# duwt/OrienMask

Hardware: AMD Instinct MI355X
Metric: images/sec end-to-end (544^2, bs=32) forward+postprocess (higher is better)
Workload: dtype f32 (fp32 tensors and accumulation; products from hi/lo fp16 pairs of the fp32 operands, three fp16 MFMAs per product group)

## Files before the change

### include/orienmask_hip.h

```cpp
#ifndef ORIENMASK_HIP_H
#define ORIENMASK_HIP_H

#include <stddef.h>
#include <stdint.h>

#ifdef __cplusplus
extern "C" {
#endif

#define OM_VERSION 140

#define OM_OK 0
#define OM_EINVAL (-1)
#define OM_ESTATE (-2)
#define OM_ENOMEM (-3)
#define OM_EHIP (-4)

#define OM_MAX_SCALES 3
#define OM_MAX_ANCHORS 9

typedef struct om_model om_model;
typedef void* om_stream;

typedef struct om_layer_info {
// ... 40 lines not shown
int om_model_layer_info(const om_model* m, int index, om_layer_info* info);
size_t om_model_weight_floats(const om_model* m);
int om_model_load_weights(om_model* m, const void* packed_dev, size_t bytes, int dtype);

size_t om_model_weight_split_words(const om_model* m);
int om_model_load_weights_split(om_model* m, const void* packed_split_dev, size_t bytes);
int om_model_set_precision(om_model* m, int mode);
int om_model_set_latency_cells(om_model* m, long long cells);
int om_model_set_latency_ksplit(om_model* m, int max_parts);
int om_model_get_precision(const om_model* m);
int om_model_set_upsample_on_read(om_model* m, int enable);

size_t om_forward_workspace_bytes(const om_model* m, int B, int H, int W);
int om_forward(om_model* m, const float* x, int B, int H, int W, float* bbox32, float* bbox16, float* bbox8,
               float* oriens, void* workspace, size_t ws_bytes, om_stream stream);
#define OM_STATUS_SPLIT_RANGE 1
#define OM_STATUS_SK_TIMEOUT 2
size_t om_forward_status_offset(const om_model* m, int B, int H, int W);

size_t om_model_weight_halfs(const om_model* m);
int om_model_load_weights_f16(om_model* m, const void* packed_f16_dev, size_t bytes);
size_t om_forward_f16_workspace_bytes(const om_model* m, int B, int H, int W);
int om_forward_f16(om_model* m, const float* x, int B, int H, int W, float* bbox32, float* bbox16, float* bbox8,
                   float* oriens, void* workspace, size_t ws_bytes, om_stream stream);
int om_layer_tile_f16(const om_model* m, int index, int B, int H, int W, int* bm, int* bn, int* algo);

int om_layer_output_view(const om_model* m, int index, int B, int H, int W, int f16, size_t* byte_offset, int* channels,
                         int* pix_stride, int* div);
int om_model_keep_activations(om_model* m, int keep);

int om_layer_tile(const om_model* m, int index, int B, int H, int W, int* bm, int* bn, int* algo);
int om_profile_enable(om_model* m, int enable);
int om_profile_enable_layers(om_model* m, const unsigned char* layer_mask, int n_layers);
int om_profile_read(om_model* m, float* layer_ms, float* layer_pre_ms, int n_layers, int* n_forwards);

int om_conv2d(const float* in, int B, int H, int W, int cin, int in_pix_stride, const float* w,
              const float* scale, const float* shift, int cout, int ksize, int stride, int leaky,
              const float* res, int res_pix_stride, float* out, int out_pix_stride, om_stream stream);
int om_conv2d_mode(const float* in, int B, int H, int W, int cin, int in_pix_stride, const float* w,
                   const float* scale, const float* shift, int cout, int ksize, int stride, int leaky,
                   const float* res, int res_pix_stride, float* out, int out_pix_stride, int out_mode, int up,
                   om_stream stream);
size_t om_conv2d_winograd_scratch_bytes(int B, int H, int W, int cin);
int om_conv2d_winograd(const float* in, int B, int H, int W, int cin, int in_pix_stride, const float* u,
                       const float* scale, const float* shift, int cout, int leaky, const float* res,
                       int res_pix_stride, float* out, int out_pix_stride, void* scratch, size_t scratch_bytes,
                       om_stream stream);
int om_conv2d_f16(const void* in, int B, int H, int W, int cin, int in_pix_stride, const void* w, const float* scale,
                  const float* shift, int cout, int ksize, int stride, int leaky, const void* res, int res_pix_stride,
                  void* out, int out_pix_stride, int out_f32, om_stream stream);
int om_conv2d_stem_f16(const float* in, int B, int H, int W, const float* w, const float* scale, const float* shift,
                       int cout, void* out, om_stream stream);
size_t om_conv2d_winograd24_scratch_bytes(int B, int H, int W, int cin);
int om_conv2d_winograd24(const float* in, int B, int H, int W, int cin, int in_pix_stride, const float* u,
                         const float* scale, const float* shift, int cout, int leaky, const float* res,
                         int res_pix_stride, float* out, int out_pix_stride, void* scratch, size_t scratch_bytes,
                         om_stream stream);
int om_conv2d_split(const float* in, int B, int H, int W, int cin, int in_pix_stride, const void* w_split,
                    const float* scale_split, const float* shift, int cout, int ksize, int stride, int leaky, const float* res,
                    int res_pix_stride, float* out, int out_pix_stride, int out_mode, int up, int tile_bm, int tile_bn,
                    int32_t* status_dev, om_stream stream);
int om_conv2d_split_k(const float* in, int B, int H, int W, int cin, int in_pix_stride, const void* w_split,
                      const float* scale_split, const float* shift, int cout, int ksize, int stride, int leaky, const float* res,
                      int res_pix_stride, float* out, int out_pix_stride, int out_mode, int up, int tile_bm, int tile_bn,
                      int max_parts, int32_t* status_dev, om_stream stream);
int om_conv2d_split_gather(int nseg, const float* const* seg_ptr, const int* seg_channels, const int* seg_pix_stride,
                           const int* seg_up, int B, int H, int W, const void* w_split, const float* scale_split, const float* shift,
                           int cout, int leaky, float* out, int out_pix_stride, int32_t* status_dev, om_stream stream);
int om_conv2d_winograd24_split(const float* in, int B, int H, int W, int cin, int in_pix_stride, const void* u_split,
                               const float* scale_split, const float* shift, int cout, int leaky, const float* res,
                               int res_pix_stride, float* out, int out_pix_stride, void* scratch, size_t scratch_bytes,
                               int32_t* status_dev, om_stream stream);
int om_conv2d_wino14_split(const float* in, int B, int H, int W, int cin, int in_pix_stride, const void* u14_split,
                           const float* scale_split, const float* shift, int cout, int leaky, const float* res,
                           int res_pix_stride, float* out, int out_pix_stride, int32_t* status_dev, om_stream stream);
int om_conv2d_wino14_blocks(int B, int H, int W, int* classes, int* row_pitch, long long* m_tiles);
size_t om_conv2d_wino14_wide_scratch_bytes(int B, int H, int W, int cin);
int om_conv2d_wino14_wide(const float* in, int B, int H, int W, int cin, int in_pix_stride, const void* u14_split,
                          const float* scale_split, const float* shift, int cout, int leaky, const float* res,
                          int res_pix_stride, float* out, int out_pix_stride, void* scratch, size_t scratch_bytes,
                          int32_t* status_dev, om_stream stream);
int om_set_wino14_wide(int on);
int om_get_wino14_wide(void);
int om_set_stem_fusion(int which, int on);
int om_get_stem_fusion(int which);
int om_set_conv3x3_f16_variant(int mode);
int om_get_conv3x3_f16_variant(void);
int om_conv2d_stem(const float* in, int B, int H, int W, const float* w, const float* scale,
                   const float* shift, int cout, float* out, om_stream stream);
int om_conv2d_stem2_split(const float* in, int B, int H, int W, const float* w1, const float* scale1, const float* shift1,
                          const void* w2_split, const float* scale2_split, const float* shift2, int cout2, int leaky2, float* out,
                          int out_pix_stride, int32_t* status_dev, om_stream stream);
int om_conv2d_stem3_split(const float* in, int B, int H, int W, const float* w1, const float* scale1, const float* shift1,
                          const void* w2_split, const float* scale2_split, const float* shift2, int cout2, int leaky2, float* out,
                          int out_pix_stride, const void* w3_split, const float* scale3_split, const float* shift3, int cout3, int leaky3,
                          float* out3, int out3_pix_stride, int32_t* status_dev, om_stream stream);
int om_conv2d_stem2_f16(const float* in, int B, int H, int W, const float* w1, const float* scale1, const float* shift1,
                        const void* w2_f16, const float* scale2, const float* shift2, int cout2, int leaky2, void* out,
                        int out_pix_stride, om_stream stream);

int om_preprocess(const float* in_nhwc, int N, int h, int w, int resize_h, int resize_w, const float* mean3,
                  const float* std3, int pad_top, int pad_left, int out_h, int out_w, float pad_value, float* out_nchw,
                  om_stream stream);
int om_pad_nchw(const float* in, long long planes, int h, int w, int pad_top, int pad_left, int out_h, int out_w,
                float pad_value, float* out, om_stream stream);

size_t om_postprocess_workspace_bytes(const om_post_cfg* cfg, int B);
int om_postprocess(const om_post_cfg* cfg, const float* bbox32, const float* bbox16, const float* bbox8,
                   const float* oriens, int B, float* out_bbox, int64_t* out_cls, uint8_t* out_mask,
                   int32_t* out_count, int32_t* out_keep, void* workspace, size_t ws_bytes, om_stream stream);
int om_postprocess_detect(const om_post_cfg* cfg, const float* bbox32, const float* bbox16, const float* bbox8, int B,
                          float* out_bbox, int64_t* out_cls, int32_t* out_count, int32_t* out_keep, void* workspace, size_t ws_bytes,
                          om_stream stream);
int om_postprocess_assemble(const om_post_cfg* cfg, const float* oriens, int B, const int32_t* out_count, uint8_t* out_mask,
                            void* workspace, size_t ws_bytes, om_stream stream);
int om_model_attach_postprocess(om_model* m, const om_post_cfg* cfg, float* out_bbox, int64_t* out_cls, uint8_t* out_mask,
                                int32_t* out_count, int32_t* out_keep, void* post_workspace, size_t post_ws_bytes);

int om_postprocess_candidates(const om_post_cfg* cfg, const float* bbox32, const float* bbox16, const float* bbox8, int B,
                              float* cand_dets, int64_t* cand_cls, int32_t* cand_field, int32_t* cand_count, void* workspace,
                              size_t ws_bytes, om_stream stream);
int om_postprocess_masks(const om_post_cfg* cfg, const float* oriens, int B, const float* dets, const int32_t* field,
                         const int32_t* count, uint8_t* out_mask, void* workspace, size_t ws_bytes, om_stream stream);

int om_post_kernel_occupancy(int which, int* threads, int* vgprs, int* lds_bytes, int* max_blocks_per_cu);

int om_recover_bbox(const float* bbox, int K, int stride, const int32_t* collate_pad6, const int32_t* pad6, int hflip,
                    int vflip, int orig_h, int orig_w, float* out_xywh, om_stream stream);
int om_recover_masks_rle(const uint8_t* mask, int K, int H, int W, int crop_top, int crop_down, int crop_left,
                         int crop_right, int hflip, int vflip, int orig_h, int orig_w, uint32_t* counts, int max_runs,
                         int32_t* n_runs, uint8_t* resized_or_null, om_stream stream);
typedef struct om_rle_image {
    const uint8_t* mask;
    int32_t K, H, W;
    int32_t crop_top, crop_down, crop_left, crop_right;
    int32_t hflip, vflip, orig_h, orig_w;
} om_rle_image;
int om_recover_masks_rle_strings(const om_rle_image* images, int n_images, uint32_t* counts, int max_runs, int32_t* n_runs,
                                 uint8_t* str_bytes, long long str_capacity, int32_t* str_cursor, int32_t* str_off,
                                 int32_t* str_len, om_stream stream);

#define OM_VIS_MAX_KEPT 512
#define OM_VIS_BATCH 16
typedef struct om_vis_image {
    const float* image;
    uint8_t* out;
    float* out_float;
    const uint8_t* mask;
    const int32_t* keep;
    const float* colors;
    const int32_t* boxes;
    int32_t n_keep, Hn, Wn;
    int32_t crop_left, crop_right, crop_top, crop_down;
    int32_t h, w;
    int32_t with_mask, draw_boxes;
    float alpha;
} om_vis_image;
size_t om_visualize_workspace_bytes(const om_vis_image* images, int n_images);
int om_visualize(const om_vis_image* images, int n_images, void* workspace, size_t ws_bytes, om_stream stream);

size_t om_cocoeval_workspace_bytes(long long bitmap_words, int n_masks);
int om_cocoeval_masks(int n_masks, const int32_t* mask_hw, const int64_t* mask_word_off, const int32_t* mask_src_first,
                      const int64_t* mask_src_word_off, int n_poly, int n_srcs, const int32_t* src_kind, const int32_t* src_mask, const int64_t* src_data_off,
                      const int32_t* src_len, const int64_t* src_word_off, const double* poly, const uint32_t* counts,
                      const uint8_t* strings, long long bitmap_words, void* workspace, size_t ws_bytes, om_stream stream);
int om_cocoeval_mask_stats(int n_masks, long long bitmap_words, const void* workspace, int32_t* stats, om_stream stream);
// ... 146 lines not shown
```

### orienmask_amd/csrc/conv_igemm_split.hip

```cpp
#include <cstdlib>

#include "conv_f16_common.h"

namespace om {

struct IgemmSParams {
    const _Float16* in;
    const _Float16* w;
    const float* scale;
    const float* shift;
    const float* res;
    float* out;
    int* ticket;
    int* status;
    int H, W, cin_h, in_pix_stride_h;
    int Ho, Wo, HoWo, cout;
    int ks, stride, pad;
    int M, kc, ksteps, taps;
    int n_tiles, total_tiles;
    float* partial;
    int* kflags;
    int ksplit, total_tickets, m_tiles;
    int leaky, res_pix_stride, out_pix_stride, out_mode, up;
    int vec_io;
    int total_in_pixels;
    int w_bytes;
    int nseg, nimg;
    const _Float16* seg_ptr[4];
    int seg_stride_h[4], seg_shift[4], seg_end[4];
};

template <int BM, int BN>
constexpr int split_blocks_per_cu() { return BM * BN >= 256 * 128 ? 2 : (BM * BN >= 128 * 128 ? 3 : 4); }

template <int BM, int BN, int WM, int WN, bool FAST = false>
__device__ __forceinline__ void split_epilogue(const IgemmSParams& p, f32x4* smem, const f32x16 (&acc)[WM / 32][WN / 32],
                                               int m0, int n0, int tid, int wm, int wn, int fi, int fk, float (&sc)[8], float (&sh)[8]) {
    constexpr int TM = WM / 32, TN = WN / 32;
    constexpr int CH8 = BN / 8;
    constexpr int RP = 256 / CH8;
    constexpr int CH = BN / 4;
    f32x4* sC = smem;
    const int n8 = tid % CH8, r0 = tid / CH8;
    const int n = n0 + n8 * 8;
    const int nvalid = p.cout - n;
    const bool vec = p.vec_io && nvalid >= 8;
    if constexpr (!FAST) {
#pragma unroll
        for (int k = 0; k < 8; ++k) { sc[k] = p.scale[n + k]; sh[k] = p.shift[n + k]; }
    }
    float nonfinite = 0.f;
#pragma unroll 1
    for (int pass = 0; pass < BM / WM; ++pass) {
        if (wm == pass) {
#pragma unroll
            for (int a = 0; a < TM; ++a) {
                const int ml = a * 32 + fi;
#pragma unroll
                for (int b = 0; b < TN; ++b)
#pragma unroll
                    for (int g = 0; g < 4; ++g) {
                        const int n4 = (wn * WN + b * 32) / 4 + 2 * g + fk;
                        f32x4 v = {acc[a][b][4 * g], acc[a][b][4 * g + 1], acc[a][b][4 * g + 2], acc[a][b][4 * g + 3]};
                        sC[ml * CH + (n4 ^ (ml & 7))] = v;
                    }
            }
        }
        asm volatile("s_waitcnt lgkmcnt(0)" ::: "memory");
        __builtin_amdgcn_s_barrier();
        if constexpr (FAST) {
#pragma unroll
            for (int ps = 0; ps < (WM + RP - 1) / RP; ++ps) {
                const int ml = ps * RP + r0;
                const int m = m0 + pass * WM + ml;
                if (ml >= WM) continue;
                const f32x4 v0 = sC[ml * CH + ((2 * n8) ^ (ml & 7))];
                const f32x4 v1 = sC[ml * CH + ((2 * n8 + 1) ^ (ml & 7))];
                float v[8] = {v0[0], v0[1], v0[2], v0[3], v1[0], v1[1], v1[2], v1[3]};
#pragma unroll
                for (int k = 0; k < 8; ++k) {
                    const float t = fmaf(v[k], sc[k], sh[k]);
                    v[k] = p.leaky ? (t > 0.f ? t : t * 0.1f) : t;
                    nonfinite = fmaf(t, 0.f, nonfinite);
                }
                if (m < p.M) {
                    float* o = p.out + (size_t)m * p.out_pix_stride + n;
                    *reinterpret_cast<f32x4*>(o) = f32x4{v[0], v[1], v[2], v[3]};
                    *reinterpret_cast<f32x4*>(o + 4) = f32x4{v[4], v[5], v[6], v[7]};
                }
            }
        } else if (p.out_mode != 2) {
#pragma unroll 2
            for (int ps = 0; ps < (WM + RP - 1) / RP; ++ps) {
                const int ml = ps * RP + r0;
                const int m = m0 + pass * WM + ml;
                if (ml >= WM || m >= p.M || nvalid <= 0) continue;
                const f32x4 v0 = sC[ml * CH + ((2 * n8) ^ (ml & 7))];
                const f32x4 v1 = sC[ml * CH + ((2 * n8 + 1) ^ (ml & 7))];
                float v[8] = {v0[0], v0[1], v0[2], v0[3], v1[0], v1[1], v1[2], v1[3]};
#pragma unroll
                for (int k = 0; k < 8; ++k) {
                    const float t = fmaf(v[k], sc[k], sh[k]);
                    v[k] = p.leaky ? (t > 0.f ? t : t * 0.1f) : t;
                    nonfinite = fmaf(t, 0.f, nonfinite);
                }
                if (p.out_mode == 0) {
                    float* o = p.out + (size_t)m * p.out_pix_stride + n;
                    if (p.res) {
                        const float* rp = p.res + (size_t)m * p.res_pix_stride + n;
                        if (vec) {
                            const f32x4 ra = *reinterpret_cast<const f32x4*>(rp), rb = *reinterpret_cast<const f32x4*>(rp + 4);
#pragma unroll
                            for (int k = 0; k < 4; ++k) { v[k] += ra[k]; v[4 + k] += rb[k]; }
                        } else {
                            for (int k = 0; k < 8 && k < nvalid; ++k) v[k] += rp[k];
                        }
                    }
                    if (vec) {
                        *reinterpret_cast<f32x4*>(o) = f32x4{v[0], v[1], v[2], v[3]};
                        *reinterpret_cast<f32x4*>(o + 4) = f32x4{v[4], v[5], v[6], v[7]};
                    } else {
                        for (int k = 0; k < 8 && k < nvalid; ++k) o[k] = v[k];
                    }
                } else {
                    const int bi = m / p.HoWo;
                    const int rr = m - bi * p.HoWo;
                    const int oy = rr / p.Wo, ox = rr - oy * p.Wo;
                    const int Wu = p.Wo * p.up;
                    const size_t base = ((size_t)bi * p.Ho * p.up + (size_t)oy * p.up) * Wu + (size_t)ox * p.up;
                    for (int dy = 0; dy < p.up; ++dy)
                        for (int dx = 0; dx < p.up; ++dx) {
                            float* o = p.out + (base + (size_t)dy * Wu + dx) * p.out_pix_stride + n;
                            if (vec) {
                                *reinterpret_cast<f32x4*>(o) = f32x4{v[0], v[1], v[2], v[3]};
                                *reinterpret_cast<f32x4*>(o + 4) = f32x4{v[4], v[5], v[6], v[7]};
                            } else {
                                for (int k = 0; k < 8 && k < nvalid; ++k) o[k] = v[k];
                            }
                        }
                }
            }
        } else {
            const float* sCf = reinterpret_cast<const float*>(smem);
            const int nch = min(BN, p.cout - n0);
            for (int idx = tid; idx < nch * WM; idx += 256) {
                const int nl = idx / WM, ml = idx - nl * WM;
                const int m = m0 + pass * WM + ml;
                if (m >= p.M) continue;
                const int nn = n0 + nl;
                float t = fmaf(sCf[(ml * CH + ((nl >> 2) ^ (ml & 7))) * 4 + (nl & 3)], p.scale[nn], p.shift[nn]);
                nonfinite = fmaf(t, 0.f, nonfinite);
                if (p.leaky) t = t > 0.f ? t : t * 0.1f;
                const int bi = m / p.HoWo;
                const int rr = m - bi * p.HoWo;
                p.out[((size_t)bi * p.cout + nn) * p.HoWo + rr] = t;
            }
        }
        asm volatile("s_waitcnt lgkmcnt(0)" ::: "memory");
        __builtin_amdgcn_s_barrier();
    }
    if (p.status && nonfinite != nonfinite) atomicOr(p.status, OM_STATUS_SPLIT_RANGE);
}

template <int BN>
__device__ __forceinline__ void split_scale_shift(const IgemmSParams& p, int n0, int tid, float (&sc)[8], float (&sh)[8]) {
    const int n = n0 + (tid % (BN / 8)) * 8;
    const f32x4 a0 = *reinterpret_cast<const f32x4*>(p.scale + n), a1 = *reinterpret_cast<const f32x4*>(p.scale + n + 4);
    const f32x4 b0 = *reinterpret_cast<const f32x4*>(p.shift + n), b1 = *reinterpret_cast<const f32x4*>(p.shift + n + 4);
#pragma unroll
    for (int k = 0; k < 4; ++k) { sc[k] = a0[k]; sc[4 + k] = a1[k]; sh[k] = b0[k]; sh[4 + k] = b1[k]; }
}

__device__ __forceinline__ void split8(const f32x4& x0, const f32x4& x1, f16x8& hi, f16x8& lo) {
#pragma unroll
    for (int i = 0; i < 4; ++i) {
        hi[i] = (_Float16)x0[i];
        hi[4 + i] = (_Float16)x1[i];
    }
#pragma unroll
    for (int i = 0; i < 4; ++i) {
        lo[i] = (_Float16)(x0[i] - (float)hi[i]);
        lo[4 + i] = (_Float16)(x1[i] - (float)hi[4 + i]);
    }
}

template <int BM, int BN, int WM, int WN, bool FAST = false, int NBUF = 3>
__global__ __launch_bounds__(256, (NBUF > 3 ? 2 : split_blocks_per_cu<BM, BN>())) void conv_igemm_split_kernel(const IgemmSParams p) {
    constexpr int TM = WM / 32, TN = WN / 32;
    constexpr int NWN = BN / WN;
    constexpr int A_CH = BM / 64, B_CH = (BN + 63) / 64, NP = A_CH + B_CH;
    constexpr int STAGE = (BM + (BN < 64 ? 64 : BN)) * 4;
    static_assert((BM / WM) * (BN / WN) == 4, "four waves per workgroup");
    static_assert(BM % 64 == 0, "A tile = whole 64-row pieces");
    static_assert(WM * BN / 4 <= NBUF * STAGE, "one wave-row of the fp32 C tile must fit in the operand ring");
    __shared__ f32x4 smem[NBUF * STAGE + 1];
    int* const s_ticket = reinterpret_cast<int*>(smem + NBUF * STAGE);
    constexpr bool KSPLIT = NBUF > 3;

    const int tid = threadIdx.x;
    const int lane = tid & 63;
    const int wave = tid >> 6;
    const int wave_u = __builtin_amdgcn_readfirstlane(wave);
    const int wm = wave / NWN, wn = wave % NWN;
    const int lrow = tid >> 2, lcol = tid & 3;
    const int scol = lcol ^ ((lrow >> 2) & 3);
    const int fi = lane & 31, fk = lane >> 5;
    const int fsw = (fi >> 2) & 3;

    for (int round = 0;; ++round) {
        int tile;
        int s_begin = 0, nsteps = p.ksteps;
        [[maybe_unused]] int part = 0;
        int tile_n, tile_m;
        if constexpr (KSPLIT) {
            if (round) break;
            const int b = blockIdx.x, x = b & 7;
            int unit = b >> 3;
            for (int y = 0; y < x; ++y) unit += (p.total_tickets - y + 7) >> 3;
            tile_m = unit % p.m_tiles;
            const int t = unit / p.m_tiles;
            tile_n = t % p.n_tiles;
            part = t / p.n_tiles;
            tile = tile_m * p.n_tiles + tile_n;
            s_begin = part * p.ksteps / p.ksplit;
            nsteps = (part + 1) * p.ksteps / p.ksplit - s_begin;
        } else {
            if (tid == 0) *s_ticket = atomicAdd(p.ticket, 1);
            asm volatile("s_waitcnt lgkmcnt(0)" ::: "memory");
            __builtin_amdgcn_s_barrier();
            tile = *s_ticket;
            if (tile >= p.total_tiles) break;
            tile = __builtin_amdgcn_readfirstlane(tile);
            tile_n = tile % p.n_tiles;
            tile_m = tile / p.n_tiles;
        }
        const int m0 = tile_m * BM, n0 = tile_n * BN;

        int rowoff[A_CH];
        unsigned invmask[A_CH];
        const int b_first = (m0 < p.M ? m0 : p.M - 1) / p.HoWo;
#pragma unroll
        for (int j = 0; j < A_CH; ++j) {
            int m = m0 + lrow + 64 * j;
            const bool mok = m < p.M;
            if (!mok) m = p.M - 1;
            const int b = m / p.HoWo;
            const int rr = m - b * p.HoWo;
            const int oy = rr / p.Wo;
            const int ox = rr - oy * p.Wo;
            const int iy0 = oy * p.stride - p.pad, ix0 = ox * p.stride - p.pad;
            rowoff[j] = (((b - b_first) * p.H * p.W + iy0 * p.W + ix0) * p.in_pix_stride_h + scol * 8) * 2;
            unsigned badrow = 0, badcol = 0;
#pragma unroll
            for (int k = 0; k < 3; ++k) {
                badrow |= ((unsigned)(iy0 + k) < (unsigned)p.H ? 0u : 1u) << k;
// ... 76 lines not shown
#pragma unroll
        for (int st = 0; st < NBUF; ++st) {
#pragma unroll
            for (int piece = 0; piece < NP; ++piece) issue_piece(piece, st, st < nsteps);
            advance();
        }
        asm volatile("s_waitcnt vmcnt(%0)" ::"i"((NBUF - 1) * NP) : "memory");
        __builtin_amdgcn_s_barrier();
        read_raw(0);
        convert();
        int buf = 0;
        for (int s = 0; s < nsteps; ++s) {
            const int buf1 = buf == NBUF - 1 ? 0 : buf + 1;
            asm volatile("s_waitcnt vmcnt(%0) lgkmcnt(0)" ::"i"((NBUF - 2) * NP) : "memory");
            __builtin_amdgcn_s_barrier();
            read_raw(buf1);
            const bool live3 = s + NBUF < nsteps;
#pragma unroll
            for (int piece = 0; piece < NP; ++piece) issue_piece(piece, buf, live3);
#pragma unroll
            for (int a = 0; a < TM; ++a)
#pragma unroll
                for (int b = 0; b < TN; ++b) {
                    acc[a][b] = __builtin_amdgcn_mfma_f32_32x32x16_f16(bh[b], al[a], acc[a][b], 0, 0, 0);
                    acc[a][b] = __builtin_amdgcn_mfma_f32_32x32x16_f16(bl[b], ah[a], acc[a][b], 0, 0, 0);
                    acc[a][b] = __builtin_amdgcn_mfma_f32_32x32x16_f16(bh[b], ah[a], acc[a][b], 0, 0, 0);
                }
            convert();
            buf = buf1;
            advance();
        }
        asm volatile("s_waitcnt vmcnt(0) lgkmcnt(0)" ::: "memory");
        __syncthreads();

        if constexpr (KSPLIT) {
            if (p.ksplit > 1) {
                const auto rs_part = __builtin_amdgcn_make_buffer_rsrc(p.partial, 0, 0x7FFFFFFF, 0x00020000);
                constexpr int PART_BYTES = TM * TN * 4 * 256 * 16;
                const int pbase = (tile * p.ksplit + part) * PART_BYTES + tid * 16;
#pragma unroll
                for (int a = 0; a < TM; ++a)
#pragma unroll
                    for (int b = 0; b < TN; ++b)
#pragma unroll
                        for (int g = 0; g < 4; ++g) {
                            const f32x4 v = {acc[a][b][4 * g], acc[a][b][4 * g + 1], acc[a][b][4 * g + 2], acc[a][b][4 * g + 3]};
                            __builtin_amdgcn_raw_buffer_store_b128(__builtin_bit_cast(__attribute__((__vector_size__(4 * sizeof(unsigned)))) unsigned, v),
                                                                   rs_part, pbase, ((a * TN + b) * 4 + g) * 256 * 16, 16);
                        }
                asm volatile("s_waitcnt vmcnt(0)" ::: "memory");
                __syncthreads();
                if (tid == 0) s_ticket[1] = __hip_atomic_fetch_add(p.kflags + tile, 1, __ATOMIC_RELAXED, __HIP_MEMORY_SCOPE_AGENT);
                __syncthreads();
                if (s_ticket[1] != p.ksplit - 1) break;
#pragma unroll
                for (int a = 0; a < TM; ++a)
#pragma unroll
                    for (int b = 0; b < TN; ++b)
#pragma unroll
                        for (int r = 0; r < 16; ++r) acc[a][b][r] = 0.f;
                for (int q = 0; q < p.ksplit; ++q) {
                    const int qbase = (tile * p.ksplit + q) * PART_BYTES + tid * 16;
#pragma unroll
                    for (int a = 0; a < TM; ++a)
#pragma unroll
                        for (int b = 0; b < TN; ++b)
#pragma unroll
                            for (int g = 0; g < 4; ++g) {
                                const f32x4 v = __builtin_bit_cast(f32x4, __builtin_amdgcn_raw_buffer_load_b128(rs_part, qbase, ((a * TN + b) * 4 + g) * 256 * 16, 16));
#pragma unroll
                                for (int k = 0; k < 4; ++k) acc[a][b][4 * g + k] += v[k];
                            }
                }
                asm volatile("s_waitcnt vmcnt(0)" ::: "memory");
            }
        }

        float sc[8], sh[8];
        if constexpr (FAST) split_scale_shift<BN>(p, n0, tid, sc, sh);
        split_epilogue<BM, BN, WM, WN, FAST>(p, smem, acc, m0, n0, tid, wm, wn, fi, fk, sc, sh);
    }
}

template <int BM, int BN, int WM, int WN, bool GATHER = false, bool FAST = false, int NBUF = 2>
__global__ __launch_bounds__(256, 2) void conv_igemm_split_wide_kernel(const IgemmSParams p) {
    constexpr int TM = WM / 32, TN = WN / 32;
    constexpr int NWN = BN / WN;
    constexpr int A_CH = BM / 32, B_CH = BN / 32, NP = A_CH + B_CH;
    constexpr bool KSPLIT = NBUF > 2;
    static_assert(!(KSPLIT && GATHER), "the deep-ring form has no gathered input");
    constexpr int STAGE = (BM + BN) * 8;
    static_assert((BM / WM) * (BN / WN) == 4, "four waves per workgroup");
    static_assert(BM % 32 == 0 && BN % 32 == 0, "whole 32-row pieces");
    static_assert(WM * BN / 4 <= NBUF * STAGE, "one wave-row of the fp32 C tile must fit in the operand ring");
    __shared__ f32x4 smem[NBUF * STAGE + 1];
    int* const s_ticket = reinterpret_cast<int*>(smem + NBUF * STAGE);

    const int tid = threadIdx.x;
    const int lane = tid & 63;
    const int wave = tid >> 6;
    const int wave_u = __builtin_amdgcn_readfirstlane(wave);
    const int wm = wave / NWN, wn = wave % NWN;
    const int lrow = tid >> 3, lcol = tid & 7;
    const int scol = lcol ^ ((lrow >> 1) & 7);
    const int fi = lane & 31, fk = lane >> 5;
    const int fsw = (fi >> 1) & 7;

    if constexpr (!KSPLIT) {
        if (tid == 0) *s_ticket = atomicAdd(p.ticket, 1);
        asm volatile("s_waitcnt lgkmcnt(0)" ::: "memory");
        __builtin_amdgcn_s_barrier();
    }
    for (int round = 0;; ++round) {
        int tile, tile_n, tile_m;
        [[maybe_unused]] int part = 0;
        if constexpr (KSPLIT) {
            if (round) break;
            const int b = blockIdx.x, x = b & 7;
            int unit = b >> 3;
            for (int y = 0; y < x; ++y) unit += (p.total_tickets - y + 7) >> 3;
            tile_m = unit % p.m_tiles;
            const int t = unit / p.m_tiles;
            tile_n = t % p.n_tiles;
            part = t / p.n_tiles;
            tile = tile_m * p.n_tiles + tile_n;
        } else {
            tile = *s_ticket;
            if (tile >= p.total_tiles) break;
            tile = __builtin_amdgcn_readfirstlane(tile);
            tile_n = tile % p.n_tiles;
            tile_m = tile / p.n_tiles;
        }
        const int m0 = tile_m * BM, n0 = tile_n * BN;

        int rowoff[A_CH];
        unsigned invmask[A_CH];
        [[maybe_unused]] int g_img[A_CH], g_y[A_CH], g_x[A_CH];
        const int b_first = (m0 < p.M ? m0 : p.M - 1) / p.HoWo;
#pragma unroll
        for (int j = 0; j < A_CH; ++j) {
            int m = m0 + lrow + 32 * j;
            const bool mok = m < p.M;
            if (!mok) m = p.M - 1;
            const int b = m / p.HoWo;
            const int rr = m - b * p.HoWo;
            const int oy = rr / p.Wo;
            const int ox = rr - oy * p.Wo;
            const int iy0 = oy * p.stride - p.pad, ix0 = ox * p.stride - p.pad;
            rowoff[j] = (((b - b_first) * p.H * p.W + iy0 * p.W + ix0) * p.in_pix_stride_h + scol * 8) * 2;
            if constexpr (GATHER) { g_img[j] = b - b_first; g_y[j] = oy; g_x[j] = ox; }
            unsigned badrow = 0, badcol = 0;
#pragma unroll
            for (int k = 0; k < 3; ++k) {
                badrow |= ((unsigned)(iy0 + k) < (unsigned)p.H ? 0u : 1u) << k;
                badcol |= ((unsigned)(ix0 + k) < (unsigned)p.W ? 0u : 1u) << k;
            }
            unsigned inv;
            if (p.ks == 3) {
                inv = ((badrow & 1u) ? 0x007u : 0u) | ((badrow & 2u) ? 0x038u : 0u) | ((badrow & 4u) ? 0x1C0u : 0u) | badcol * 0x49u;
            } else {
                inv = (badrow | badcol) & 1u;
            }
            invmask[j] = mok ? inv : 0xFFFFFFFFu;
        }
        int rowoffB[B_CH];
        const int row_halfs = p.taps * p.cin_h;
#pragma unroll
        for (int j = 0; j < B_CH; ++j) rowoffB[j] = ((n0 + lrow + 32 * j) * row_halfs + scol * 8) * 2;
        const _Float16* in_base = p.in + (size_t)b_first * p.H * p.W * p.in_pix_stride_h;
        const size_t in_left = ((size_t)p.total_in_pixels - (size_t)b_first * p.H * p.W) * p.in_pix_stride_h * 2;
        int in_bytes = in_left < 0x7FFFFFFFull ? (int)in_left : 0x7FFFFFFF;
        [[maybe_unused]] int seg = 0, seg_c0 = 0, seg_c1 = 0x7FFFFFFF;
        [[maybe_unused]] auto set_segment = [&](int g) {
            auto pick = [g](const auto (&v)[4]) { return g == 0 ? v[0] : g == 1 ? v[1] : g == 2 ? v[2] : v[3]; };
            const int sh = pick(p.seg_shift), Hs = p.Ho >> sh, Ws = p.Wo >> sh, st = pick(p.seg_stride_h);
            in_base = pick(p.seg_ptr) + (size_t)b_first * Hs * Ws * st;
            const size_t left = (size_t)(p.nimg - b_first) * Hs * Ws * st * 2;
            in_bytes = left < 0x7FFFFFFFull ? (int)left : 0x7FFFFFFF;
#pragma unroll
            for (int j = 0; j < A_CH; ++j)
                rowoff[j] = (((g_img[j] * Hs + (g_y[j] >> sh)) * Ws + (g_x[j] >> sh)) * st + scol * 8) * 2;
            seg = g;
            seg_c0 = g == 0 ? 0 : g == 1 ? p.seg_end[0] : g == 2 ? p.seg_end[1] : p.seg_end[2];
            seg_c1 = pick(p.seg_end);
        };
        if constexpr (GATHER) set_segment(0);

        const int kc2 = p.kc >> 1;
        int nstages = p.taps * kc2;
        int n_kh = 0, n_kw = 0, n_cc = 0;
        if constexpr (KSPLIT) {
            const int s_begin = part * nstages / p.ksplit;
            nstages = (part + 1) * nstages / p.ksplit - s_begin;
            const int tap0 = s_begin / kc2;
            n_cc = s_begin - tap0 * kc2;
            n_kh = tap0 / p.ks;
            n_kw = tap0 - n_kh * p.ks;
        }
        auto advance = [&]() {
            if (++n_cc == kc2) {
                n_cc = 0;
                if (++n_kw == p.ks) { n_kw = 0; ++n_kh; }
            }
        };
        auto issue_piece = [&](int piece, int buf, bool live) {
            f32x4* dst = smem + buf * STAGE + wave_u * 64;
            if (piece < A_CH) {
                const int j = piece;
                if constexpr (GATHER) {
                    if (piece == 0 && live && n_cc >= seg_c1) set_segment(seg + 1);
                }
                const auto rs_in = __builtin_amdgcn_make_buffer_rsrc(const_cast<_Float16*>(in_base), 0, live ? in_bytes : 0, 0x00020000);
                const int tap = n_kh * p.ks + n_kw;
                const int tap_off = GATHER ? (n_cc - seg_c0) * 128
                                           : ((n_kh * p.W + n_kw) * p.in_pix_stride_h + n_cc * 64) * 2;
                const int voff = (rowoff[j] + tap_off) | ((invmask[j] << (31 - tap)) & 0x80000000u);
                __builtin_amdgcn_raw_ptr_buffer_load_lds(rs_in, (lds_ptr_t)(dst + j * 256), 16, voff, 0, 0, 0);
            } else {
                const int j = piece - A_CH;
                const auto rs_w = __builtin_amdgcn_make_buffer_rsrc(const_cast<_Float16*>(p.w), 0, live ? p.w_bytes : 0, 0x00020000);
                const int koff = ((n_kh * p.ks + n_kw) * p.cin_h + n_cc * 64) * 2;
                const int vo = rowoffB[j] + koff;
                __builtin_amdgcn_raw_ptr_buffer_load_lds(rs_w, (lds_ptr_t)(dst + BM * 8 + j * 256), 16, vo, 0, 0, 0);
            }
        };

// ... 35 lines not shown
                    acc[a][b] = __builtin_amdgcn_mfma_f32_32x32x16_f16(bh[b], ah[a], acc[a][b], 0, 0, 0);
                }
        };

#pragma unroll
        for (int st = 0; st < NBUF; ++st) {
#pragma unroll
            for (int piece = 0; piece < NP; ++piece) issue_piece(piece, st, st < nstages);
            advance();
        }
        [[maybe_unused]] int next_ticket = 0;
        if constexpr (!KSPLIT) {
            if (tid == 0) next_ticket = atomicAdd(p.ticket, 1);
        }
        asm volatile("s_waitcnt vmcnt(%0)" ::"i"((NBUF - 1) * NP) : "memory");
        __builtin_amdgcn_s_barrier();
        read_raw(0, 0);
        convert();
        int buf = 0;
        for (int s = 0; s < nstages; ++s) {
            read_raw(buf, 1);
            multiply();
            convert();
            asm volatile("s_waitcnt vmcnt(%0) lgkmcnt(0)" ::"i"((NBUF - 2) * NP) : "memory");
            __builtin_amdgcn_s_barrier();
            const bool live2 = s + NBUF < nstages;
#pragma unroll
            for (int piece = 0; piece < NP; ++piece) issue_piece(piece, buf, live2);
            advance();
            const int buf1 = buf == NBUF - 1 ? 0 : buf + 1;
            read_raw(buf1, 0);
            multiply();
            convert();
            buf = buf1;
        }
        asm volatile("s_waitcnt vmcnt(0) lgkmcnt(0)" ::: "memory");
        if constexpr (!KSPLIT) {
            if (tid == 0) *s_ticket = next_ticket;
        }
        __syncthreads();
        if constexpr (KSPLIT) {
            if (p.ksplit > 1) {
                const auto rs_part = __builtin_amdgcn_make_buffer_rsrc(p.partial, 0, 0x7FFFFFFF, 0x00020000);
                constexpr int PART_BYTES = TM * TN * 4 * 256 * 16;
                const int pbase = (tile * p.ksplit + part) * PART_BYTES + tid * 16;
#pragma unroll
                for (int a = 0; a < TM; ++a)
#pragma unroll
                    for (int b = 0; b < TN; ++b)
#pragma unroll
                        for (int g = 0; g < 4; ++g) {
                            const f32x4 v = {acc[a][b][4 * g], acc[a][b][4 * g + 1], acc[a][b][4 * g + 2], acc[a][b][4 * g + 3]};
                            __builtin_amdgcn_raw_buffer_store_b128(__builtin_bit_cast(__attribute__((__vector_size__(4 * sizeof(unsigned)))) unsigned, v),
                                                                   rs_part, pbase, ((a * TN + b) * 4 + g) * 256 * 16, 16);
                        }
                asm volatile("s_waitcnt vmcnt(0)" ::: "memory");
                __syncthreads();
                if (tid == 0) s_ticket[1] = __hip_atomic_fetch_add(p.kflags + tile, 1, __ATOMIC_RELAXED, __HIP_MEMORY_SCOPE_AGENT);
                __syncthreads();
                if (s_ticket[1] != p.ksplit - 1) break;
#pragma unroll
                for (int a = 0; a < TM; ++a)
#pragma unroll
                    for (int b = 0; b < TN; ++b)
#pragma unroll
                        for (int r = 0; r < 16; ++r) acc[a][b][r] = 0.f;
                for (int q = 0; q < p.ksplit; ++q) {
                    const int qbase = (tile * p.ksplit + q) * PART_BYTES + tid * 16;
#pragma unroll
                    for (int a = 0; a < TM; ++a)
#pragma unroll
                        for (int b = 0; b < TN; ++b)
#pragma unroll
                            for (int g = 0; g < 4; ++g) {
                                const f32x4 v = __builtin_bit_cast(f32x4, __builtin_amdgcn_raw_buffer_load_b128(rs_part, qbase, ((a * TN + b) * 4 + g) * 256 * 16, 16));
#pragma unroll
                                for (int kk = 0; kk < 4; ++kk) acc[a][b][4 * g + kk] += v[kk];
                            }
                }
                asm volatile("s_waitcnt vmcnt(0)" ::: "memory");
            }
        }

        split_epilogue<BM, BN, WM, WN, FAST>(p, smem, acc, m0, n0, tid, wm, wn, fi, fk, sc, sh);
    }
}

template <int BM, int BN, int WM, int WN, bool WIDE = false, bool GATHER = false, int NBUF = 3, int WSTAGES = 0>
static int launch_tile_split(IgemmSParams p, int cout_pad, int blocks_per_cu, hipStream_t stream) {
    const int m_tiles = (p.M + BM - 1) / BM;
    p.n_tiles = cout_pad / BN;
    const long long total = (long long)m_tiles * p.n_tiles;
    OM_REQUIRE(total > 0 && total < (1ll << 31), OM_EINVAL, "conv split: %lld tiles out of range", total);
    p.total_tiles = (int)total;
    constexpr bool DEEP = WIDE ? WSTAGES > 2 : NBUF > 3;
    int parts = 1;
    if constexpr (DEEP) {
        if (p.ksplit > 1 && p.partial && total <= SK_SLOTS) {
            parts = p.ksplit;
            if (parts > 512 / (int)total) parts = 512 / (int)total;
            if (parts > p.ksteps / 16) parts = p.ksteps / 16;
            if (parts > 8) parts = 8;
            if (parts < 1) parts = 1;
        }
    }
    p.ksplit = parts;
    p.total_tickets = p.total_tiles * parts;
    p.m_tiles = m_tiles;
    const long long tickets = total * parts;
    long long grid = tickets < 256ll * blocks_per_cu ? tickets : 256ll * blocks_per_cu;
    if constexpr (DEEP) {
        OM_REQUIRE(tickets <= 512, OM_EINVAL, "conv split: %lld units in a deep-ring launch", tickets);
        grid = tickets;
    }
    const bool fast = p.out_mode == 0 && !p.res && p.vec_io && p.cout == cout_pad;
    if constexpr (WIDE) {
        constexpr int WNBUF = DEEP ? WSTAGES : 2;
        if (fast) hipLaunchKernelGGL((conv_igemm_split_wide_kernel<BM, BN, WM, WN, GATHER, true, WNBUF>), dim3((unsigned)grid), dim3(256), 0, stream, p);
        else hipLaunchKernelGGL((conv_igemm_split_wide_kernel<BM, BN, WM, WN, GATHER, false, WNBUF>), dim3((unsigned)grid), dim3(256), 0, stream, p);
    } else {
        if (fast) hipLaunchKernelGGL((conv_igemm_split_kernel<BM, BN, WM, WN, true, NBUF>), dim3((unsigned)grid), dim3(256), 0, stream, p);
        else hipLaunchKernelGGL((conv_igemm_split_kernel<BM, BN, WM, WN, false, NBUF>), dim3((unsigned)grid), dim3(256), 0, stream, p);
    }
    OM_CHECK_HIP(hipGetLastError());
    return OM_OK;
}

void conv_tile_for_split(int M, int cout_pad, int* bm, int* bn, bool gather) {
    if (gather) { *bm = 128; *bn = 128; return; }
    struct Cand { int bm, bn; double eff; };
    const Cand cands[] = {{128, 128, 1.00}, {256, 128, 0.91}, {128, 64, 0.82}, {64, 64, 0.69}, {128, 32, 0.57}};
    double best = 1e300;
    for (const Cand& c : cands) {
        if (cout_pad % c.bn) continue;
        const double cost = (double)((M + c.bm - 1) / c.bm) * (cout_pad / c.bn) * c.bm * c.bn / c.eff;
        if (cost < best) { best = cost; *bm = c.bm; *bn = c.bn; }
    }
    const Cand small[] = {{128, 64, 0}, {64, 64, 0}};
    for (const Cand& c : small) {
        const long long tiles = (long long)((M + *bm - 1) / *bm) * (cout_pad / *bn);
        if (tiles > 128 || cout_pad % c.bn || c.bm * c.bn >= *bm * *bn) continue;
        *bm = c.bm; *bn = c.bn;
    }
}

int launch_conv_igemm_split(const ConvArgs& a, hipStream_t stream) {
    OM_REQUIRE((a.in || a.nseg > 0) && a.w && a.scale && a.shift && a.out, OM_EINVAL, "conv split: null pointer");
    OM_REQUIRE(a.cin % 16 == 0 && a.cin >= 16, OM_EINVAL, "conv split: cin=%d must be a multiple of 16", a.cin);
    OM_REQUIRE(a.ks == 1 || a.ks == 3, OM_EINVAL, "conv split: ksize=%d not supported", a.ks);
    OM_REQUIRE(a.stride == 1 || a.stride == 2, OM_EINVAL, "conv split: stride=%d not supported", a.stride);
    OM_REQUIRE((a.nseg > 0 || (a.in_pix_stride % 4 == 0 && (reinterpret_cast<uintptr_t>(a.in) & 15) == 0)) &&
                   (reinterpret_cast<uintptr_t>(a.w) & 15) == 0,
               OM_EINVAL, "conv split: input view / weights must be 16-byte aligned");
    OM_REQUIRE(a.cout_pad % 32 == 0 && a.cout <= a.cout_pad, OM_EINVAL, "conv split: cout_pad=%d", a.cout_pad);
    OM_REQUIRE((long long)a.B * a.H * a.W * a.in_pix_stride < (1ll << 40) && (long long)a.B * a.H * a.W < (1ll << 31) &&
                   (long long)a.B * a.Ho * a.Wo < (1ll << 31),
               OM_EINVAL, "conv split: problem too large");
    OM_REQUIRE(!(a.res && a.out_mode != 0), OM_EINVAL, "conv split: residual only with plain NHWC output");
    OM_REQUIRE(a.ticket, OM_EINVAL, "conv split: the tile queue needs a zeroed ticket word");
    IgemmSParams p;
    p.in = reinterpret_cast<const _Float16*>(a.in); p.w = reinterpret_cast<const _Float16*>(a.w);
    p.scale = a.scale; p.shift = a.shift; p.res = a.res; p.out = a.out; p.ticket = a.ticket; p.status = a.status;
    p.H = a.H; p.W = a.W; p.cin_h = 2 * a.cin; p.in_pix_stride_h = 2 * a.in_pix_stride;
    p.Ho = a.Ho; p.Wo = a.Wo; p.HoWo = a.Ho * a.Wo; p.cout = a.cout;
    p.ks = a.ks; p.stride = a.stride; p.pad = a.ks / 2;
    p.M = a.B * a.Ho * a.Wo; p.taps = a.ks * a.ks;
    p.kc = a.cin / 16;
    p.ksteps = p.taps * p.kc;
    p.leaky = a.leaky; p.res_pix_stride = a.res_pix_stride; p.out_pix_stride = a.out_pix_stride;
    p.out_mode = a.out_mode; p.up = a.up;
    p.n_tiles = 0; p.total_tiles = 0;
    p.partial = a.sk_partial; p.kflags = a.ticket + SK_FLAG_OFF; p.ksplit = a.ksplit_max; p.total_tickets = 0;
    p.total_in_pixels = a.B * a.H * a.W;
    p.w_bytes = a.cout_pad * p.taps * a.cin * 4;
    p.vec_io = (a.out_mode != 2 && a.out_pix_stride % 4 == 0 && (reinterpret_cast<uintptr_t>(a.out) & 15) == 0 &&
                (!a.res || (a.res_pix_stride % 4 == 0 && (reinterpret_cast<uintptr_t>(a.res) & 15) == 0)))
                   ? 1 : 0;
    p.nseg = 0; p.nimg = a.B;
    for (int g = 0; g < 4; ++g) { p.seg_ptr[g] = p.in; p.seg_stride_h[g] = 0; p.seg_shift[g] = 0; p.seg_end[g] = 0x7FFFFFFF; }
    if (a.nseg > 0) {
        OM_REQUIRE(a.nseg <= 4 && a.ks == 1 && a.stride == 1 && a.cout_pad % 128 == 0, OM_EINVAL,
                   "conv split: a gathered input needs a 1x1 stride-1 layer with cout_pad %% 128 == 0 and at most 4 segments (nseg=%d ks=%d "
                   "stride=%d cout_pad=%d)", a.nseg, a.ks, a.stride, a.cout_pad);
        int end = 0;
        for (int g = 0; g < a.nseg; ++g) {
            const int up = a.seg_up[g];
            int sh = 0;
            while ((1 << sh) < up) ++sh;
            OM_REQUIRE(a.seg_ptr[g] && up >= 1 && (1 << sh) == up && a.H % up == 0 && a.W % up == 0 && a.seg_channels[g] > 0 &&
                           a.seg_channels[g] % 32 == 0 && a.seg_pix_stride[g] % 4 == 0 && a.seg_pix_stride[g] >= a.seg_channels[g] &&
                           (reinterpret_cast<uintptr_t>(a.seg_ptr[g]) & 15) == 0,
                       OM_EINVAL, "conv split: segment %d (channels=%d pix_stride=%d up=%d) of a gathered input", g, a.seg_channels[g],
                       a.seg_pix_stride[g], up);
            end += a.seg_channels[g] / 32;
            p.seg_ptr[g] = reinterpret_cast<const _Float16*>(a.seg_ptr[g]);
            p.seg_stride_h[g] = 2 * a.seg_pix_stride[g]; p.seg_shift[g] = sh; p.seg_end[g] = end;
        }
        OM_REQUIRE(end * 32 == a.cin, OM_EINVAL, "conv split: the segments hold %d channels, the layer reads %d", end * 32, a.cin);
        p.nseg = a.nseg;
        p.in = p.seg_ptr[0];
    }
    int bm, bn;
    conv_tile_for_split(p.M, a.cout_pad, &bm, &bn, a.nseg > 0);
    OM_REQUIRE(a.nseg == 0 || (bm == 128 && bn == 128), OM_EINVAL, "conv split: no gathered-input kernel with a %d x %d tile", bm, bn);
    if (a.nseg > 0) return launch_tile_split<128, 128, 64, 64, true, true>(p, a.cout_pad, 2, stream);
    if (a.force_bm || a.force_bn) {
        const bool built = (a.force_bm == 256 && a.force_bn == 128) || (a.force_bm == 128 && (a.force_bn == 128 || a.force_bn == 64 || a.force_bn == 32)) ||
                           (a.force_bm == 64 && a.force_bn == 64);
        OM_REQUIRE(built && a.cout_pad % a.force_bn == 0, OM_EINVAL, "conv split: %d x %d is not a built tile shape for cout_pad=%d",
                   a.force_bm, a.force_bn, a.cout_pad);
        bm = a.force_bm; bn = a.force_bn;
    }
    if (bm == 256 && bn == 128) return launch_tile_split<256, 128, 128, 64>(p, a.cout_pad, 2, stream);
    if (bm == 128 && bn == 128 && a.cin % 32 == 0 && !a.force_bm) return launch_tile_split<128, 128, 64, 64, true>(p, a.cout_pad, 2, stream);
    if (bm == 128 && bn == 128) return launch_tile_split<128, 128, 64, 64>(p, a.cout_pad, 3, stream);
    const long long ntile = (long long)((p.M + bm - 1) / bm) * (a.cout_pad / bn);
    const bool deep = ntile <= 256 && (!a.force_bm || a.ksplit_max >= 1);
    if (deep && a.cin % 32 == 0) {
        if (bm == 128 && bn == 64) return launch_tile_split<128, 64, 64, 32, true, false, 3, 3>(p, a.cout_pad, 2, stream);
        if (bm == 64 && bn == 64) return launch_tile_split<64, 64, 32, 32, true, false, 3, 4>(p, a.cout_pad, 2, stream);
    }
    if (bm == 128 && bn == 64 && deep) return launch_tile_split<128, 64, 64, 32, false, false, 5>(p, a.cout_pad, 2, stream);
    if (bm == 64 && bn == 64 && deep) return launch_tile_split<64, 64, 32, 32, false, false, 8>(p, a.cout_pad, 2, stream);
    if (bm == 128 && bn == 64) return launch_tile_split<128, 64, 64, 32>(p, a.cout_pad, 4, stream);
    if (bm == 64 && bn == 64) return launch_tile_split<64, 64, 32, 32>(p, a.cout_pad, 4, stream);
    return launch_tile_split<128, 32, 32, 32>(p, a.cout_pad, 4, stream);
}

}
```

### orienmask_amd/csrc/conv_wino14.hip

```cpp
#include "wino14_shared.h"

namespace om {

constexpr int W14_RING = 4;
constexpr int W14_EMAX = 144;
constexpr int W14_VPLANE = W14_EMAX * 4;
constexpr int W14_VBUF = 6 * W14_VPLANE;
constexpr int W14_UGRP = 3 * W14_BN * 4;
constexpr int W14_THREADS = 768;

template <int MODE>
__global__ __launch_bounds__(W14_THREADS, 3) void wino14_split_kernel(const Wino14Params p) {
    __shared__ f32x4 smem[2 * W14_VBUF + W14_RING * W14_UGRP + 1];
    int* const s_ticket = reinterpret_cast<int*>(smem + 2 * W14_VBUF + W14_RING * W14_UGRP);
    f32x4* const s_u = smem + 2 * W14_VBUF;

    const int tid = threadIdx.x;
    const int lane = tid & 63;
    const int wave = __builtin_amdgcn_readfirstlane(tid >> 6);
    const int ngroups = 6 * p.nch;

    int q_xcd = 0, q_hops = 0;
    auto draw_tile = [&]() {
        const int m_tiles = p.total_tiles / p.n_tiles;
// ... 237 lines not shown
            for (int r = 0; r < 16; ++r) acc[j][r] = 0.f;
        if (W14_EPI_OPS<MODE> == 0 || first_of_wg) asm volatile("s_waitcnt vmcnt(0)" ::: "memory");
        else asm volatile("s_waitcnt vmcnt(%0)" ::"n"(W14_EPI_OPS<MODE>) : "memory");
        first_of_wg = false;
        __builtin_amdgcn_s_barrier();
        const int next_tile = __builtin_amdgcn_readfirstlane(s_ticket[tslot ^ 1]);
        f32x4 ca[4], na[4];
        auto read_a = [&](f32x4(&f)[4], const f32x4* sV, int j, int ky) {
            f[0] = sV[w14_plane(j) * W14_VPLANE + aoff_hi[ky]];
            f[1] = sV[w14_plane(j) * W14_VPLANE + aoff_lo[ky]];
        };
        auto read_b = [&](f32x4(&f)[4], int ky, int slot) {
            f[2] = s_u[slot * W14_UGRP + ky * (W14_BN * 4) + boff_hi];
            f[3] = s_u[slot * W14_UGRP + ky * (W14_BN * 4) + boff_lo];
        };
        auto read_frags = [&](f32x4(&f)[4], const f32x4* sV, int j, int ky, int slot) {
            read_a(f, sV, j, ky);
            read_b(f, ky, slot);
        };
        read_frags(ca, smem, 0, 0, 0);
        auto mma = [&](const f32x4(&f)[4], auto plc) {
            constexpr int pl = decltype(plc)::value;
            const f16x8 ah = __builtin_bit_cast(f16x8, f[0]), al = __builtin_bit_cast(f16x8, f[1]);
            const f16x8 bh = __builtin_bit_cast(f16x8, f[2]), bl = __builtin_bit_cast(f16x8, f[3]);
            acc[pl] = __builtin_amdgcn_mfma_f32_32x32x16_f16(bh, al, acc[pl], 0, 0, 0);
            acc[pl] = __builtin_amdgcn_mfma_f32_32x32x16_f16(bl, ah, acc[pl], 0, 0, 0);
            acc[pl] = __builtin_amdgcn_mfma_f32_32x32x16_f16(bh, ah, acc[pl], 0, 0, 0);
        };
        int g = 0;
        for (int c = 0; c < p.nch; ++c) {
            const f32x4* sV = smem + (c & 1) * W14_VBUF;
            [[maybe_unused]] const f32x4* sVn = smem + ((c & 1) ^ 1) * W14_VBUF;
            auto group = [&](auto jc) {
                constexpr int j = decltype(jc)::value;
                const int slot = g % W14_RING, slot1 = slot == W14_RING - 1 ? 0 : slot + 1;
#pragma unroll
                for (int ky = 0; ky < 3; ++ky) {
                    if (ky < 2) read_frags(na, sV, j, ky + 1, slot);
                    else if (j < 5) read_frags(na, sV, j + 1, 0, slot1);
                    else if (c + 1 < p.nch) read_frags(na, sVn, 0, 0, slot1);
                    mma(ca, std::integral_constant<int, w14_plane(j)>{});
#pragma unroll
                    for (int i = 0; i < 4; ++i) ca[i] = na[i];
                    if (ky == 0) issue_group(ubase, g + W14_RING - 1);
                }
                if (g + W14_RING - 1 >= ngroups) asm volatile("s_waitcnt vmcnt(0) lgkmcnt(0)" ::: "memory");
                else if (wave < 4) asm volatile("s_waitcnt vmcnt(2) lgkmcnt(0)" ::: "memory");
                else asm volatile("s_waitcnt vmcnt(1) lgkmcnt(0)" ::: "memory");
                __builtin_amdgcn_s_barrier();
                ++g;
            };
            group(std::integral_constant<int, 0>{});
            group(std::integral_constant<int, 1>{});
            group(std::integral_constant<int, 2>{});
            group(std::integral_constant<int, 3>{});
            group(std::integral_constant<int, 4>{});
            group(std::integral_constant<int, 5>{});
        }
        Wino14Tile tn = tl;
        if (next_tile < p.total_tiles) wino14_decode(p, next_tile, tn);
        wino14_epilogue<MODE>(p, acc, tl, smem + W14_VBUF + wave * 256, wm, wn, lane, [&]() {
            if (next_tile < p.total_tiles) {
                const int ub = tn.tile_n * p.nch * 6 * (W14_UGRP * 16);
                issue_group(ub, 0);
                issue_group(ub, 1);
                issue_group(ub, 2);
            }
        });
        tl = tn;
        tile = next_tile;
        tslot ^= 1;
    }
}

constexpr int W14B_UGRP = 2 * W14_UGRP;

struct Wino14VParams {
    const float* in;
    _Float16* v;
    int B, H, W, in_ps, in_bytes, nch, TW, gtot;
    long long items;
};

__device__ __forceinline__ f32x4 w14_point(const f32x4 (&d)[6], int j) {
    const f32x4 c4 = 4.f, cm4 = -4.f, c2 = 2.f, cm2 = -2.f, cm5 = -5.f;
    switch (j) {
        case 0: return __builtin_elementwise_fma(d[2], cm5, __builtin_elementwise_fma(d[0], c4, d[4]));
        case 1: return __builtin_elementwise_fma(d[1] + d[2], cm4, d[3] + d[4]);
        case 2: return __builtin_elementwise_fma(d[1] - d[2], c4, d[4] - d[3]);
        case 3: return __builtin_elementwise_fma(d[3] - d[1], c2, d[4] - d[2]);
        case 4: return __builtin_elementwise_fma(d[3] - d[1], cm2, d[4] - d[2]);
        default: return __builtin_elementwise_fma(d[3], cm5, __builtin_elementwise_fma(d[1], c4, d[5]));
    }
}

__global__ __launch_bounds__(256) void wino14_v_kernel(const Wino14VParams p) {
    const long long id = (long long)blockIdx.x * 256 + threadIdx.x;
    if (id >= p.items) return;
    const int o = (int)(id & 1);
    long long r = id >> 1;
    const int t = (int)(r % p.TW); r /= p.TW;
    const int c = (int)(r % p.nch); r /= p.nch;
    const int b = (int)(r / p.H), y = (int)(r - (long long)b * p.H);
    const auto rs_in = __builtin_amdgcn_make_buffer_rsrc(const_cast<float*>(p.in), 0, p.in_bytes, 0x00020000);
    f32x4 d[2][6];
#pragma unroll
    for (int x = 0; x < 6; ++x) {
        const int px = 4 * t - 1 + x;
        const bool ok = (unsigned)px < (unsigned)p.W;
        const int off = ok ? (((b * p.H + y) * p.W + px) * p.in_ps + 16 * c + 8 * o) * 4 : (int)0x80000000;
        d[0][x] = __builtin_bit_cast(f32x4, __builtin_amdgcn_raw_buffer_load_b128(rs_in, off, 0, 0));
        d[1][x] = __builtin_bit_cast(f32x4, __builtin_amdgcn_raw_buffer_load_b128(rs_in, ok ? off + 16 : off, 0, 0));
    }
    const long long G = (long long)b * (p.H + 2) + y + 1;
#pragma unroll
    for (int j = 0; j < 6; ++j) {
        f16x8 h, l;
#pragma unroll
        for (int q = 0; q < 2; ++q) {
            const f32x4 v = w14_point(d[q], j);
            const f16x4 hh = __builtin_convertvector(v, f16x4);
            f32x4 rem;
#pragma unroll
            for (int k = 0; k < 4; ++k) rem[k] = __builtin_fmaf((float)hh[k], -1.0f, v[k]);
            const f16x4 ll = __builtin_convertvector(rem, f16x4);
#pragma unroll
            for (int k = 0; k < 4; ++k) { h[4 * q + k] = hh[k]; l[4 * q + k] = ll[k]; }
        }
        _Float16* e = p.v + ((((long long)c * 6 + j) * p.gtot + G) * p.TW + t) * 32;
        *reinterpret_cast<f16x8*>(e + 8 * o) = h;
        *reinterpret_cast<f16x8*>(e + 16 + 8 * o) = l;
    }
}

struct Wino14WideParams {
    Wino14Params k;
    const _Float16* v;
    int v_bytes, TW;
};

template <int MODE>
__global__ __launch_bounds__(512, 2) void wino14_wide_kernel(const Wino14WideParams pw) {
    const Wino14Params& p = pw.k;
    static_assert(W14_EMAX == 144, "the nine 1-KiB pieces of a V plane and the 128-entry sub-tile offsets below assume 144 entries");
    __shared__ f32x4 smem[2 * W14_VBUF + 2 * W14B_UGRP + 1];
    f32x4* const s_u = smem + 2 * W14_VBUF;
    int* const s_ticket = reinterpret_cast<int*>(smem + 2 * W14_VBUF + 2 * W14B_UGRP);
    const int tid = threadIdx.x, lane = tid & 63;
    const int wave = __builtin_amdgcn_readfirstlane(tid >> 6);
    const int wm2 = wave >> 2, wn4 = wave & 3;
    const int fi = lane & 31, fk = lane >> 5;
    const int ngroups = 6 * p.nch;
    const int n_tiles2 = p.n_tiles >> 1, total2 = (p.total_tiles / p.n_tiles) * n_tiles2;
    const int TW = pw.TW, hp2 = p.H + 2;
    const int ecount = (p.R + 2) * p.Ct;
    const auto rs_u = __builtin_amdgcn_make_buffer_rsrc(const_cast<_Float16*>(p.u), 0, p.u_bytes, 0x00020000);
    const auto rs_v = __builtin_amdgcn_make_buffer_rsrc(const_cast<_Float16*>(pw.v), 0, pw.v_bytes, 0x00020000);
    const int drow = lane >> 2, dcol = lane & 3;
    int dvo[3], dhalf[3];
#pragma unroll
    for (int i = 0; i < 3; ++i) {
        const int piece = wave + 8 * i;
        dhalf[i] = piece >= 12;
        const int row = 16 * (piece - 12 * dhalf[i]) + drow;
        dvo[i] = row * 64 + ((dcol ^ ((row >> 2) & 3)) * 16);
    }
    const int swB = (fi >> 2) & 3;
    const int brow = (wn4 >> 1) * (W14_UGRP) + (32 * (wn4 & 1) + fi) * 4;
    const int boff_hi = brow + (fk ^ swB), boff_lo = brow + ((2 + fk) ^ swB);
    int aoff_hi[3], aoff_lo[3];
#pragma unroll
    for (int ky = 0; ky < 3; ++ky) {
        const int e = 64 * wm2 + fi + ky * p.Ct;
        const int sw = (e >> 2) & 3;
        aoff_hi[ky] = e * 4 + (fk ^ sw);
        aoff_lo[ky] = e * 4 + ((2 + fk) ^ sw);
    }
    auto issue_group = [&](int tn2, int g) {
        if (g >= ngroups) return;
        const int slot = g & 1;
        const int c = g / 6, j = g - 6 * c;
#pragma unroll
        for (int i = 0; i < 3; ++i) {
            const int t64 = 2 * tn2 + dhalf[i];
            const int soff = ((t64 * p.nch + c) * 6 + w14_plane(j)) * (W14_UGRP * 16);
            __builtin_amdgcn_raw_ptr_buffer_load_lds(rs_u, (lds_ptr_t)(s_u + slot * W14B_UGRP + (wave + 8 * i) * 64), 16, dvo[i], soff, 0, 0);
        }
    };
    int vsrc[2];
    auto setup_v = [&](const Wino14Tile& tl) {
#pragma unroll
        for (int i = 0; i < 2; ++i) {
            const int e = 16 * (wave + 8 * i) + drow;
            const int rr = e / p.Ct, t = e - rr * p.Ct;
            const int sw = (e >> 2) & 3;
            const int g = tl.g0 - 1 + rr;
            const int b = g / hp2;
            const int y = g - b * hp2 - 1;
            const bool ok = e < ecount && g >= 0 && g < p.gtot && y >= 0 && y < p.H && tl.t0 + t < TW;
            vsrc[i] = ok ? ((g * TW + tl.t0 + t) * 64 + ((dcol ^ sw) * 16)) : (int)0x80000000;
        }
    };
    auto issue_v_plane = [&](int c, int pl, int vb) {
        if (c >= p.nch) return;
        const int soff = (c * 6 + pl) * (p.gtot * TW * 64);
        __builtin_amdgcn_raw_ptr_buffer_load_lds(rs_v, (lds_ptr_t)(smem + vb * W14_VBUF + pl * W14_VPLANE + wave * 64), 16, vsrc[0], soff, 0, 0);
        if (wave == 0)
            __builtin_amdgcn_raw_ptr_buffer_load_lds(rs_v, (lds_ptr_t)(smem + vb * W14_VBUF + pl * W14_VPLANE + 8 * 64), 16, vsrc[1], soff, 0, 0);
    };
    f32x16 acc[2][6];
    for (;;) {
// ... 169 lines not shown
    s.npix = (long long)a.B * a.H * a.W;
    s.in_bytes = (s.npix - 1) * a.in_pix_stride * 4 + (long long)a.cin * 4;
    s.out_bytes = ((s.npix - 1) * a.out_pix_stride + a.cout) * 4;
    s.res_bytes = has_res ? ((s.npix - 1) * a.res_pix_stride + a.cout) * 4 : 0;
    s.aligned_in = a.in_pix_stride % 4 == 0 && in_align_bytes >= 16;
    s.fast_io = a.cout % 4 == 0 && a.out_pix_stride % 4 == 0 && out_align_bytes >= 16 &&
                (!has_res || (a.res_pix_stride % 4 == 0 && res_align_bytes >= 16)) && s.out_bytes < 0x7FFFFFF0ll && s.res_bytes < 0x7FFFFFF0ll;
    long long m_tiles = 0;
    if (fused) {
        s.ncls = wino14_blocks(a.B, a.H, a.W, s.cls, &s.hp, &s.gtot, &m_tiles);
    } else {
        wino14_geometry(a.B, a.H, a.W, &s.R, &s.Ct, &s.ncb, &s.nrb);
        s.hp = a.H + 2; s.gtot = (long long)a.B * s.hp;
        m_tiles = (long long)s.nrb * s.ncb;
        s.ncls = s.R >= 1 && s.Ct >= 1 ? 1 : 0;
        s.cls[0] = Wino14Class{0, s.Ct, s.ncb, s.R, s.nrb, 0};
    }
    if (s.ncls == 1) s.cls[1] = Wino14Class{0, s.cls[0].Ct, s.cls[0].ncb, s.cls[0].R, 0, m_tiles < (1ll << 31) ? (int)m_tiles : 0};
    s.total_tiles = m_tiles * (a.cout_pad / W14_BN);
    s.u_bytes = wino14_weight_halfs(a.cout_pad, a.cin) * 2;
    return s;
}
static bool wino14_layer_kind_ok(const ConvArgs& a) { return a.ks == 3 && a.stride == 1 && a.out_mode == 0 && a.cin % 16 == 0 && a.cin >= 16 && a.cout_pad % 64 == 0; }

static int wino14_fill_params(const ConvArgs& a, bool fused, Wino14Params& p) {
    OM_REQUIRE(a.in && a.w && a.scale && a.shift && a.out && a.ticket, OM_EINVAL, "wino14: null pointer");
    OM_REQUIRE(wino14_layer_kind_ok(a), OM_EINVAL, "wino14: 3x3 stride-1 NHWC layers only, cin=%d cout_pad=%d", a.cin, a.cout_pad);
    OM_REQUIRE((reinterpret_cast<uintptr_t>(a.w) & 15) == 0, OM_EINVAL, "wino14: the weights must be 16-byte aligned");
    const Wino14Shape s = wino14_shape(a, fused, align_bytes(a.in), align_bytes(a.out), a.res != nullptr, align_bytes(a.res));
    OM_REQUIRE(s.fits(), OM_EINVAL, "wino14: %d x %d x %d: input view (%lld bytes) not 16-byte aligned, or it, the weights, %lld pixels or "
               "%lld tiles (first block %d x %d) out of range", a.B, a.H, a.W, s.in_bytes, s.npix, s.total_tiles, s.cls[0].R, s.cls[0].Ct);
    p.in = a.in; p.u = reinterpret_cast<const _Float16*>(a.w); p.scale = a.scale; p.shift = a.shift; p.res = a.res; p.out = a.out;
    p.ticket = a.ticket; p.status = a.status;
    p.B = a.B; p.H = a.H; p.W = a.W; p.in_ps = a.in_pix_stride; p.in_bytes = (int)s.in_bytes;
    p.cout = a.cout; p.out_ps = a.out_pix_stride; p.res_ps = a.res_pix_stride; p.leaky = a.leaky;
    p.fast_io = s.fast_io ? 1 : 0;
    p.out_bytes = s.fast_io ? (int)s.out_bytes : 0;
    p.res_bytes = s.fast_io ? (int)s.res_bytes : 0;
    p.R = s.R; p.Ct = s.Ct; p.ncb = s.ncb; p.gtot = (int)s.gtot; p.hp = s.hp;
    for (int k = 0; k < W14_MAXCLS; ++k) p.cls[k] = s.cls[k];
    p.n_tiles = a.cout_pad / W14_BN;
    p.nch = a.cin / 16;
    p.total_tiles = (int)s.total_tiles;
    p.u_bytes = (int)s.u_bytes;
    return OM_OK;
}

int launch_conv_wino14_split(const ConvArgs& a, hipStream_t stream) {
    Wino14Params p;
    if (int rc = wino14_fill_params(a, true, p)) return rc;
    const long long total = p.total_tiles;
    const long long grid = total < 256 ? total : 256;
    if (!p.fast_io) hipLaunchKernelGGL(wino14_split_kernel<2>, dim3((unsigned)grid), dim3(W14_THREADS), 0, stream, p);
    else if (a.res) hipLaunchKernelGGL(wino14_split_kernel<1>, dim3((unsigned)grid), dim3(W14_THREADS), 0, stream, p);
    else hipLaunchKernelGGL(wino14_split_kernel<0>, dim3((unsigned)grid), dim3(W14_THREADS), 0, stream, p);
    OM_CHECK_HIP(hipGetLastError());
    return OM_OK;
}

size_t wino14_wide_scratch_floats(int B, int H, int W, int cin) {
    return (size_t)(cin / 16) * 6 * B * (H + 2) * ((W + 3) / 4) * 16;
}

bool wino14_wide_supported(const ConvArgs& a, int in_align_bytes, int out_align_bytes, bool has_res, int res_align_bytes) {
    if (!wino14_layer_kind_ok(a) || a.cout_pad % 128) return false;
    const Wino14Shape s = wino14_shape(a, false, in_align_bytes, out_align_bytes, has_res, res_align_bytes);
    return s.fits() && s.fast_io && wino14_wide_scratch_floats(a.B, a.H, a.W, a.cin) * 4 < 0x7FFFFFF0ull;
}

int launch_conv_wino14_wide(const ConvArgs& a, float* scratch, hipStream_t stream) {
    OM_REQUIRE(scratch && (reinterpret_cast<uintptr_t>(scratch) & 15) == 0, OM_EINVAL, "wino14 wide: scratch must be 16-byte aligned");
    OM_REQUIRE(wino14_wide_supported(a, align_bytes(a.in), align_bytes(a.out), a.res != nullptr, align_bytes(a.res)), OM_EINVAL,
               "wino14 wide: cout_pad=%d must be a multiple of 128, the views 16-byte aligned and, like V, below 2 GiB", a.cout_pad);
    Wino14WideParams pw;
    if (int rc = wino14_fill_params(a, false, pw.k)) return rc;
    const int TW = (a.W + 3) / 4;
    pw.TW = TW;
    pw.v = reinterpret_cast<const _Float16*>(scratch);
    pw.v_bytes = (int)(wino14_wide_scratch_floats(a.B, a.H, a.W, a.cin) * 4);
    Wino14VParams pv;
    pv.in = a.in; pv.v = reinterpret_cast<_Float16*>(scratch);
    pv.B = a.B; pv.H = a.H; pv.W = a.W; pv.in_ps = a.in_pix_stride; pv.in_bytes = pw.k.in_bytes; pv.nch = pw.k.nch; pv.TW = TW; pv.gtot = pw.k.gtot;
    pv.items = (long long)a.B * a.H * TW * pv.nch * 2;
    hipLaunchKernelGGL(wino14_v_kernel, dim3((unsigned)((pv.items + 255) / 256)), dim3(256), 0, stream, pv);
    OM_CHECK_HIP(hipGetLastError());
    if (a.mid_event) OM_CHECK_HIP(hipEventRecord(a.mid_event, stream));
    const long long total2 = (long long)(pw.k.total_tiles / pw.k.n_tiles) * (pw.k.n_tiles / 2);
    const unsigned grid = (unsigned)(total2 < 256 ? total2 : 256);
    if (a.res) hipLaunchKernelGGL(wino14_wide_kernel<1>, dim3(grid), dim3(512), 0, stream, pw);
    else hipLaunchKernelGGL(wino14_wide_kernel<0>, dim3(grid), dim3(512), 0, stream, pw);
    OM_CHECK_HIP(hipGetLastError());
    return OM_OK;
}

}
```

### orienmask_amd/csrc/om_common.h

```cpp
#pragma once
#include <hip/hip_runtime.h>
#include <cstdarg>
#include <cstdint>
#include <cstdio>

#include "../../include/orienmask_hip.h"

namespace om {

void set_error(const char* fmt, ...);

#define OM_CHECK_HIP(expr)                                                              \
    do {                                                                                \
        hipError_t _e = (expr);                                                         \
        if (_e != hipSuccess) {                                                         \
            om::set_error("%s failed: %s (%s:%d)", #expr, hipGetErrorString(_e), __FILE__, __LINE__); \
            return OM_EHIP;                                                             \
        }                                                                               \
    } while (0)

#define OM_REQUIRE(cond, code, ...)                                                     \
    do {                                                                                \
        if (!(cond)) {                                                                  \
            om::set_error(__VA_ARGS__);                                                 \
            return (code);                                                              \
        }                                                                               \
    } while (0)

static inline int round_up(int v, int m) { return (v + m - 1) / m * m; }
static inline size_t align_up(size_t v, size_t a) { return (v + a - 1) / a * a; }
static inline int align_bytes(uintptr_t addr) { return (int)((addr | 256) & (~(addr | 256) + 1)); }
static inline int align_bytes(const void* p) { return align_bytes(reinterpret_cast<uintptr_t>(p)); }

struct ConvArgs {
    const float* in;
    const float* w;
    const float* scale;
    const float* shift;
    const float* res;
    float* out;
    int* ticket = nullptr;
    float* sk_partial = nullptr;
    hipEvent_t mid_event = nullptr;
    int B, H, W, cin, in_pix_stride;
    int Ho, Wo, cout, cout_pad;
    int ks, stride;
    int leaky;
    int res_pix_stride;
    int out_pix_stride;
    int out_mode;
    int up;
    int split = 0;
    int* status = nullptr;
    int ksplit_max = 0;
    int force_bm = 0, force_bn = 0;
    int nseg = 0;
    const float* seg_ptr[4] = {nullptr, nullptr, nullptr, nullptr};
    int seg_channels[4] = {0, 0, 0, 0}, seg_pix_stride[4] = {0, 0, 0, 0}, seg_up[4] = {1, 1, 1, 1};
};

constexpr int SK_SLOTS = 1024;
constexpr int SK_FLAG_OFF = 16;
constexpr int SYNC_WORDS = SK_FLAG_OFF + SK_SLOTS;
constexpr int STATUS_WORDS = 16;
constexpr size_t SK_PARTIAL_BYTES = (size_t)512 * 32 * 256 * 16;

int launch_conv_igemm(const ConvArgs& a, hipStream_t stream);
int launch_conv_igemm_split(const ConvArgs& a, hipStream_t stream);
void conv_tile_for_split(int M, int cout_pad, int* bm, int* bn, bool gather = false);

struct ConvArgsH {
    const void* in;
    const void* w;
    const float* scale;
    const float* shift;
    const void* res;
    void* out;
    int* ticket = nullptr;
    int B, H, W, cin, in_pix_stride;
    int Ho, Wo, cout, cout_pad;
    int ks, stride;
    int leaky;
    int res_pix_stride;
    int out_pix_stride;
    int out_mode;
    int up;
    int out_f32;
    int nseg = 0;
    const void* seg_ptr[4] = {nullptr, nullptr, nullptr, nullptr};
    int seg_channels[4] = {0, 0, 0, 0}, seg_pix_stride[4] = {0, 0, 0, 0}, seg_up[4] = {1, 1, 1, 1};
};
int launch_conv_igemm_f16(const ConvArgsH& a, hipStream_t stream);
int launch_conv3x3_f16(const ConvArgsH& a, hipStream_t stream);
bool conv3x3_f16_supported(const ConvArgsH& a);
void conv3x3_tile_for_f16(int M, int cout_pad, int W, int kc, int* bm, int* bn);
int conv3x3_f16_get_tall();
void conv3x3_f16_set_tall(int mode);
void conv_tile_for_f16(int M, int cout_pad, int cin, int* bm, int* bn, bool gather = false);
inline size_t conv_f16_weight_halfs(int cout_pad, int ks, int cin) {
    return (size_t)cout_pad * ks * ks * cin;
}
int launch_conv_stem_f16(const float* in_nchw, int B, int H, int W, const float* w, const float* scale,
                         const float* shift, int cout, void* out_nhwc_f16, hipStream_t stream);
void conv_tile_for(int M, int cout_pad, int* bm, int* bn);
int launch_conv_winograd(const ConvArgs& a, float* scratch, hipStream_t stream);
size_t wino_scratch_floats(int B, int H, int W, int C);
int launch_conv_winograd24(const ConvArgs& a, float* scratch, hipStream_t stream);
size_t wino24_scratch_floats(int B, int H, int W, int C);
int launch_conv_wino14_split(const ConvArgs& a, hipStream_t stream);
size_t wino14_wide_scratch_floats(int B, int H, int W, int cin);
bool wino14_wide_supported(const ConvArgs& a, int in_align_bytes, int out_align_bytes, bool has_res, int res_align_bytes);
int launch_conv_wino14_wide(const ConvArgs& a, float* scratch, hipStream_t stream);
bool stem2_f16_supported(int B, int H, int W, int cout2, int out_pix_stride, int out_align_bytes);
int launch_conv_stem2_f16(const float* in_nchw, int B, int H, int W, const float* w1, const float* scale1, const float* shift1,
                          const void* w2_f16, const float* scale2, const float* shift2, int cout2, int leaky2, void* out_nhwc_f16,
                          int out_pix_stride, hipStream_t stream);
struct Stem2Third {
    const void* w_split;
    const float* scale_split;
    const float* shift;
    float* out;
    int cout, leaky, out_pix_stride;
};
bool stem2_split_supported(int B, int H, int W, int cout2, int out_pix_stride, int out_align_bytes, int cout3 = 0,
                           int out3_pix_stride = 0, int out3_align_bytes = 0);
int launch_conv_stem2_split(const float* in_nchw, int B, int H, int W, const float* w1, const float* scale1, const float* shift1,
                            const void* w2_split, const float* scale2_split, const float* shift2, int cout2, int leaky2,
                            float* out_nhwc, int out_pix_stride, int* status, hipStream_t stream, const Stem2Third* third = nullptr);
size_t wino14_weight_halfs(int cout_pad, int cin);
void wino14_geometry(int B, int H, int W, int* R, int* Ct, int* ncb, int* nrb);
constexpr int W14_MAXCLS = 2;
struct Wino14Class {
    int t0, Ct, ncb, R, nrb, m0;
};
int wino14_blocks(int B, int H, int W, Wino14Class* cls, int* pitch, long long* gtot, long long* m_tiles);
bool wino_enabled();
int wino_bn(long long T, int cout_pad);
bool wino_fused_for(int cin);
int launch_zero_words(void* ptr, size_t n_words, hipStream_t stream);
int launch_conv_stem(const float* in_nchw, int B, int H, int W, const float* w, const float* scale,
                     const float* shift, int cout, float* out_nhwc, hipStream_t stream);

}
```

### orienmask_amd/csrc/om_model.cpp

```cpp
#include <algorithm>
#include <atomic>
#include <cstdlib>
#include <cstring>
#include <mutex>
#include <string>
#include <vector>

#include "om_common.h"

namespace om {

static thread_local char g_err[512] = "";

void set_error(const char* fmt, ...) {
    va_list ap;
    va_start(ap, fmt);
    vsnprintf(g_err, sizeof(g_err), fmt, ap);
    va_end(ap);
}

enum : int { BUF_INPUT = -1, BUF_BBOX32 = -2, BUF_BBOX16 = -3, BUF_BBOX8 = -4, BUF_ORIENS = -5 };
constexpr int HEAD_PIX_STRIDE = 256;

struct BufDef {
    int div;
    int C;
};

struct View {
    int buf;
    int ch_off;
};

struct LayerDef {
    om_layer_info info;
    View in, out, res;
    bool has_res = false;
    bool stem = false;
    int in_div = 1;
    int out_mode = 0, up = 1;
    int side = -1;
    struct Seg { int producer; View view; int channels, up; };
    std::vector<Seg> gather;
};

enum class Form {
    Stem,
    Stem2Split, Stem3Split, Stem2F16,
    InPrevious,
    Igemm,
    Split, SplitGather, SplitDirect3x3,
    Wino, WinoFused, Wino24,
    Wino14, Wino14Wide,
    IgemmF16, IgemmF16Gather,
    Conv3x3F16, Conv3x3F16Tall,
};

struct LayerPlan {
    Form form = Form::Stem;
    int bm = 0, bn = 0;
    size_t scratch_floats = 0;
    enum Blob { F32, SPLIT, F16 } blob = F32;
    int64_t w_off = -1, scale_off = -1;
    int ksplit_max = 0;
    bool to_side = false;
    bool gather = false;
};

static int algo_code(Form f, bool f16) {
    switch (f) {
        case Form::Stem: return 0;
        case Form::Igemm: case Form::IgemmF16: return 1;
        case Form::Wino: return 2;
        case Form::WinoFused: return 3;
        case Form::Conv3x3F16: return 4;
        case Form::Wino24: case Form::IgemmF16Gather: return 5;
        case Form::Conv3x3F16Tall: return 6;
        case Form::Split: case Form::SplitDirect3x3: case Form::Stem2F16: return 7;
        case Form::Wino14: return 8;
        case Form::Stem2Split: case Form::Stem3Split: return 9;
        case Form::InPrevious: return f16 ? 8 : 10;
        case Form::SplitGather: return 11;
        case Form::Wino14Wide: return 12;
    }
    return -1;
}

template <class Args>
static void fill_conv_shape(Args& a, int B, int H, int W, int cin, int in_pix_stride, int cout, int cout_pad, int ks, int stride, int leaky,
                            int res_pix_stride, int out_pix_stride, int out_mode = 0, int up = 1) {
    a.B = B; a.H = H; a.W = W; a.cin = cin; a.in_pix_stride = in_pix_stride;
    a.Ho = H / stride; a.Wo = W / stride; a.cout = cout; a.cout_pad = cout_pad;
    a.ks = ks; a.stride = stride; a.leaky = leaky; a.res_pix_stride = res_pix_stride;
    a.out_pix_stride = out_pix_stride; a.out_mode = out_mode; a.up = up;
}

}

enum : int { SW_STEM3 = 0, SW_STEM2_F16 = 1, SW_W14_WIDE = 2 };
static int switch_default(const char* env) {
    const char* e = std::getenv(env);
    return (e && e[0] == '1') ? 0 : 1;
}
static std::atomic<int>& switch_flag(int which) {
    static std::atomic<int> flags[3] = {{switch_default("OM_NO_STEM3")}, {switch_default("OM_NO_STEM2_F16")}, {switch_default("OM_NO_W14_WIDE")}};
    return flags[which];
}
static bool switch_on(int which) { return switch_flag(which).load(std::memory_order_relaxed) != 0; }

struct om_model {
    int num_anchors = 0, num_classes = 0;
    int variant = 0;
    std::vector<om::BufDef> bufs;
    std::vector<om::LayerDef> layers;
    size_t weight_floats = 0;
    const float* weights = nullptr;
    size_t weight_halfs = 0;
    const _Float16* weights16 = nullptr;
    size_t split_words = 0;
    const float* weights_split = nullptr;
    int precision = 0;
    bool profiling = false;
    std::vector<unsigned char> prof_mask;
    std::vector<hipEvent_t> ev_pool;
    size_t ev_used = 0;
    int prof_forwards = 0;

    int new_buf(int div, int C) {
        bufs.push_back({div, C});
        return (int)bufs.size() - 1;
    }
    int pix_stride(int buf) const { return buf >= 0 ? bufs[buf].C : om::HEAD_PIX_STRIDE; }

    void add(const std::string& name, int cin, int cout, int ks, int stride, bool bn, om::View in, int in_div,
             om::View out, const om::View* res = nullptr, int out_mode = 0, int up = 1, bool stem = false) {
        om::LayerDef L;
        std::memset(&L.info, 0, sizeof(L.info));
        std::snprintf(L.info.name, sizeof(L.info.name), "%s", name.c_str());
        L.info.cin = cin; L.info.cout = cout; L.info.cout_pad = om::round_up(cout, 32);
        L.info.ksize = ks; L.info.stride = stride; L.info.has_bn = bn ? 1 : 0; L.info.leaky = bn ? 1 : 0;
        L.info.w_off = (int64_t)weight_floats;
        weight_floats += (size_t)L.info.cout_pad * ks * ks * cin;
        weight_floats = om::align_up(weight_floats, 4);
        L.info.scale_off = (int64_t)weight_floats; weight_floats += L.info.cout_pad;
        L.info.shift_off = (int64_t)weight_floats; weight_floats += L.info.cout_pad;
        L.info.wino_off = -1;
        L.info.wino_alt_off = -1;
        L.info.wino_planes = 0;
        if (ks == 3 && stride == 1 && !stem && L.info.cout_pad % 64 == 0 && cin % 32 == 0) {
            L.info.wino_planes = 24;
            weight_floats = om::align_up(weight_floats, 4);
            L.info.wino_off = (int64_t)weight_floats;
            weight_floats += (size_t)L.info.wino_planes * L.info.cout_pad * cin;
            weight_floats = om::align_up(weight_floats, 4);
            L.info.wino_alt_off = (int64_t)weight_floats;
            weight_floats += (size_t)16 * L.info.cout_pad * cin;
        }
        const bool wino = L.info.wino_planes != 0;
        L.info.wsplit_off = L.info.wsplit_scale_off = -1;
        if (!stem) {
            L.info.wsplit_off = (int64_t)split_words;
            split_words += (size_t)(wino ? 18 : ks * ks) * L.info.cout_pad * cin;
            L.info.wsplit_scale_off = (int64_t)split_words;
            split_words = om::align_up(split_words + L.info.cout_pad, 4);
        }
        L.info.wsplit_direct_off = L.info.wsplit_direct_scale_off = -1;
        if (wino) {
            L.info.wsplit_direct_off = (int64_t)split_words;
            split_words += (size_t)ks * ks * L.info.cout_pad * cin;
            L.info.wsplit_direct_scale_off = (int64_t)split_words;
            split_words = om::align_up(split_words + L.info.cout_pad, 4);
        }
        L.info.w16_off = -1;
        if (!stem) {
            L.info.w16_off = (int64_t)weight_halfs;
            weight_halfs = om::align_up(weight_halfs + om::conv_f16_weight_halfs(L.info.cout_pad, ks, cin), 8);
        }
        L.in = in; L.out = out; L.in_div = in_div; L.out_mode = out_mode; L.up = up; L.stem = stem;
        if (res) { L.res = *res; L.has_res = true; }
        layers.push_back(L);
    }

    om::View cbl(const std::string& name, om::View in, int cin, int cout, int ks, int div) {
        om::View o{new_buf(div, cout), 0};
        add(name, cin, cout, ks, 1, true, in, div, o);
        return o;
    }

// ... 109 lines not shown
                    ok = false;
            if (!ok) continue;
            for (auto& sg : segs)
                if (sg.producer >= 0) layers[sg.producer].side = new_buf(layers[sg.producer].in_div, layers[sg.producer].info.cout);
            C.gather = segs;
        }
    }
    bool upsample_on_read = true;
    bool keep_all = false;
    long long latency_cells = 0;
    int latency_ksplit = 8;
    struct PostAttach {
        bool on = false;
        om_post_cfg cfg;
        float* out_bbox = nullptr; int64_t* out_cls = nullptr; uint8_t* out_mask = nullptr;
        int32_t* out_count = nullptr; int32_t* out_keep = nullptr;
        void* ws = nullptr; size_t ws_bytes = 0;
    } post;
    struct Side { hipStream_t main = nullptr, side = nullptr; hipEvent_t ev_fork = nullptr, ev_join = nullptr; unsigned long long used = 0; };
    std::vector<Side> sides;
    Side capture_side;
    unsigned long long side_clock = 0;
    std::mutex side_mutex;
    int head_last = -2;
    void find_head_last() {
        head_last = -1;
        for (int l = 0; l < (int)layers.size(); ++l)
            if (std::strncmp(layers[l].info.name, "bbox_head", 9) == 0) head_last = l;
    }

    int take_side(hipStream_t main_stream, bool f16, PostAttach* post_q, Side* sd) {
        std::lock_guard<std::mutex> lock(side_mutex);
        *post_q = post;
        if (!post.on || f16 || head_last < 0) return OM_OK;
        hipStreamCaptureStatus cs = hipStreamCaptureStatusNone;
        if (hipStreamIsCapturing(main_stream, &cs) == hipSuccess && cs == hipStreamCaptureStatusActive) {
            OM_REQUIRE(capture_side.side, OM_ESTATE, "om_forward: stream capture with an attached postprocess, but no capture stream (re-attach)");
            *sd = capture_side;
            sd->main = main_stream;
            return OM_OK;
        }
        for (Side& have : sides)
            if (have.main == main_stream) { have.used = ++side_clock; *sd = have; }
        if (sd->side) return OM_OK;
        if (sides.size() >= 64) {
            size_t lru = 0;
            for (size_t i = 1; i < sides.size(); ++i)
                if (sides[i].used < sides[lru].used) lru = i;
            sides[lru].main = main_stream;
            sides[lru].used = ++side_clock;
            *sd = sides[lru];
            return OM_OK;
        }
        sd->main = main_stream;
        sd->used = ++side_clock;
        OM_CHECK_HIP(hipStreamCreateWithFlags(&sd->side, hipStreamNonBlocking));
        OM_CHECK_HIP(hipEventCreateWithFlags(&sd->ev_fork, hipEventDisableTiming));
        OM_CHECK_HIP(hipEventCreateWithFlags(&sd->ev_join, hipEventDisableTiming));
        sides.push_back(*sd);
        return OM_OK;
    }

    static int view_align_bytes(const om::View& v, bool f16) { return om::align_bytes((uintptr_t)v.ch_off * (f16 ? 2 : 4)); }

    int first_layers_fusable(bool f16, int B, int H, int W) const {
        if (layers.size() < 2 || !layers[0].stem || (f16 && !switch_on(SW_STEM2_F16))) return 0;
        const om::LayerDef& a = layers[0];
        const om::LayerDef& b = layers[1];
        if (!(a.info.cout == 32 && b.info.cin == 32 && b.info.ksize == 3 && b.info.stride == 2 && !b.has_res && b.out_mode == 0 &&
              b.in.buf == a.out.buf && b.in.ch_off == a.out.ch_off && b.out.buf >= 0))
            return 0;
        const int b_stride = pix_stride(b.out.buf), b_align = view_align_bytes(b.out, f16);
        if (f16) return b.info.w16_off >= 0 && om::stem2_f16_supported(B, H, W, b.info.cout, b_stride, b_align) ? 1 : 0;
        if (b.info.wsplit_off < 0 || b.info.wino_planes != 0 || !om::stem2_split_supported(B, H, W, b.info.cout, b_stride, b_align)) return 0;
        if (!switch_on(SW_STEM3) || layers.size() < 3) return 1;
        const om::LayerDef& c = layers[2];
        return c.info.cin == 64 && c.info.ksize == 1 && c.info.stride == 1 && !c.has_res && c.out_mode == 0 && c.in.buf == b.out.buf &&
                       c.in.ch_off == b.out.ch_off && c.info.wsplit_off >= 0 && c.out.buf >= 0 && c.gather.empty() && c.side < 0 &&
                       om::stem2_split_supported(B, H, W, b.info.cout, b_stride, b_align, c.info.cout, pix_stride(c.out.buf),
                                                 view_align_bytes(c.out, false))
                   ? 2 : 1;
    }

    template <class Args>
    void layer_shape(Args& a, const om::LayerDef& L, const om::LayerPlan& p, int B, int H, int W) const {
        const om_layer_info& li = L.info;
        om::fill_conv_shape(a, B, H / L.in_div, W / L.in_div, li.cin, pix_stride(L.in.buf), li.cout, li.cout_pad, li.ksize, li.stride,
                            li.leaky, L.has_res ? pix_stride(L.res.buf) : 0, pix_stride(p.to_side ? L.side : L.out.buf),
                            p.to_side ? 0 : L.out_mode, p.to_side ? 1 : L.up);
    }

    om::LayerPlan plan(int index, int B, int H, int W, bool f16) const {
        using om::Form;
        const om::LayerDef& L = layers[index];
        const om_layer_info& li = L.info;
        om::LayerPlan p;
        p.w_off = li.w_off; p.scale_off = li.scale_off;
        const bool split = !f16 && precision == 1;
        const int fused = (f16 || split) && !keep_all ? first_layers_fusable(f16, B, H, W) : 0;
        if (L.stem) {
            if (index == 0 && fused) { p.form = f16 ? Form::Stem2F16 : fused == 2 ? Form::Stem3Split : Form::Stem2Split; p.bm = 128; p.bn = 64; }
            return p;
        }
        if (index >= 1 && index <= fused) { p.form = Form::InPrevious; return p; }
        const int Hin = H / L.in_div, Win = W / L.in_div, Ho = Hin / li.stride, Wo = Win / li.stride;
        const long long cells = (long long)B * (H / 32) * (W / 32);
        const bool on_read = (f16 || split) && !keep_all && upsample_on_read;
        if (f16) {
            p.blob = om::LayerPlan::F16; p.w_off = li.w16_off;
            p.to_side = on_read && L.side >= 0; p.gather = on_read && !L.gather.empty();
            om::ConvArgsH a{};
            layer_shape(a, L, p, B, H, W);
            if (!p.gather && om::conv3x3_f16_supported(a)) {
                om::conv3x3_tile_for_f16(B * Ho * Wo, li.cout_pad, Wo, li.cin / 32, &p.bm, &p.bn);
                p.form = p.bm == 512 ? Form::Conv3x3F16Tall : Form::Conv3x3F16;
            } else {
                om::conv_tile_for_f16(B * Ho * Wo, li.cout_pad, li.cin, &p.bm, &p.bn, p.gather);
                p.form = p.gather ? Form::IgemmF16Gather : Form::IgemmF16;
            }
            return p;
        }
        const bool latency = split && !keep_all && latency_cells > 0 && cells < latency_cells;
        p.ksplit_max = latency ? latency_ksplit : 0;
        const bool wino = li.wino_planes != 0 && om::wino_enabled();
        if (wino && split) {
            om::Wino14Class cls[om::W14_MAXCLS];
            int pitch = 0;
            long long gtot = 0, m_tiles = 0;
            om::wino14_blocks(B, Hin, Win, cls, &pitch, &gtot, &m_tiles);
            const long long tiles = m_tiles * (li.cout_pad / 64);
            p.blob = om::LayerPlan::SPLIT;
            if (latency && tiles <= 128) {
                p.form = Form::SplitDirect3x3;
                p.w_off = li.wsplit_direct_off; p.scale_off = li.wsplit_direct_scale_off;
                om::conv_tile_for_split(B * Hin * Win, li.cout_pad, &p.bm, &p.bn);
                return p;
            }
            p.form = Form::Wino14; p.bm = 128; p.bn = 64;
            p.w_off = li.wsplit_off; p.scale_off = li.wsplit_scale_off;
            int R = 0, Ct = 0, ncb = 0, nrb = 0;
            om::wino14_geometry(B, Hin, Win, &R, &Ct, &ncb, &nrb);
            if (switch_on(SW_W14_WIDE) && li.cin >= 512 && (long long)nrb * ncb * (li.cout_pad / 64) > 256 && L.in.buf >= 0 && L.out.buf >= 0 && (!L.has_res || L.res.buf >= 0)) {
                om::ConvArgs a{};
                layer_shape(a, L, p, B, H, W);
                if (om::wino14_wide_supported(a, view_align_bytes(L.in, false), view_align_bytes(L.out, false), L.has_res,
                                              L.has_res ? view_align_bytes(L.res, false) : 0)) {
                    p.form = Form::Wino14Wide; p.bn = 128;
                    p.scratch_floats = om::wino14_wide_scratch_floats(B, Hin, Win, li.cin);
                }
            }
        } else if (wino && cells >= 1700ll) {
            p.form = Form::Wino24; p.bm = 64; p.bn = 64;
            p.w_off = li.wino_off;
            p.scratch_floats = om::wino24_scratch_floats(B, Hin, Win, li.cin);
        } else if (wino) {
            const bool fused_transform = om::wino_fused_for(li.cin);
            p.form = fused_transform ? Form::WinoFused : Form::Wino;
            p.bm = 64;
            p.bn = fused_transform ? (li.cout_pad % 128 == 0 ? 128 : 64) : om::wino_bn((long long)B * ((Hin + 1) / 2) * ((Win + 1) / 2), li.cout_pad);
            p.w_off = li.wino_alt_off;
            p.scratch_floats = om::wino_scratch_floats(B, Hin, Win, li.cin);
        } else if (split && li.wino_planes == 0) {
            p.blob = om::LayerPlan::SPLIT;
            p.w_off = li.wsplit_off; p.scale_off = li.wsplit_scale_off;
            p.to_side = on_read && L.side >= 0; p.gather = on_read && !L.gather.empty();
            p.form = p.gather ? Form::SplitGather : Form::Split;
            om::conv_tile_for_split(B * Ho * Wo, li.cout_pad, &p.bm, &p.bn, p.gather);
        } else {
            p.form = Form::Igemm;
            om::conv_tile_for(B * Ho * Wo, li.cout_pad, &p.bm, &p.bn);
        }
        return p;
    }

    size_t buf_floats(int i, int B, int H, int W) const {
        return (size_t)B * (H / bufs[i].div) * (W / bufs[i].div) * bufs[i].C;
    }

    struct Layout {
        std::vector<om::LayerPlan> plans;
        std::vector<size_t> buf_off;
        std::vector<size_t> scratch_off;
        size_t tickets_off = 0, partial_off = 0, total = 0;
    };

    Layout layout(int B, int H, int W, bool f16) const {
        const size_t esz = f16 ? 2 : 4;
        const int nb = (int)bufs.size(), nl = (int)layers.size();
        Layout out;
        out.plans.resize(nl);
        struct Item { size_t bytes; int first, last; size_t off; };
        std::vector<Item> items(nb + nl);
        for (int i = 0; i < nb; ++i) items[i] = {om::align_up(buf_floats(i, B, H, W) * esz, 256), nl, -1, 0};
        for (int l = 0; l < nl; ++l) {
            const om::LayerDef& L = layers[l];
            const om::LayerPlan& p = out.plans[l] = plan(l, B, H, W, f16);
            auto touch = [&](int buf) {
                if (buf < 0) return;
                if (l < items[buf].first) items[buf].first = l;
                if (l > items[buf].last) items[buf].last = l;
            };
            touch(L.in.buf); touch(L.out.buf);
            if (L.has_res) touch(L.res.buf);
            if (p.to_side) touch(L.side);
            if (p.gather)
                for (const auto& sg : L.gather)
                    if (sg.producer >= 0) touch(layers[sg.producer].side);
            items[nb + l] = {om::align_up(p.scratch_floats * sizeof(float), 256), l, l, 0};
        }
        if (keep_all)
            for (int i = 0; i < nb; ++i) { items[i].first = 0; items[i].last = nl; }
        std::vector<int> order;
        for (int i = 0; i < nb + nl; ++i)
            if (items[i].bytes && items[i].last >= items[i].first) order.push_back(i);
        std::stable_sort(order.begin(), order.end(), [&](int a, int b) { return items[a].first < items[b].first; });
        std::vector<int> placed;
        size_t peak = 0;
        for (int id : order) {
            Item& it = items[id];
            std::vector<std::pair<size_t, size_t>> busy;
            for (int o : placed)
                if (items[o].last >= it.first && items[o].first <= it.last) busy.push_back({items[o].off, items[o].off + items[o].bytes});
            std::sort(busy.begin(), busy.end());
            size_t at = 0;
            for (auto& b : busy) {
                if (at + it.bytes <= b.first) break;
                if (b.second > at) at = b.second;
            }
            it.off = at;
            if (at + it.bytes > peak) peak = at + it.bytes;
            placed.push_back(id);
        }
        out.buf_off.resize(nb);
        out.scratch_off.resize(nl);
        for (int i = 0; i < nb; ++i) out.buf_off[i] = items[i].off;
        for (int l = 0; l < nl; ++l) out.scratch_off[l] = items[nb + l].off;
        out.tickets_off = peak;
        out.partial_off = peak + om::align_up(((size_t)nl * om::SYNC_WORDS + om::STATUS_WORDS) * sizeof(int), 256);
        out.total = out.partial_off + (f16 ? 0 : om::SK_PARTIAL_BYTES);
        return out;
    }
};

namespace {

int fail_in(int rc, const char* what, const char* name) {
    char msg[512];
    std::snprintf(msg, sizeof(msg), "%s", om::g_err);
    om::set_error("%s %s: %s", what, name, msg);
    return rc;
}

struct LayerEvents {
    hipEvent_t ev_mid = nullptr, ev_stop = nullptr;
    hipStream_t stream = nullptr;
    int begin(om_model* m, int layer, hipStream_t s) {
        stream = s;
        if (!m->profiling || !(m->prof_mask.empty() || m->prof_mask[layer])) return OM_OK;
        while (m->ev_used + 3 > m->ev_pool.size()) {
            hipEvent_t e;
            OM_CHECK_HIP(hipEventCreate(&e));
            m->ev_pool.push_back(e);
        }
        OM_CHECK_HIP(hipEventRecord(m->ev_pool[m->ev_used], s));
        ev_mid = m->ev_pool[m->ev_used + 1];
        ev_stop = m->ev_pool[m->ev_used + 2];
        m->ev_used += 3;
        return OM_OK;
    }
    int mid() const {
        if (ev_mid) OM_CHECK_HIP(hipEventRecord(ev_mid, stream));
        return OM_OK;
    }
    ~LayerEvents() { if (ev_stop) (void)hipEventRecord(ev_stop, stream); }
};

struct JoinGuard {
    om_model::Side sd; bool forked;
    void join() {
        if (!forked) return;
        forked = false;
        (void)hipEventRecord(sd.ev_join, sd.side);
        (void)hipStreamWaitEvent(sd.main, sd.ev_join, 0);
    }
    ~JoinGuard() { join(); }
};

struct ForwardRun {
    const om_model* m;
    const float* x;
    int B, H, W;
    bool f16;
    float *bbox32, *bbox16, *bbox8, *oriens;
    char* workspace;
    const om_model::Layout* lay;
    hipStream_t stream;
    int* tickets;
    float* sk_partial;
    int* status;

    char* buf(int i) const { return workspace + lay->buf_off[i]; }
    void* ptr_of(const om::View& v) const {
        switch (v.buf) {
            case om::BUF_BBOX32: return bbox32;
            case om::BUF_BBOX16: return bbox16;
            case om::BUF_BBOX8: return bbox8;
            case om::BUF_ORIENS: return oriens;
            default: return buf(v.buf) + (size_t)v.ch_off * (f16 ? 2 : 4);
        }
    }
    const void* weights_of(const om::LayerPlan& p) const {
        if (p.blob == om::LayerPlan::F16) return m->weights16 + p.w_off;
        return (p.blob == om::LayerPlan::SPLIT ? m->weights_split : m->weights) + p.w_off;
    }
    const float* scale_of(const om::LayerPlan& p) const { return (p.blob == om::LayerPlan::SPLIT ? m->weights_split : m->weights) + p.scale_off; }

    template <class Args>
    Args conv_args(int index, const om::LayerPlan& p) const {
        const om::LayerDef& L = m->layers[index];
        Args a{};
        m->layer_shape(a, L, p, B, H, W);
        a.in = static_cast<decltype(a.in)>(ptr_of(L.in));
        a.w = static_cast<decltype(a.w)>(weights_of(p));
        a.scale = scale_of(p);
        a.shift = m->weights + L.info.shift_off;
        a.res = L.has_res ? static_cast<decltype(a.res)>(ptr_of(L.res)) : nullptr;
        a.out = static_cast<decltype(a.out)>(p.to_side ? static_cast<void*>(buf(L.side)) : ptr_of(L.out));
        a.ticket = tickets + (size_t)index * om::SYNC_WORDS;
        if (p.gather) {
            a.nseg = (int)L.gather.size();
            for (int g = 0; g < a.nseg; ++g) {
                const om::LayerDef::Seg& sg = L.gather[g];
                const int side = sg.producer >= 0 ? m->layers[sg.producer].side : -1;
                a.seg_ptr[g] = static_cast<decltype(a.in)>(side >= 0 ? static_cast<void*>(buf(side)) : ptr_of(sg.view));
                a.seg_pix_stride[g] = m->pix_stride(side >= 0 ? side : sg.view.buf);
                a.seg_channels[g] = sg.channels; a.seg_up[g] = sg.up;
            }
        }
        return a;
    }

    int launch_layer(int index, const om::LayerPlan& p, const LayerEvents& ev) const {
        using om::Form;
        const om::LayerDef& L = m->layers[index];
        if (p.form == Form::InPrevious) return ev.mid();
        if (p.form == Form::Stem2Split || p.form == Form::Stem3Split || p.form == Form::Stem2F16) return launch_first_layers(p, ev);
        if (p.form == Form::Stem) {
            if (int rc = ev.mid()) return rc;
            const float* shift = m->weights + L.info.shift_off;
            return f16 ? om::launch_conv_stem_f16(x, B, H / L.in_div, W / L.in_div, m->weights + p.w_off, scale_of(p), shift, L.info.cout, ptr_of(L.out), stream)
                       : om::launch_conv_stem(x, B, H / L.in_div, W / L.in_div, m->weights + p.w_off, scale_of(p), shift, L.info.cout,
                                              static_cast<float*>(ptr_of(L.out)), stream);
        }
        if (f16) {
            om::ConvArgsH a = conv_args<om::ConvArgsH>(index, p);
            a.out_f32 = L.out.buf < 0 ? 1 : 0;
            if (int rc = ev.mid()) return rc;
            return om::launch_conv_igemm_f16(a, stream);
        }
        om::ConvArgs a = conv_args<om::ConvArgs>(index, p);
        a.sk_partial = sk_partial;
        a.status = status;
        a.ksplit_max = p.ksplit_max;
        a.split = p.form == Form::Wino14 || p.form == Form::Wino14Wide ? 1 : 0;
        float* scratch = reinterpret_cast<float*>(workspace + lay->scratch_off[index]);
        switch (p.form) {
            case Form::Wino: case Form::WinoFused: a.mid_event = ev.ev_mid; return om::launch_conv_winograd(a, scratch, stream);
            case Form::Wino24: a.mid_event = ev.ev_mid; return om::launch_conv_winograd24(a, scratch, stream);
            case Form::Wino14Wide: a.mid_event = ev.ev_mid; return om::launch_conv_wino14_wide(a, scratch, stream);
            default: break;
        }
        if (int rc = ev.mid()) return rc;
        switch (p.form) {
            case Form::Wino14: return om::launch_conv_wino14_split(a, stream);
            case Form::Split: case Form::SplitGather: case Form::SplitDirect3x3: return om::launch_conv_igemm_split(a, stream);
            case Form::Igemm: return om::launch_conv_igemm(a, stream);
            default: break;
        }
        om::set_error("no launch for kernel form %d", (int)p.form);
        return OM_ESTATE;
    }

    int launch_first_layers(const om::LayerPlan& p, const LayerEvents& ev) const {
        const om::LayerDef& S = m->layers[0];
        const om::LayerDef& N = m->layers[1];
        const float *w = m->weights + p.w_off, *scale = scale_of(p), *shift = m->weights + S.info.shift_off;
        const float* n_shift = m->weights + N.info.shift_off;
        const int n_stride = m->pix_stride(N.out.buf);
        if (int rc = ev.mid()) return rc;
        if (p.form == om::Form::Stem2F16)
            return om::launch_conv_stem2_f16(x, B, H, W, w, scale, shift, m->weights16 + N.info.w16_off, m->weights + N.info.scale_off, n_shift,
                                             N.info.cout, N.info.leaky, ptr_of(N.out), n_stride, stream);
        om::Stem2Third third{};
        if (p.form == om::Form::Stem3Split) {
            const om::LayerDef& T = m->layers[2];
            third = {m->weights_split + T.info.wsplit_off, m->weights_split + T.info.wsplit_scale_off, m->weights + T.info.shift_off,
                     static_cast<float*>(ptr_of(T.out)), T.info.cout, T.info.leaky, m->pix_stride(T.out.buf)};
        }
        return om::launch_conv_stem2_split(x, B, H, W, w, scale, shift, m->weights_split + N.info.wsplit_off,
                                           m->weights_split + N.info.wsplit_scale_off, n_shift, N.info.cout, N.info.leaky,
                                           static_cast<float*>(ptr_of(N.out)), n_stride, status, stream,
                                           p.form == om::Form::Stem3Split ? &third : nullptr);
    }
};

int unit_ticket(hipStream_t stream, int** out) {
    static int* g_ticket = nullptr;
    if (!g_ticket) OM_CHECK_HIP(hipMalloc(reinterpret_cast<void**>(&g_ticket), om::SYNC_WORDS * sizeof(int)));
    if (int rc = om::launch_zero_words(g_ticket, om::SYNC_WORDS, stream)) return rc;
    *out = g_ticket;
    return OM_OK;
}

}

extern "C" {

int om_version(void) { return OM_VERSION; }
const char* om_last_error(void) { return om::g_err; }

int om_model_create(om_model** out, int num_anchors, int num_classes) {
    return om_model_create_variant(out, 0, num_anchors, num_classes);
}

int om_model_create_variant(om_model** out, int variant, int num_anchors, int num_classes) {
    OM_REQUIRE(out, OM_EINVAL, "om_model_create: out is null");
    OM_REQUIRE(variant == 0 || variant == 1, OM_EINVAL, "om_model_create_variant: variant %d (0 = FPNPlus, 1 = OrienMaskYOLO)", variant);
    OM_REQUIRE(num_anchors >= 1 && num_anchors <= 3 && num_classes >= 1 &&
                   num_anchors * (5 + num_classes) <= om::HEAD_PIX_STRIDE,
               OM_EINVAL, "om_model_create: unsupported head (anchors=%d classes=%d)", num_anchors, num_classes);
    om_model* m = new om_model();
    m->num_anchors = num_anchors;
    m->num_classes = num_classes;
    m->variant = variant;
    m->build();
    *out = m;
    return OM_OK;
}

void om_model_destroy(om_model* m) {
    if (!m) return;
    for (hipEvent_t e : m->ev_pool) (void)hipEventDestroy(e);
    if (m->capture_side.side) m->sides.push_back(m->capture_side);
    for (om_model::Side& sd : m->sides) {
        (void)hipEventDestroy(sd.ev_fork);
        (void)hipEventDestroy(sd.ev_join);
        (void)hipStreamDestroy(sd.side);
    }
// ... 372 lines not shown
}

size_t om_conv2d_winograd24_scratch_bytes(int B, int H, int W, int cin) {
    if (B <= 0 || H <= 0 || W <= 0 || cin <= 0) return 0;
    return om::align_up(om::wino24_scratch_floats(B, H, W, cin) * sizeof(float), 256) + om::SK_PARTIAL_BYTES;
}

static int conv2d_winograd24_impl(const float* in, int B, int H, int W, int cin, int in_pix_stride, const float* u,
                                  const float* scale, const float* shift, int cout, int leaky, const float* res,
                                  int res_pix_stride, float* out, int out_pix_stride, void* scratch, size_t scratch_bytes,
                                  om_stream stream, int split, int32_t* status_dev) {
    OM_REQUIRE(B > 0 && H > 0 && W > 0, OM_EINVAL, "om_conv2d_winograd24: bad shape");
    OM_REQUIRE(scratch && scratch_bytes >= om_conv2d_winograd24_scratch_bytes(B, H, W, cin), OM_ENOMEM,
               "om_conv2d_winograd24: scratch too small");
    om::ConvArgs a;
    a.in = in; a.w = u; a.scale = scale; a.shift = shift; a.res = res; a.out = out;
    om::fill_conv_shape(a, B, H, W, cin, in_pix_stride, cout, om::round_up(cout, 64), 3, 1, leaky, res_pix_stride, out_pix_stride);
    a.split = split; a.status = status_dev;
    if (int rc = unit_ticket(static_cast<hipStream_t>(stream), &a.ticket)) return rc;
    a.sk_partial = reinterpret_cast<float*>(static_cast<char*>(scratch) + om::align_up(om::wino24_scratch_floats(B, H, W, cin) * sizeof(float), 256));
    return om::launch_conv_winograd24(a, static_cast<float*>(scratch), static_cast<hipStream_t>(stream));
}

int om_conv2d_winograd24(const float* in, int B, int H, int W, int cin, int in_pix_stride, const float* u,
                         const float* scale, const float* shift, int cout, int leaky, const float* res,
                         int res_pix_stride, float* out, int out_pix_stride, void* scratch, size_t scratch_bytes,
                         om_stream stream) {
    return conv2d_winograd24_impl(in, B, H, W, cin, in_pix_stride, u, scale, shift, cout, leaky, res, res_pix_stride, out,
                                  out_pix_stride, scratch, scratch_bytes, stream, 0, nullptr);
}

int om_conv2d_winograd24_split(const float* in, int B, int H, int W, int cin, int in_pix_stride, const void* u_split,
                               const float* scale_split, const float* shift, int cout, int leaky, const float* res,
                               int res_pix_stride, float* out, int out_pix_stride, void* scratch, size_t scratch_bytes,
                               int32_t* status_dev, om_stream stream) {
    return conv2d_winograd24_impl(in, B, H, W, cin, in_pix_stride, static_cast<const float*>(u_split), scale_split, shift, cout,
                                  leaky, res, res_pix_stride, out, out_pix_stride, scratch, scratch_bytes, stream, 1, status_dev);
}

int om_conv2d_wino14_split(const float* in, int B, int H, int W, int cin, int in_pix_stride, const void* u14_split,
                           const float* scale_split, const float* shift, int cout, int leaky, const float* res,
                           int res_pix_stride, float* out, int out_pix_stride, int32_t* status_dev, om_stream stream) {
    OM_REQUIRE(B > 0 && H > 0 && W > 0, OM_EINVAL, "om_conv2d_wino14_split: bad shape");
    om::ConvArgs a;
    a.in = in; a.w = static_cast<const float*>(u14_split); a.scale = scale_split; a.shift = shift; a.res = res; a.out = out;
    om::fill_conv_shape(a, B, H, W, cin, in_pix_stride, cout, om::round_up(cout, 64), 3, 1, leaky, res_pix_stride, out_pix_stride);
    a.split = 1; a.status = status_dev;
    if (int rc = unit_ticket(static_cast<hipStream_t>(stream), &a.ticket)) return rc;
    return om::launch_conv_wino14_split(a, static_cast<hipStream_t>(stream));
}

int om_conv2d_wino14_blocks(int B, int H, int W, int* classes, int* row_pitch, long long* m_tiles) {
    OM_REQUIRE(B > 0 && H > 0 && W > 0 && classes && row_pitch && m_tiles, OM_EINVAL, "om_conv2d_wino14_blocks: bad argument");
    om::Wino14Class cls[om::W14_MAXCLS];
    long long gtot = 0;
    const int n = om::wino14_blocks(B, H, W, cls, row_pitch, &gtot, m_tiles);
    for (int k = 0; k < n; ++k) {
        const int v[5] = {cls[k].t0, cls[k].Ct, cls[k].ncb, cls[k].R, cls[k].nrb};
        for (int i = 0; i < 5; ++i) classes[5 * k + i] = v[i];
    }
    return n;
}

size_t om_conv2d_wino14_wide_scratch_bytes(int B, int H, int W, int cin) {
    if (B <= 0 || H <= 0 || W <= 0 || cin <= 0 || cin % 16) return 0;
    return om::align_up(om::wino14_wide_scratch_floats(B, H, W, cin) * sizeof(float), 256);
}

int om_conv2d_wino14_wide(const float* in, int B, int H, int W, int cin, int in_pix_stride, const void* u14_split,
                          const float* scale_split, const float* shift, int cout, int leaky, const float* res,
                          int res_pix_stride, float* out, int out_pix_stride, void* scratch, size_t scratch_bytes,
                          int32_t* status_dev, om_stream stream) {
    OM_REQUIRE(B > 0 && H > 0 && W > 0, OM_EINVAL, "om_conv2d_wino14_wide: bad shape");
    OM_REQUIRE(scratch && scratch_bytes >= om_conv2d_wino14_wide_scratch_bytes(B, H, W, cin), OM_ENOMEM,
               "om_conv2d_wino14_wide: scratch too small");
    om::ConvArgs a;
    a.in = in; a.w = static_cast<const float*>(u14_split); a.scale = scale_split; a.shift = shift; a.res = res; a.out = out;
    om::fill_conv_shape(a, B, H, W, cin, in_pix_stride, cout, om::round_up(cout, 64), 3, 1, leaky, res_pix_stride, out_pix_stride);
    a.split = 1; a.status = status_dev;
    if (int rc = unit_ticket(static_cast<hipStream_t>(stream), &a.ticket)) return rc;
    return om::launch_conv_wino14_wide(a, static_cast<float*>(scratch), static_cast<hipStream_t>(stream));
}

int om_set_wino14_wide(int on) {
    OM_REQUIRE(on == 0 || on == 1, OM_EINVAL, "om_set_wino14_wide: %d", on);
    switch_flag(SW_W14_WIDE).store(on, std::memory_order_relaxed);
    return OM_OK;
}
int om_get_wino14_wide(void) { return switch_on(SW_W14_WIDE) ? 1 : 0; }

int om_conv2d_stem3_split(const float* in, int B, int H, int W, const float* w1, const float* scale1, const float* shift1,
                          const void* w2_split, const float* scale2_split, const float* shift2, int cout2, int leaky2, float* out,
                          int out_pix_stride, const void* w3_split, const float* scale3_split, const float* shift3, int cout3, int leaky3,
                          float* out3, int out3_pix_stride, int32_t* status_dev, om_stream stream) {
    om::Stem2Third third{w3_split, scale3_split, shift3, out3, cout3, leaky3, out3_pix_stride};
    return om::launch_conv_stem2_split(in, B, H, W, w1, scale1, shift1, w2_split, scale2_split, shift2, cout2, leaky2, out,
                                       out_pix_stride, status_dev, static_cast<hipStream_t>(stream), &third);
}

int om_conv2d_stem2_f16(const float* in, int B, int H, int W, const float* w1, const float* scale1, const float* shift1,
                        const void* w2_f16, const float* scale2, const float* shift2, int cout2, int leaky2, void* out, int out_pix_stride,
                        om_stream stream) {
    return om::launch_conv_stem2_f16(in, B, H, W, w1, scale1, shift1, w2_f16, scale2, shift2, cout2, leaky2, out, out_pix_stride,
                                     static_cast<hipStream_t>(stream));
}

int om_set_stem_fusion(int which, int on) {
    OM_REQUIRE((which == 0 || which == 1) && (on == 0 || on == 1), OM_EINVAL, "om_set_stem_fusion: which=%d on=%d", which, on);
    switch_flag(which).store(on, std::memory_order_relaxed);
    return OM_OK;
}

int om_get_stem_fusion(int which) {
    if (which != 0 && which != 1) return -1;
    return switch_on(which) ? 1 : 0;
}

int om_get_conv3x3_f16_variant(void) { return om::conv3x3_f16_get_tall(); }

int om_set_conv3x3_f16_variant(int mode) {
    OM_REQUIRE(mode >= 0 && mode <= 2, OM_EINVAL, "om_set_conv3x3_f16_variant: %d", mode);
    om::conv3x3_f16_set_tall(mode);
    return OM_OK;
}

int om_conv2d_stem(const float* in, int B, int H, int W, const float* w, const float* scale, const float* shift,
                   int cout, float* out, om_stream stream) {
    return om::launch_conv_stem(in, B, H, W, w, scale, shift, cout, out, static_cast<hipStream_t>(stream));
}

int om_conv2d_stem2_split(const float* in, int B, int H, int W, const float* w1, const float* scale1, const float* shift1,
                          const void* w2_split, const float* scale2_split, const float* shift2, int cout2, int leaky2, float* out,
                          int out_pix_stride, int32_t* status_dev, om_stream stream) {
    return om::launch_conv_stem2_split(in, B, H, W, w1, scale1, shift1, w2_split, scale2_split, shift2, cout2, leaky2, out,
                                       out_pix_stride, status_dev, static_cast<hipStream_t>(stream));
}

}
```

### orienmask_amd/csrc/wino14_shared.h

```cpp
#pragma once
#include <cstdlib>
#include <type_traits>

#include "conv_f16_common.h"

namespace om {

typedef _Float16 f16x4 __attribute__((ext_vector_type(4)));
typedef _Float16 f16x2 __attribute__((ext_vector_type(2)));
typedef float f32x2 __attribute__((ext_vector_type(2)));
typedef unsigned u32x2 __attribute__((ext_vector_type(2)));
typedef unsigned u32x4v __attribute__((__vector_size__(4 * sizeof(unsigned))));

constexpr int W14_BM = 128, W14_BN = 64;

struct Wino14Params {
    const float* in;
    const _Float16* u;
    const float* scale;
    const float* shift;
    const float* res;
    float* out;
    int* ticket;
    int* status;
    int B, H, W, in_ps, in_bytes;
    int cout, out_ps, res_ps, leaky, fast_io, out_bytes, res_bytes;
    int R, Ct, ncb, gtot, hp;
    Wino14Class cls[W14_MAXCLS];
    int n_tiles, total_tiles, nch;
    int u_bytes;
};

__host__ __device__ constexpr int w14_plane(int g) { return g == 0 ? 0 : g == 1 ? 5 : g - 1; }

struct Wino14Tile {
    int g0, t0, n0, tile_n;
    int R, Ct;
};

__device__ __forceinline__ void wino14_decode(const Wino14Params& p, int tile, Wino14Tile& t) {
    static_assert(W14_MAXCLS == 2, "one comparison picks the class");
    t.tile_n = tile % p.n_tiles;
    const int tm = tile / p.n_tiles;
    const bool k = tm >= p.cls[1].m0;
    const int ncb = k ? p.cls[1].ncb : p.cls[0].ncb;
    const int tl = tm - (k ? p.cls[1].m0 : 0);
    const int rb = tl / ncb, cb = tl - rb * ncb;
    t.R = k ? p.cls[1].R : p.cls[0].R;
    t.Ct = k ? p.cls[1].Ct : p.cls[0].Ct;
    t.g0 = rb * t.R; t.t0 = (k ? p.cls[1].t0 : p.cls[0].t0) + cb * t.Ct; t.n0 = t.tile_n * W14_BN;
}

template <int MODE> constexpr int W14_EPI_OPS = MODE == 0 ? 16 : MODE == 1 ? 28 : 0;
template <int MODE, typename F>
__device__ __forceinline__ void wino14_epilogue(const Wino14Params& p, const f32x16 (&acc)[6], const Wino14Tile& tl, f32x4* sT, int wm,
                                                int wn, int lane, F before_requests) {
    asm volatile("" : "+v"(lane));
    const int fi = lane & 31, fk = lane >> 5;
    const int hp = p.hp;
    const int c8 = lane & 7;
    const int nb = tl.n0 + 32 * wn + 4 * c8;
    const int nvalid = p.cout - nb;
    const f32x4 sc = *reinterpret_cast<const f32x4*>(p.scale + nb);
    const f32x4 sh = *reinterpret_cast<const f32x4*>(p.shift + nb);
    int pix0[4], oxe[4];
#pragma unroll
    for (int rd = 0; rd < 4; ++rd) {
        const int ml = 32 * wm + 8 * rd + (lane >> 3);
        const int r = ml / tl.Ct, t = ml - r * tl.Ct;
        const int gg = tl.g0 + r;
        const int b = gg / hp;
        const int y = gg - b * hp - 1;
        const bool rowok = r < tl.R && gg < p.gtot && y >= 0 && y < p.H && nvalid > 0;
        oxe[rd] = rowok ? 4 * (tl.t0 + t) : p.W;
        pix0[rd] = (b * p.H + y) * p.W + 4 * (tl.t0 + t);
    }
    float nonfinite = 0.f;
    auto position = [&](int px, int gq, int k) {
        const int i = 4 * gq + k;
        if (px == 0) return acc[0][i] + acc[1][i] + acc[2][i] + acc[3][i] + acc[4][i];
        if (px == 1) return (acc[1][i] - acc[2][i]) + 2.f * (acc[3][i] - acc[4][i]);
        if (px == 2) return (acc[1][i] + acc[2][i]) + 4.f * (acc[3][i] + acc[4][i]);
        return (acc[1][i] - acc[2][i]) + 8.f * (acc[3][i] - acc[4][i]) + acc[5][i];
    };
    auto transpose_in = [&](int px) {
#pragma unroll
        for (int gq = 0; gq < 4; ++gq) {
            const f32x4 v = {position(px, gq, 0), position(px, gq, 1), position(px, gq, 2), position(px, gq, 3)};
            sT[fi * 8 + ((2 * gq + fk) ^ (fi & 7))] = v;
        }
    };
    auto transpose_out = [&](int rd) {
        const int e = 8 * rd + (lane >> 3);
        return sT[e * 8 + (c8 ^ (e & 7))];
    };
    auto activate = [&](f32x4 v, bool ok) {
        float nf = 0.f;
#pragma unroll
        for (int k = 0; k < 4; ++k) {
            const float tv = fmaf(v[k], sc[k], sh[k]);
            nf = fmaf(tv, 0.f, nf);
            v[k] = p.leaky ? fmaxf(tv, tv * 0.1f) : tv;
        }
        nonfinite += ok ? nf : 0.f;
        return v;
    };
    if constexpr (MODE < 2) {
        const auto rs_out = __builtin_amdgcn_make_buffer_rsrc(p.out, 0, p.out_bytes, 0x00020000);
        const auto rs_res = __builtin_amdgcn_make_buffer_rsrc(const_cast<float*>(p.res), 0, MODE == 1 ? p.res_bytes : 0, 0x00020000);
        auto offset = [&](int rd, int px, int ps) { return oxe[rd] + px < p.W ? ((pix0[rd] + px) * ps + nb) * 4 : (int)0x80000000; };
        f32x4 rc[4];
        if constexpr (MODE == 1) {
#pragma unroll
            for (int rd = 0; rd < 4; ++rd) rc[rd] = __builtin_bit_cast(f32x4, __builtin_amdgcn_raw_buffer_load_b128(rs_res, offset(rd, 0, p.res_ps), 0, 0));
        }
        before_requests();
        auto one_position = [&](auto pxc, auto nextc) {
            constexpr int px = decltype(pxc)::value, nx = decltype(nextc)::value;
            transpose_in(px);
            f32x4 v[4];
#pragma unroll
            for (int rd = 0; rd < 4; ++rd) {
                v[rd] = activate(transpose_out(rd), oxe[rd] + px < p.W);
                if constexpr (MODE == 1) v[rd] += rc[rd];
            }
            if constexpr (MODE == 1 && nx >= 0) {
#pragma unroll
                for (int rd = 0; rd < 4; ++rd)
                    rc[rd] = __builtin_bit_cast(f32x4, __builtin_amdgcn_raw_buffer_load_b128(rs_res, offset(rd, nx, p.res_ps), 0, 0));
            }
#pragma unroll
            for (int rd = 0; rd < 4; ++rd)
                __builtin_amdgcn_raw_buffer_store_b128(__builtin_bit_cast(u32x4v, v[rd]), rs_out, offset(rd, px, p.out_ps), 0, 0);
// ... 33 lines not shown
```

### orienmask_amd/lib.py

```python
import ctypes
import os

_HERE = os.path.dirname(os.path.abspath(__file__))
LIB_PATH = os.path.join(_HERE, "lib", "liborienmask_hip.so")

OM_MAX_SCALES = 3
OM_MAX_ANCHORS = 9
OM_STATUS_SPLIT_RANGE = 1
OM_STATUS_SK_TIMEOUT = 2


class LayerInfo(ctypes.Structure):
    _fields_ = [("name", ctypes.c_char * 64),
                ("cin", ctypes.c_int32), ("cout", ctypes.c_int32), ("cout_pad", ctypes.c_int32),
                ("ksize", ctypes.c_int32), ("stride", ctypes.c_int32),
                ("has_bn", ctypes.c_int32), ("leaky", ctypes.c_int32), ("wino_planes", ctypes.c_int32),
                ("w_off", ctypes.c_int64), ("scale_off", ctypes.c_int64), ("shift_off", ctypes.c_int64),
                ("wino_off", ctypes.c_int64), ("wino_alt_off", ctypes.c_int64), ("w16_off", ctypes.c_int64),
                ("wsplit_off", ctypes.c_int64), ("wsplit_scale_off", ctypes.c_int64),
                ("wsplit_direct_off", ctypes.c_int64), ("wsplit_direct_scale_off", ctypes.c_int64)]


class PostCfg(ctypes.Structure):
    _fields_ = [("num_scales", ctypes.c_int32),
# ... 12 lines not shown


class RleImage(ctypes.Structure):
    _fields_ = [("mask", ctypes.c_void_p), ("K", ctypes.c_int32), ("H", ctypes.c_int32), ("W", ctypes.c_int32),
                ("crop_top", ctypes.c_int32), ("crop_down", ctypes.c_int32), ("crop_left", ctypes.c_int32),
                ("crop_right", ctypes.c_int32), ("hflip", ctypes.c_int32), ("vflip", ctypes.c_int32),
                ("orig_h", ctypes.c_int32), ("orig_w", ctypes.c_int32)]


class VisImage(ctypes.Structure):
    _fields_ = [("image", ctypes.c_void_p), ("out", ctypes.c_void_p), ("out_float", ctypes.c_void_p), ("mask", ctypes.c_void_p),
                ("keep", ctypes.c_void_p), ("colors", ctypes.c_void_p), ("boxes", ctypes.c_void_p),
                ("n_keep", ctypes.c_int32), ("Hn", ctypes.c_int32), ("Wn", ctypes.c_int32),
                ("crop_left", ctypes.c_int32), ("crop_right", ctypes.c_int32), ("crop_top", ctypes.c_int32),
                ("crop_down", ctypes.c_int32), ("h", ctypes.c_int32), ("w", ctypes.c_int32),
                ("with_mask", ctypes.c_int32), ("draw_boxes", ctypes.c_int32), ("alpha", ctypes.c_float)]


OM_LOSS_MAX_CLASSES = 2047
OM_LOSS_MAX_GT = 1024
OM_LOSS_TERMS = 7
OM_LOSS_METRICS = 8
OM_LOSS_SCALE_FLOATS = OM_LOSS_TERMS + 2 * OM_LOSS_METRICS
OM_LOSS_FLAG_OFF = OM_MAX_SCALES * OM_LOSS_SCALE_FLOATS
OM_LOSS_RESULT_FLOATS = OM_LOSS_FLAG_OFF + 1
OM_LOSS_FLAG_NONFINITE_WH = 1
OM_LOSS_FLAG_TOO_MANY_GT = 2
OM_LOSS_FLAG_BAD_CLASS = 4


class LossCfg(ctypes.Structure):
    _fields_ = [("num_scales", ctypes.c_int32),
                ("grid_h", ctypes.c_int32 * OM_MAX_SCALES), ("grid_w", ctypes.c_int32 * OM_MAX_SCALES),
                ("image_h", ctypes.c_int32), ("image_w", ctypes.c_int32),
                ("anchors_of_scale", ctypes.c_int32 * OM_MAX_SCALES),
                ("anchor_mask", (ctypes.c_int32 * 3) * OM_MAX_SCALES),
                ("num_anchors_total", ctypes.c_int32),
                ("anchor_w", ctypes.c_float * OM_MAX_ANCHORS), ("anchor_h", ctypes.c_float * OM_MAX_ANCHORS),
                ("num_classes", ctypes.c_int32),
                ("center_region", ctypes.c_float), ("valid_region", ctypes.c_float),
                ("label_smooth", ctypes.c_float), ("label_on", ctypes.c_float),
                ("obj_ignore_threshold", ctypes.c_float),
                ("weight", (ctypes.c_float * OM_LOSS_TERMS) * OM_MAX_SCALES),
                ("bbox_stride", (ctypes.c_int64 * 4) * OM_MAX_SCALES),
                ("orien_stride", (ctypes.c_int64 * 3) * OM_MAX_SCALES)]


OM_VIS_MAX_KEPT = 512
OM_VIS_BATCH = 16

_vp, _i, _f, _sz = ctypes.c_void_p, ctypes.c_int, ctypes.c_float, ctypes.c_size_t

SIGNATURES = {
    "om_version": (_i, []),
    "om_last_error": (ctypes.c_char_p, []),
    "om_model_create": (_i, [ctypes.POINTER(_vp), _i, _i]),
    "om_model_create_variant": (_i, [ctypes.POINTER(_vp), _i, _i, _i]),
    "om_model_destroy": (None, [_vp]),
    "om_model_num_layers": (_i, [_vp]),
    "om_model_layer_info": (_i, [_vp, _i, ctypes.POINTER(LayerInfo)]),
    "om_model_weight_floats": (_sz, [_vp]),
    "om_model_load_weights": (_i, [_vp, _vp, _sz, _i]),
    "om_model_weight_split_words": (_sz, [_vp]),
    "om_model_load_weights_split": (_i, [_vp, _vp, _sz]),
    "om_model_set_precision": (_i, [_vp, _i]),
    "om_model_get_precision": (_i, [_vp]),
    "om_model_set_latency_cells": (_i, [_vp, ctypes.c_longlong]),
    "om_model_set_latency_ksplit": (_i, [_vp, _i]),
    "om_model_attach_postprocess": (_i, [_vp, ctypes.POINTER(PostCfg), _vp, _vp, _vp, _vp, _vp, _vp, ctypes.c_size_t]),
    "om_model_set_upsample_on_read": (_i, [_vp, _i]),
    "om_conv2d_split": (_i, [_vp, _i, _i, _i, _i, _i, _vp, _vp, _vp, _i, _i, _i, _i, _vp, _i, _vp, _i, _i, _i, _i, _i, _vp, _vp]),
    "om_conv2d_split_k": (_i, [_vp, _i, _i, _i, _i, _i, _vp, _vp, _vp, _i, _i, _i, _i, _vp, _i, _vp, _i, _i, _i, _i, _i, _i, _vp, _vp]),
    "om_conv2d_winograd24_split": (_i, [_vp, _i, _i, _i, _i, _i, _vp, _vp, _vp, _i, _i, _vp, _i, _vp, _i, _vp, _sz, _vp, _vp]),
    "om_set_stem_fusion": (_i, [_i, _i]),
    "om_get_stem_fusion": (_i, [_i]),
    "om_get_conv3x3_f16_variant": (_i, []),
    "om_set_conv3x3_f16_variant": (_i, [_i]),
    "om_conv2d_wino14_split": (_i, [_vp, _i, _i, _i, _i, _i, _vp, _vp, _vp, _i, _i, _vp, _i, _vp, _i, _vp, _vp]),
    "om_conv2d_wino14_blocks": (_i, [_i, _i, _i, ctypes.POINTER(_i), ctypes.POINTER(_i), ctypes.POINTER(ctypes.c_longlong)]),
    "om_conv2d_wino14_wide_scratch_bytes": (_sz, [_i, _i, _i, _i]),
    "om_conv2d_wino14_wide": (_i, [_vp, _i, _i, _i, _i, _i, _vp, _vp, _vp, _i, _i, _vp, _i, _vp, _i, _vp, _sz, _vp, _vp]),
    "om_set_wino14_wide": (_i, [_i]),
    "om_get_wino14_wide": (_i, []),
    "om_forward_workspace_bytes": (_sz, [_vp, _i, _i, _i]),
    "om_forward_status_offset": (_sz, [_vp, _i, _i, _i]),
    "om_forward": (_i, [_vp, _vp, _i, _i, _i, _vp, _vp, _vp, _vp, _vp, _sz, _vp]),
    "om_layer_tile": (_i, [_vp, _i, _i, _i, _i, ctypes.POINTER(ctypes.c_int), ctypes.POINTER(ctypes.c_int),
                           ctypes.POINTER(ctypes.c_int)]),
    "om_model_weight_halfs": (_sz, [_vp]),
    "om_model_load_weights_f16": (_i, [_vp, _vp, _sz]),
    "om_forward_f16_workspace_bytes": (_sz, [_vp, _i, _i, _i]),
    "om_forward_f16": (_i, [_vp, _vp, _i, _i, _i, _vp, _vp, _vp, _vp, _vp, _sz, _vp]),
    "om_layer_tile_f16": (_i, [_vp, _i, _i, _i, _i, ctypes.POINTER(ctypes.c_int), ctypes.POINTER(ctypes.c_int),
                               ctypes.POINTER(ctypes.c_int)]),
    "om_conv2d_f16": (_i, [_vp, _i, _i, _i, _i, _i, _vp, _vp, _vp, _i, _i, _i, _i, _vp, _i, _vp, _i, _i, _vp]),
    "om_conv2d_stem_f16": (_i, [_vp, _i, _i, _i, _vp, _vp, _vp, _i, _vp, _vp]),
    "om_conv2d_winograd_scratch_bytes": (_sz, [_i, _i, _i, _i]),
    "om_conv2d_winograd": (_i, [_vp, _i, _i, _i, _i, _i, _vp, _vp, _vp, _i, _i, _vp, _i, _vp, _i, _vp, _sz, _vp]),
    "om_layer_output_view": (_i, [_vp, _i, _i, _i, _i, _i, ctypes.POINTER(ctypes.c_size_t), ctypes.POINTER(ctypes.c_int),
                                  ctypes.POINTER(ctypes.c_int), ctypes.POINTER(ctypes.c_int)]),
    "om_model_keep_activations": (_i, [_vp, _i]),
    "om_conv2d_winograd24_scratch_bytes": (_sz, [_i, _i, _i, _i]),
    "om_conv2d_winograd24": (_i, [_vp, _i, _i, _i, _i, _i, _vp, _vp, _vp, _i, _i, _vp, _i, _vp, _i, _vp, _sz, _vp]),
    "om_profile_enable": (_i, [_vp, _i]),
    "om_profile_enable_layers": (_i, [_vp, ctypes.c_char_p, _i]),
    "om_profile_read": (_i, [_vp, ctypes.POINTER(ctypes.c_float), ctypes.POINTER(ctypes.c_float), _i,
                             ctypes.POINTER(ctypes.c_int)]),
    "om_conv2d": (_i, [_vp, _i, _i, _i, _i, _i, _vp, _vp, _vp, _i, _i, _i, _i, _vp, _i, _vp, _i, _vp]),
    "om_conv2d_mode": (_i, [_vp, _i, _i, _i, _i, _i, _vp, _vp, _vp, _i, _i, _i, _i, _vp, _i, _vp, _i, _i, _i, _vp]),
    "om_conv2d_stem": (_i, [_vp, _i, _i, _i, _vp, _vp, _vp, _i, _vp, _vp]),
    "om_conv2d_stem2_split": (_i, [_vp, _i, _i, _i, _vp, _vp, _vp, _vp, _vp, _vp, _i, _i, _vp, _i, _vp, _vp]),
    "om_conv2d_stem3_split": (_i, [_vp, _i, _i, _i, _vp, _vp, _vp, _vp, _vp, _vp, _i, _i, _vp, _i, _vp, _vp, _vp, _i, _i, _vp, _i, _vp, _vp]),
    "om_conv2d_stem2_f16": (_i, [_vp, _i, _i, _i, _vp, _vp, _vp, _vp, _vp, _vp, _i, _i, _vp, _i, _vp]),
    "om_conv2d_split_gather": (_i, [_i, ctypes.POINTER(_vp), ctypes.POINTER(_i), ctypes.POINTER(_i), ctypes.POINTER(_i), _i, _i, _i,
                                    _vp, _vp, _vp, _i, _i, _vp, _i, _vp, _vp]),
    "om_preprocess": (_i, [_vp, _i, _i, _i, _i, _i, ctypes.POINTER(ctypes.c_float), ctypes.POINTER(ctypes.c_float),
                           _i, _i, _i, _i, _f, _vp, _vp]),
    "om_pad_nchw": (_i, [_vp, ctypes.c_longlong, _i, _i, _i, _i, _i, _i, _f, _vp, _vp]),
    "om_postprocess_workspace_bytes": (_sz, [ctypes.POINTER(PostCfg), _i]),
    "om_postprocess": (_i, [ctypes.POINTER(PostCfg), _vp, _vp, _vp, _vp, _i, _vp, _vp, _vp, _vp, _vp, _vp, _sz, _vp]),
    "om_postprocess_detect": (_i, [ctypes.POINTER(PostCfg), _vp, _vp, _vp, _i, _vp, _vp, _vp, _vp, _vp, _sz, _vp]),
    "om_postprocess_assemble": (_i, [ctypes.POINTER(PostCfg), _vp, _i, _vp, _vp, _vp, _sz, _vp]),
    "om_postprocess_candidates": (_i, [ctypes.POINTER(PostCfg), _vp, _vp, _vp, _i, _vp, _vp, _vp, _vp, _vp, _sz, _vp]),
    "om_postprocess_masks": (_i, [ctypes.POINTER(PostCfg), _vp, _i, _vp, _vp, _vp, _vp, _vp, _sz, _vp]),
    "om_recover_bbox": (_i, [_vp, _i, _i, ctypes.POINTER(ctypes.c_int32), ctypes.POINTER(ctypes.c_int32), _i, _i, _i, _i,
                             _vp, _vp]),
    "om_recover_masks_rle": (_i, [_vp, _i, _i, _i, _i, _i, _i, _i, _i, _i, _i, _i, _vp, _i, _vp, _vp, _vp]),
    "om_recover_masks_rle_strings": (_i, [_vp, _i, _vp, _i, _vp, _vp, ctypes.c_longlong, _vp, _vp, _vp, _vp]),
    "om_visualize_workspace_bytes": (_sz, [_vp, _i]),
    "om_visualize": (_i, [_vp, _i, _vp, _sz, _vp]),
    "om_cocoeval_workspace_bytes": (_sz, [ctypes.c_longlong, _i]),
    "om_cocoeval_masks": (_i, [_i, _vp, _vp, _vp, _vp, _i, _i, _vp, _vp, _vp, _vp, _vp, _vp, _vp, _vp, ctypes.c_longlong, _vp, _sz, _vp]),
    "om_cocoeval_mask_stats": (_i, [_i, ctypes.c_longlong, _vp, _vp, _vp]),
    "om_cocoeval_mask_iou": (_i, [_i, _vp, _vp, _i, _vp, _vp, ctypes.c_longlong, _vp, _vp, _vp]),
    "om_cocoeval_bbox_iou": (_i, [_i, _vp, _vp, _vp, _vp, _vp, _vp]),
    "om_cocoeval_match": (_i, [_i, _vp, _vp, _vp, _vp, _vp, _vp, _vp, _vp, _vp, _vp, _i, _i, _vp, _vp, _vp, _vp]),
    "om_post_kernel_occupancy": (_i, [_i, ctypes.POINTER(_i), ctypes.POINTER(_i), ctypes.POINTER(_i), ctypes.POINTER(_i)]),
    "om_nms_workspace_bytes": (_sz, [_i]),
    "om_nms": (_i, [_vp, _i, _f, _vp, _vp, _vp, _sz, _vp]),
    "om_nms_ex": (_i, [_vp, _i, _f, _i, _vp, _vp, _vp, _sz, _vp]),
    "om_ref_math": (_i, [_vp, ctypes.c_longlong, _i, _i, _vp, _vp]),
    "om_loss_workspace_bytes": (_sz, [ctypes.POINTER(LossCfg), _i, _i]),
    "om_loss": (_i, [ctypes.POINTER(LossCfg), ctypes.POINTER(_vp), ctypes.POINTER(_vp), _i, _vp, _vp, _vp, _vp, _i, _vp, _vp, _sz, _vp]),
    "om_loss_targets": (_i, [ctypes.POINTER(LossCfg), ctypes.POINTER(_vp), _i, _vp, _vp, _vp, _vp, _i, _i, _vp, _vp, _vp, _vp, _vp, _vp,
                             _vp, _vp, _vp, _vp, _sz, _vp]),
    "om_augment_workspace_bytes": (_sz, [_i]),
    "om_augment": (_i, [_vp, _i, _vp, _i, ctypes.POINTER(_f), ctypes.POINTER(_f), _i, _i, _vp, _vp, _vp, _i, _vp, _i, _vp, _sz, _vp]),
    "om_loss_backward": (_i, [ctypes.POINTER(LossCfg), ctypes.POINTER(_vp), ctypes.POINTER(_vp), _i, _vp, _vp, _i, _vp, _vp, _sz, _vp,
                              ctypes.POINTER(_f), ctypes.POINTER(_vp), ctypes.POINTER(_vp), _vp]),
    "om_sgd_step": (_i, [_vp, _vp, _i, _vp, _i, _vp]),
    "om_bn_act_workspace_bytes": (_sz, [_i, _i, _i, _i]),
    "om_bn_act_forward": (_i, [_vp, _i, _i, _i, _i, _vp, _vp, _vp, _vp, _vp, _i, ctypes.c_double, ctypes.c_double, _f, _vp, _vp, _vp, _vp,
                               _vp, _sz, _vp]),
    "om_bn_act_backward": (_i, [_vp, _vp, _i, _i, _i, _i, _vp, _vp, _vp, _vp, _i, _f, _vp, _vp, _vp, _vp, _sz, _vp]),
    "om_bn_sync_stats": (_i, [_vp, _i, _i, _i, _i, _vp, _vp, _sz, _vp]),
    "om_bn_sync_forward": (_i, [_vp, _i, _i, _i, _i, _vp, _i, _vp, _vp, _vp, _vp, _vp, ctypes.c_double, ctypes.c_double, _f, _vp, _vp,
                                _vp, _vp, _vp, _vp]),
    "om_bn_sync_backward_sums": (_i, [_vp, _vp, _i, _i, _i, _i, _vp, _vp, _vp, _vp, _f, _vp, _vp, _vp, _vp, _sz, _vp]),
    "om_bn_sync_backward_dx": (_i, [_vp, _vp, _i, _i, _i, _i, _vp, _vp, _vp, _vp, _f, _vp, _i, _vp, _vp, _vp]),
    "om_conv2d_grad_workspace_bytes": (_sz, [_i, _i, _i, _i, _i, _i, _i]),
    "om_conv2d_grad_input": (_i, [_vp, _vp, _i, _i, _i, _i, _i, _i, _i, _vp, _vp, _sz, _vp]),
    "om_conv2d_grad_weight": (_i, [_vp, _vp, _i, _i, _i, _i, _i, _i, _i, _vp, _vp, _vp, _sz, _vp]),
    "om_conv2d_forward": (_i, [_vp, _vp, _vp, _i, _i, _i, _i, _i, _i, _i, _vp, _vp]),
    "om_route_concat_forward": (_i, [ctypes.POINTER(_vp), ctypes.POINTER(_i), ctypes.POINTER(_i), _i, _i, _i, _i, _vp, _vp]),
    "om_route_concat_backward": (_i, [_vp, ctypes.POINTER(_i), ctypes.POINTER(_i), _i, _i, _i, _i, ctypes.POINTER(_vp), _vp]),
}
# ... 48 lines not shown
```

### orienmask_amd/model.py

```python
import contextlib
import ctypes
import math

import torch
import torch.nn as nn

from . import lib as _lib
from . import pack as _pack
from .arch import model_convs, state_dict_entries

HEAD_PIX_STRIDE = 256
PRECISIONS = ("f32", "f32_split", "f16")
DEFAULT_PRECISION = "f32_split"


class Prediction(tuple):

    def __new__(cls, items, status=None, precision=None, rerun=None):
        self = super().__new__(cls, items)
        self.status = status
        self.precision = precision
        self.rerun = rerun
        return self

# ... 170 lines not shown
            _lib.check(_lib.load().om_model_load_weights_split(h, ctypes.c_void_p(blob.data_ptr()), blob.numel() * 4),
                       "om_model_load_weights_split")
        self._packed_split = blob

    LATENCY_CELLS = 3500

    def set_latency_mode(self, enable=True, cells=None, ksplit=None):
        self.latency_cells = int(cells if cells is not None else self.LATENCY_CELLS) if enable else 0
        _lib.check(_lib.load().om_model_set_latency_cells(self._ensure_handle(), self.latency_cells), "om_model_set_latency_cells")
        if ksplit is not None:
            _lib.check(_lib.load().om_model_set_latency_ksplit(self._ensure_handle(), int(ksplit)), "om_model_set_latency_ksplit")
        return self

    def set_upsample_on_read(self, enable=True):
        _lib.check(_lib.load().om_model_set_upsample_on_read(self._ensure_handle(), 1 if enable else 0), "om_model_set_upsample_on_read")
        self._workspace.clear()
        self._slot_workspaces.clear()
        return self

    def set_streams(self, n):
        if int(n) < 1:
            raise ValueError("n_streams must be >= 1")
        self.n_streams = int(n)
        return self

    @contextlib.contextmanager
    def workspace_slot(self, slot):
        if int(slot) < 0:
            raise ValueError("slot must be >= 0")
        prev, self._slot = self._slot, int(slot)
        try:
            yield self
        finally:
            self._slot = prev

    def packed_weights_f16(self, device):
        h = self._ensure_handle()
        if self._packed16 is None or self._packed16.device != device:
            total = _lib.load().om_model_weight_halfs(h)
            self.bind_packed_f16(_pack.pack_state_dict_f16(self.state_dict(), self._layers, total).to(device))
        return self._packed16

    def bind_packed_f16(self, blob):
        h = self._ensure_handle()
        _lib.require_cuda_tensor(blob, "packed fp16 weights", torch.float16)
        with torch.cuda.device(blob.device):
            _lib.check(_lib.load().om_model_load_weights_f16(h, ctypes.c_void_p(blob.data_ptr()), blob.numel() * 2),
                       "om_model_load_weights_f16")
        self._packed16 = blob

    def bind_packed(self, blob):
        h = self._ensure_handle()
        _lib.require_cuda_tensor(blob, "packed weights", torch.float32)
        L = _lib.load()
        with torch.cuda.device(blob.device):
            _lib.check(L.om_model_load_weights(h, ctypes.c_void_p(blob.data_ptr()), blob.numel() * 4, 0),
                       "om_model_load_weights")
        self._packed = blob
        self._packed_device = blob.device

    def forward(self, x):
        if self.training:
            raise RuntimeError("orienmask_amd.OrienMaskYOLOFPNPlus is inference-only: call .eval() first")
        _lib.require_cuda_tensor(x, "x", torch.float32)
        if x.dim() != 4 or x.shape[1] != 3 or x.shape[2] % 32 or x.shape[3] % 32:
            raise ValueError("x must be [B,3,H,W] with H and W multiples of 32, got %s" % (tuple(x.shape),))
        return self._forward(x.contiguous(), self.precision, self._slot)

    def _forward(self, x, precision, slot):
        B, _, H, W = x.shape
        dev = x.device
        L = _lib.load()
        self.packed_weights(dev)
        f16 = precision == "f16"
        if f16:
            self.packed_weights_f16(dev)
        h = self._handle
        split = precision == "f32_split"
        if split:
            self.packed_weights_split(dev)
        _lib.check(L.om_model_set_precision(h, 1 if split else 0), "om_model_set_precision")
        n_sub = self.n_streams if (self.n_streams > 1 and B % self.n_streams == 0) else 1
        Bs = B // n_sub
        switches = (L.om_get_wino14_wide(), L.om_get_stem_fusion(0), L.om_get_stem_fusion(1))
        key = (dev, Bs, H, W, f16, n_sub, switches, split)
        cache = self._workspace if slot == 0 else self._slot_workspaces.setdefault(slot, {})
        ws = cache.get(key)
        if ws is None:
            nbytes = (L.om_forward_f16_workspace_bytes if f16 else L.om_forward_workspace_bytes)(h, Bs, H, W)
            nbytes = (nbytes + 255) // 256 * 256
            for k in [k for k in cache if k[:7] != key[:7]]:
                del cache[k]
            ws = torch.empty(nbytes * n_sub, dtype=torch.uint8, device=dev)
            cache[key] = ws
        ws_each = ws.numel() // n_sub
        A = self.num_anchors
        bbox_dim = A * (5 + self.num_classes)
        heads = [torch.empty((B, H // s, W // s, HEAD_PIX_STRIDE), dtype=torch.float32, device=dev) for s in (32, 16, 8)]
        oriens = torch.empty((B, 6 * A, H // 4, W // 4), dtype=torch.float32, device=dev)
        fwd = L.om_forward_f16 if f16 else L.om_forward

        def launch(i, stream_ptr):
            xs, hs, os_ = x[i * Bs:], [t[i * Bs:] for t in heads], oriens[i * Bs:]
            return fwd(h, ctypes.c_void_p(xs.data_ptr()), Bs, H, W, ctypes.c_void_p(hs[0].data_ptr()),
                       ctypes.c_void_p(hs[1].data_ptr()), ctypes.c_void_p(hs[2].data_ptr()), ctypes.c_void_p(os_.data_ptr()),
                       ctypes.c_void_p(ws.data_ptr() + i * ws_each), ws_each, stream_ptr)

        with torch.cuda.device(dev):
            if n_sub == 1:
                _lib.check(launch(0, _lib.current_stream_ptr(dev)), "om_forward")
            else:
                cur = torch.cuda.current_stream(dev)
                side = self._side_streams.setdefault(dev, [])
                while len(side) < n_sub:
                    side.append(torch.cuda.Stream(device=dev))
                for i in range(n_sub):
                    side[i].wait_stream(cur)
                    _lib.check(launch(i, ctypes.c_void_p(side[i].cuda_stream)), "om_forward")
                for i in range(n_sub):
                    cur.wait_stream(side[i])
            status = None
            if not f16:
                off = L.om_forward_status_offset(h, Bs, H, W)
                status = ws.view(n_sub, ws_each)[:, off:off + 4].clone().view(torch.int32).reshape(n_sub)
        bboxes = [t[..., :bbox_dim].permute(0, 3, 1, 2) for t in heads]
        o32, o16, o8 = torch.split(oriens, A * 2, dim=1)
        rerun = (lambda: self._forward(x, "f32", slot)) if split else None
        return Prediction(((bboxes[0], o32), (bboxes[1], o16), (bboxes[2], o8)), status=status, precision=precision, rerun=rerun)

    def profile_enable(self, enable=True):
        _lib.check(_lib.load().om_profile_enable(self._ensure_handle(), 1 if enable else 0), "om_profile_enable")

    def keep_activations(self, keep=True):
        _lib.check(_lib.load().om_model_keep_activations(self._ensure_handle(), 1 if keep else 0), "om_model_keep_activations")
        self._workspace.clear()
        self._slot_workspaces.clear()
        return self

    def layer_output(self, name, x_shape):
        h = self._ensure_handle()
        idx = [l["name"] for l in self._layers].index(name)
        B, _, H, W = x_shape
        f16 = self.precision == "f16"
        ws = next(iter(self._workspace.values()))
        off, ch, ps, div = ctypes.c_size_t(0), ctypes.c_int(0), ctypes.c_int(0), ctypes.c_int(0)
        _lib.check(_lib.load().om_layer_output_view(h, idx, B, H, W, 1 if f16 else 0, ctypes.byref(off), ctypes.byref(ch),
                                                    ctypes.byref(ps), ctypes.byref(div)), "om_layer_output_view")
        dt = torch.float16 if f16 else torch.float32
        esz = 2 if f16 else 4
        hh, ww = H // div.value, W // div.value
        flat = ws[off.value:off.value + ((B * hh * ww - 1) * ps.value + ch.value) * esz].view(dt)
        return torch.as_strided(flat, (B, ch.value, hh, ww), (hh * ww * ps.value, 1, ww * ps.value, ps.value))

    def profile_enable_layers(self, names):
        h = self._ensure_handle()
        mask = bytes(1 if l["name"] in set(names) else 0 for l in self._layers)
        _lib.check(_lib.load().om_profile_enable_layers(h, mask, len(mask)), "om_profile_enable_layers")

    def layer_kernels(self, B, H, W):
        h = self._ensure_handle()
        out = []
        if self.precision == "f16":
            for i, l in enumerate(self._layers):
                bm, bn, algo = ctypes.c_int(0), ctypes.c_int(0), ctypes.c_int(0)
                _lib.check(_lib.load().om_layer_tile_f16(h, i, B, H, W, ctypes.byref(bm), ctypes.byref(bn),
                                                         ctypes.byref(algo)), "om_layer_tile_f16")
                fmt = {0: "conv_stem_kernel<f16>", 1: "conv_igemm_f16_kernel<%d,%d>", 4: "conv3x3_f16_kernel<%d,%d>",
                       5: "conv_igemm_f16_kernel<%d,%d,gather>", 6: "conv3x3_f16_tall_kernel<%d,%d>",
                       7: "conv_stem2_f16_kernel<%d,%d>", 8: "(in the previous layer's kernel)"}[algo.value]
                out.append((l["name"], fmt % (bm.value, bn.value) if algo.value not in (0, 8) else fmt))
            return out
        _lib.check(_lib.load().om_model_set_precision(h, 1 if self.precision == "f32_split" else 0), "om_model_set_precision")
        for i, l in enumerate(self._layers):
            bm, bn, algo = ctypes.c_int(0), ctypes.c_int(0), ctypes.c_int(0)
            _lib.check(_lib.load().om_layer_tile(h, i, B, H, W, ctypes.byref(bm), ctypes.byref(bn), ctypes.byref(algo)),
                       "om_layer_tile")
            fmt = {0: "conv_stem_kernel", 1: "conv_igemm_f32_kernel<%d,%d>", 2: "wino_gemm_kernel<%d,%d>",
                   3: "wino_fused_kernel<%d,%d>", 5: "wino24_gemm_kernel<%d,%d>",
                   7: "conv_igemm_split_kernel<%d,%d>", 8: "wino14_split_kernel<%d,%d>",
                   9: "conv_stem2_split_kernel<%d,%d>", 10: "(in the previous layer's kernel)",
                   11: "conv_igemm_split_kernel<%d,%d,gather>", 12: "wino14_wide_kernel<%d,%d>"}[algo.value]
            out.append((l["name"], fmt % ((bm.value, bn.value) if algo.value not in (0, 10) else ())))
        return out

    def profile_read(self):
        h = self._ensure_handle()
        n = len(self._layers)
        ms = (ctypes.c_float * n)()
        pre = (ctypes.c_float * n)()
        nf = ctypes.c_int(0)
        _lib.check(_lib.load().om_profile_read(h, ms, pre, n, ctypes.byref(nf)), "om_profile_read")
        return [(self._layers[i]["name"], float(ms[i]), float(pre[i])) for i in range(n)], nf.value

    def __del__(self):
        try:
            if getattr(self, "_handle", None) is not None:
                _lib.load().om_model_destroy(self._handle)
                self._handle = None
        except Exception:
            pass


class OrienMaskYOLO(OrienMaskYOLOFPNPlus):
    VARIANT = 1
```

Measured before the change: 2196.

## Fuse 1x1 conv epilogue with Winograd F(4,3) input transform for paired layers

When a 1x1 stride-1 split-precision conv feeds a wide Winograd 3x3 layer, the 1x1 kernel's epilogue now writes the transformed Winograd V tiles (hi/lo fp16) directly instead of an NHWC activation. The consumer then skips its separate V-transform kernel. M tiles are re-cut so each tile covers whole 4-wide Winograd entries plus halo pixels, so some border pixels are recomputed. This removes one activation write/read round trip and a kernel launch per pair, but the V buffer is larger than the activation and the tiles overlap.

```diff
diff --git a/include/orienmask_hip.h b/include/orienmask_hip.h
--- a/include/orienmask_hip.h
+++ b/include/orienmask_hip.h
@@ -146,6 +146,17 @@
                           int32_t* status_dev, om_stream stream);
 int om_set_wino14_wide(int on);
 int om_get_wino14_wide(void);
+int om_set_wino14_pair(int on);
+int om_get_wino14_pair(void);
+int om_layer_pair(const om_model* m, int index, int B, int H, int W);
+int om_conv2d_wino14_pair_tiles(int B, int H, int W, int* entries_per_tile, long long* m_tiles);
+int om_conv2d_wino14_pair_tile(int B, int H, int W, long long tile, int* entry_first, int* entry_end, int* pixel_first, int* pixel_last);
+int om_conv2d_split_v(int nseg, const float* const* seg_ptr, const int* seg_channels, const int* seg_pix_stride, const int* seg_up, int B,
+                      int H, int W, const void* w_split, const float* scale_split, const float* shift, int cout, int leaky, void* v,
+                      size_t v_bytes, int32_t* status_dev, om_stream stream);
+int om_conv2d_wino14_wide_v(const void* v, int B, int H, int W, int cin, const void* u14_split, const float* scale_split, const float* shift,
+                            int cout, int leaky, const float* res, int res_pix_stride, float* out, int out_pix_stride, int32_t* status_dev,
+                            om_stream stream);
 int om_set_stem_fusion(int which, int on);
 int om_get_stem_fusion(int which);
 int om_set_conv3x3_f16_variant(int mode);
diff --git a/orienmask_amd/csrc/conv_igemm_split.hip b/orienmask_amd/csrc/conv_igemm_split.hip
--- a/orienmask_amd/csrc/conv_igemm_split.hip
+++ b/orienmask_amd/csrc/conv_igemm_split.hip
@@ -1,6 +1,7 @@
 #include <cstdlib>
 
 #include "conv_f16_common.h"
+#include "wino14_shared.h"
 
 namespace om {
 
@@ -28,6 +29,7 @@
     int nseg, nimg;
     const _Float16* seg_ptr[4];
     int seg_stride_h[4], seg_shift[4], seg_end[4];
+    int v_tw, v_n, v_entries, v_gtot, v_bytes;
 };
 
 template <int BM, int BN>
@@ -171,6 +173,72 @@
     for (int k = 0; k < 4; ++k) { sc[k] = a0[k]; sc[4 + k] = a1[k]; sh[k] = b0[k]; sh[4 + k] = b1[k]; }
 }
 
+template <int BM, int BN, int WM, int WN>
+__device__ __forceinline__ void split_v_epilogue(const IgemmSParams& p, f32x4* smem, const f32x16 (&acc)[WM / 32][WN / 32],
+                                                 const Wino14PairTile& vt, int n0, int tid, int wm, int wn, int fi, int fk,
+                                                 const float (&sc)[8], const float (&sh)[8]) {
+    constexpr int TM = WM / 32, TN = WN / 32;
+    constexpr int CH8 = BN / 8, CH = BN / 4;
+    static_assert(BM == W14_PAIR_BM, "wino14_pair_tile's tiles");
+    f32x4* sC = smem;
+#pragma unroll
+    for (int a = 0; a < TM; ++a) {
+        const int ml = wm * WM + a * 32 + fi;
+#pragma unroll
+        for (int b = 0; b < TN; ++b)
+#pragma unroll
+            for (int g = 0; g < 4; ++g) {
+                const int n4 = (wn * WN + b * 32) / 4 + 2 * g + fk;
+                const f32x4 v = {acc[a][b][4 * g], acc[a][b][4 * g + 1], acc[a][b][4 * g + 2], acc[a][b][4 * g + 3]};
+                sC[ml * CH + (n4 ^ (ml & 7))] = v;
+            }
+    }
+    asm volatile("s_waitcnt lgkmcnt(0)" ::: "memory");
+    __builtin_amdgcn_s_barrier();
+    const int n8 = tid % CH8;
+    const int n = n0 + n8 * 8;
+    const int c = n >> 4, o = n8 & 1;
+    const auto rs_v = __builtin_amdgcn_make_buffer_rsrc(p.out, 0, p.v_bytes, 0x00020000);
+    float nonfinite = 0.f;
+#pragma unroll 1
+    for (int e = vt.e0 + tid / CH8; e < vt.e1; e += 256 / CH8) {
+        const int gr = e / p.v_tw, t = e - gr * p.v_tw;
+        const int G = gr + 2 * (gr / p.Ho) + 1;
+        const int row0 = gr * p.Wo - vt.p_lo;
+        f32x4 d[2][6];
+#pragma unroll
+        for (int x = 0; x < 6; ++x) {
+            const int px = 4 * t - 1 + x;
+            const bool ok = (unsigned)px < (unsigned)p.Wo;
+            const int ml = ok ? (row0 + px) & (BM - 1) : 0;
+            const f32x4 v0 = sC[ml * CH + ((2 * n8) ^ (ml & 7))];
+            const f32x4 v1 = sC[ml * CH + ((2 * n8 + 1) ^ (ml & 7))];
+#pragma unroll
+            for (int k = 0; k < 4; ++k) {
+                const float t0 = fmaf(v0[k], sc[k], sh[k]), t1 = fmaf(v1[k], sc[4 + k], sh[4 + k]);
+                nonfinite = fmaf(t0, 0.f, nonfinite);
+                nonfinite = fmaf(t1, 0.f, nonfinite);
+                const float a0 = p.leaky ? (t0 > 0.f ? t0 : t0 * 0.1f) : t0, a1 = p.leaky ? (t1 > 0.f ? t1 : t1 * 0.1f) : t1;
+                d[0][x][k] = ok ? a0 : 0.f;
+                d[1][x][k] = ok ? a1 : 0.f;
+            }
+            asm volatile("" : "+v"(d[0][x]), "+v"(d[1][x]));
+        }
+        const int ebase = (G * p.v_tw + t) * 64 + 16 * o;
+#pragma unroll
+        for (int j = 0; j < 6; ++j) {
+            f16x8 h, l;
+            w14_point_split8(d, j, h, l);
+            const int off = (c * 6 + j) * (p.v_gtot * p.v_tw * 64) + ebase;
+            __builtin_amdgcn_raw_buffer_store_b128(__builtin_bit_cast(u32x4v, h), rs_v, off, 0, 0);
+            __builtin_amdgcn_raw_buffer_store_b128(__builtin_bit_cast(u32x4v, l), rs_v, off + 32, 0, 0);
+        }
+    }
+    asm volatile("s_waitcnt lgkmcnt(0)" ::: "memory");
+    __builtin_amdgcn_s_barrier();
+    if (p.status && nonfinite != nonfinite) atomicOr(p.status, OM_STATUS_SPLIT_RANGE);
+}
+
 __device__ __forceinline__ void split8(const f32x4& x0, const f32x4& x1, f16x8& hi, f16x8& lo) {
 #pragma unroll
     for (int i = 0; i < 4; ++i) {
@@ -413,13 +481,14 @@
     }
 }
 
-template <int BM, int BN, int WM, int WN, bool GATHER = false, bool FAST = false, int NBUF = 2>
+template <int BM, int BN, int WM, int WN, bool GATHER = false, bool FAST = false, int NBUF = 2, bool VEPI = false>
 __global__ __launch_bounds__(256, 2) void conv_igemm_split_wide_kernel(const IgemmSParams p) {
     constexpr int TM = WM / 32, TN = WN / 32;
     constexpr int NWN = BN / WN;
     constexpr int A_CH = BM / 32, B_CH = BN / 32, NP = A_CH + B_CH;
     constexpr bool KSPLIT = NBUF > 2;
     static_assert(!(KSPLIT && GATHER), "the deep-ring form has no gathered input");
+    static_assert(!VEPI || (FAST && !KSPLIT && BM * BN / 4 <= NBUF * (BM + BN) * 8), "the V epilogue: the whole C tile in the operand ring");
     constexpr int STAGE = (BM + BN) * 8;
     static_assert((BM / WM) * (BN / WN) == 4, "four waves per workgroup");
     static_assert(BM % 32 == 0 && BN % 32 == 0, "whole 32-row pieces");
@@ -462,17 +531,19 @@
             tile_n = tile % p.n_tiles;
             tile_m = tile / p.n_tiles;
         }
-        const int m0 = tile_m * BM, n0 = tile_n * BN;
+        [[maybe_unused]] Wino14PairTile vt;
+        if constexpr (VEPI) wino14_pair_tile(p.Wo, p.v_tw, p.v_n, p.v_entries, tile_m, vt);
+        const int m0 = VEPI ? vt.p_lo : tile_m * BM, m_end = VEPI ? vt.p_hi + 1 : p.M, n0 = tile_n * BN;
 
         int rowoff[A_CH];
         unsigned invmask[A_CH];
         [[maybe_unused]] int g_img[A_CH], g_y[A_CH], g_x[A_CH];
-        const int b_first = (m0 < p.M ? m0 : p.M - 1) / p.HoWo;
+        const int b_first = (m0 < m_end ? m0 : m_end - 1) / p.HoWo;
 #pragma unroll
         for (int j = 0; j < A_CH; ++j) {
             int m = m0 + lrow + 32 * j;
-            const bool mok = m < p.M;
-            if (!mok) m = p.M - 1;
+            const bool mok = m < m_end;
+            if (!mok) m = m_end - 1;
             const int b = m / p.HoWo;
             const int rr = m - b * p.HoWo;
             const int oy = rr / p.Wo;
@@ -674,13 +745,14 @@
             }
         }
 
-        split_epilogue<BM, BN, WM, WN, FAST>(p, smem, acc, m0, n0, tid, wm, wn, fi, fk, sc, sh);
-    }
-}
-
-template <int BM, int BN, int WM, int WN, bool WIDE = false, bool GATHER = false, int NBUF = 3, int WSTAGES = 0>
+        if constexpr (VEPI) split_v_epilogue<BM, BN, WM, WN>(p, smem, acc, vt, n0, tid, wm, wn, fi, fk, sc, sh);
+        else split_epilogue<BM, BN, WM, WN, FAST>(p, smem, acc, m0, n0, tid, wm, wn, fi, fk, sc, sh);
+    }
+}
+
+template <int BM, int BN, int WM, int WN, bool WIDE = false, bool GATHER = false, int NBUF = 3, int WSTAGES = 0, bool VEPI = false>
 static int launch_tile_split(IgemmSParams p, int cout_pad, int blocks_per_cu, hipStream_t stream) {
-    const int m_tiles = (p.M + BM - 1) / BM;
+    const int m_tiles = VEPI ? (p.v_entries + p.v_n - 1) / p.v_n : (p.M + BM - 1) / BM;
     p.n_tiles = cout_pad / BN;
     const long long total = (long long)m_tiles * p.n_tiles;
     OM_REQUIRE(total > 0 && total < (1ll << 31), OM_EINVAL, "conv split: %lld tiles out of range", total);
@@ -706,7 +778,11 @@
         grid = tickets;
     }
     const bool fast = p.out_mode == 0 && !p.res && p.vec_io && p.cout == cout_pad;
-    if constexpr (WIDE) {
+    if constexpr (VEPI) {
+        static_assert(WIDE && !DEEP, "the V epilogue belongs to the whole-line kernel's queue form");
+        OM_REQUIRE(fast, OM_EINVAL, "conv split: the V epilogue needs a plain NHWC layer without residual, cout == cout_pad");
+        hipLaunchKernelGGL((conv_igemm_split_wide_kernel<BM, BN, WM, WN, GATHER, true, 2, true>), dim3((unsigned)grid), dim3(256), 0, stream, p);
+    } else if constexpr (WIDE) {
         constexpr int WNBUF = DEEP ? WSTAGES : 2;
         if (fast) hipLaunchKernelGGL((conv_igemm_split_wide_kernel<BM, BN, WM, WN, GATHER, true, WNBUF>), dim3((unsigned)grid), dim3(256), 0, stream, p);
         else hipLaunchKernelGGL((conv_igemm_split_wide_kernel<BM, BN, WM, WN, GATHER, false, WNBUF>), dim3((unsigned)grid), dim3(256), 0, stream, p);
@@ -734,6 +810,19 @@
         if (tiles > 128 || cout_pad % c.bn || c.bm * c.bn >= *bm * *bn) continue;
         *bm = c.bm; *bn = c.bn;
     }
+}
+
+bool conv_split_v_out_supported(const ConvArgs& a, int out_align_bytes) {
+    return a.ks == 1 && a.stride == 1 && a.out_mode == 0 && a.cout == a.cout_pad && a.cout_pad % 128 == 0 && a.cin % 32 == 0 && a.cin >= 32 &&
+           out_align_bytes >= 16 && (long long)a.B * a.H * a.W < (1ll << 31) && a.H >= 1 && a.W >= 1 &&
+           wino14_wide_scratch_floats(a.B, a.H, a.W, a.cout) * 4 < 0x7FFFFFF0ull;
+}
+int conv_split_v_out_entries(int W) { return wino14_pair_entries(W); }
+void conv_split_v_out_tile(int B, int H, int W, int k, int* e) {
+    Wino14PairTile t;
+    const int TW = (W + 3) / 4;
+    wino14_pair_tile(W, TW, wino14_pair_entries(W), B * H * TW, k, t);
+    e[0] = t.e0; e[1] = t.e1; e[2] = t.p_lo; e[3] = t.p_hi;
 }
 
 int launch_conv_igemm_split(const ConvArgs& a, hipStream_t stream) {
@@ -792,6 +881,16 @@
         p.nseg = a.nseg;
         p.in = p.seg_ptr[0];
     }
+    p.v_tw = p.v_n = p.v_entries = p.v_gtot = p.v_bytes = 0;
+    if (a.v_out) {
+        OM_REQUIRE(conv_split_v_out_supported(a, align_bytes(a.out)) && !a.res && !a.force_bm && !a.force_bn, OM_EINVAL,
+                   "conv split: the V epilogue needs a 1x1 stride-1 layer without residual, cin %% 32 == 0, cout = cout_pad a multiple of 128 "
+                   "(cin=%d cout=%d cout_pad=%d ks=%d stride=%d)", a.cin, a.cout, a.cout_pad, a.ks, a.stride);
+        p.v_tw = (a.W + 3) / 4; p.v_n = wino14_pair_entries(a.W); p.v_entries = a.B * a.H * p.v_tw; p.v_gtot = a.B * (a.H + 2);
+        p.v_bytes = (int)(wino14_wide_scratch_floats(a.B, a.H, a.W, a.cout) * 4);
+        if (a.nseg > 0) return launch_tile_split<128, 128, 64, 64, true, true, 3, 0, true>(p, a.cout_pad, 2, stream);
+        return launch_tile_split<128, 128, 64, 64, true, false, 3, 0, true>(p, a.cout_pad, 2, stream);
+    }
     int bm, bn;
     conv_tile_for_split(p.M, a.cout_pad, &bm, &bn, a.nseg > 0);
     OM_REQUIRE(a.nseg == 0 || (bm == 128 && bn == 128), OM_EINVAL, "conv split: no gathered-input kernel with a %d x %d tile", bm, bn);
diff --git a/orienmask_amd/csrc/conv_wino14.hip b/orienmask_amd/csrc/conv_wino14.hip
--- a/orienmask_amd/csrc/conv_wino14.hip
+++ b/orienmask_amd/csrc/conv_wino14.hip
@@ -343,18 +343,6 @@
     long long items;
 };
 
-__device__ __forceinline__ f32x4 w14_point(const f32x4 (&d)[6], int j) {
-    const f32x4 c4 = 4.f, cm4 = -4.f, c2 = 2.f, cm2 = -2.f, cm5 = -5.f;
-    switch (j) {
-        case 0: return __builtin_elementwise_fma(d[2], cm5, __builtin_elementwise_fma(d[0], c4, d[4]));
-        case 1: return __builtin_elementwise_fma(d[1] + d[2], cm4, d[3] + d[4]);
-        case 2: return __builtin_elementwise_fma(d[1] - d[2], c4, d[4] - d[3]);
-        case 3: return __builtin_elementwise_fma(d[3] - d[1], c2, d[4] - d[2]);
-        case 4: return __builtin_elementwise_fma(d[3] - d[1], cm2, d[4] - d[2]);
-        default: return __builtin_elementwise_fma(d[3], cm5, __builtin_elementwise_fma(d[1], c4, d[5]));
-    }
-}
-
 __global__ __launch_bounds__(256) void wino14_v_kernel(const Wino14VParams p) {
     const long long id = (long long)blockIdx.x * 256 + threadIdx.x;
     if (id >= p.items) return;
@@ -377,17 +365,7 @@
 #pragma unroll
     for (int j = 0; j < 6; ++j) {
         f16x8 h, l;
-#pragma unroll
-        for (int q = 0; q < 2; ++q) {
-            const f32x4 v = w14_point(d[q], j);
-            const f16x4 hh = __builtin_convertvector(v, f16x4);
-            f32x4 rem;
-#pragma unroll
-            for (int k = 0; k < 4; ++k) rem[k] = __builtin_fmaf((float)hh[k], -1.0f, v[k]);
-            const f16x4 ll = __builtin_convertvector(rem, f16x4);
-#pragma unroll
-            for (int k = 0; k < 4; ++k) { h[4 * q + k] = hh[k]; l[4 * q + k] = ll[k]; }
-        }
+        w14_point_split8(d, j, h, l);
         _Float16* e = p.v + ((((long long)c * 6 + j) * p.gtot + G) * p.TW + t) * 32;
         *reinterpret_cast<f16x8*>(e + 8 * o) = h;
         *reinterpret_cast<f16x8*>(e + 16 + 8 * o) = l;
@@ -723,8 +701,10 @@
     pv.in = a.in; pv.v = reinterpret_cast<_Float16*>(scratch);
     pv.B = a.B; pv.H = a.H; pv.W = a.W; pv.in_ps = a.in_pix_stride; pv.in_bytes = pw.k.in_bytes; pv.nch = pw.k.nch; pv.TW = TW; pv.gtot = pw.k.gtot;
     pv.items = (long long)a.B * a.H * TW * pv.nch * 2;
-    hipLaunchKernelGGL(wino14_v_kernel, dim3((unsigned)((pv.items + 255) / 256)), dim3(256), 0, stream, pv);
-    OM_CHECK_HIP(hipGetLastError());
+    if (!a.v_ready) {
+        hipLaunchKernelGGL(wino14_v_kernel, dim3((unsigned)((pv.items + 255) / 256)), dim3(256), 0, stream, pv);
+        OM_CHECK_HIP(hipGetLastError());
+    }
     if (a.mid_event) OM_CHECK_HIP(hipEventRecord(a.mid_event, stream));
     const long long total2 = (long long)(pw.k.total_tiles / pw.k.n_tiles) * (pw.k.n_tiles / 2);
     const unsigned grid = (unsigned)(total2 < 256 ? total2 : 256);
diff --git a/orienmask_amd/csrc/om_common.h b/orienmask_amd/csrc/om_common.h
--- a/orienmask_amd/csrc/om_common.h
+++ b/orienmask_amd/csrc/om_common.h
@@ -54,6 +54,7 @@
     int* status = nullptr;
     int ksplit_max = 0;
     int force_bm = 0, force_bn = 0;
+    int v_out = 0, v_ready = 0;
     int nseg = 0;
     const float* seg_ptr[4] = {nullptr, nullptr, nullptr, nullptr};
     int seg_channels[4] = {0, 0, 0, 0}, seg_pix_stride[4] = {0, 0, 0, 0}, seg_up[4] = {1, 1, 1, 1};
@@ -68,6 +69,9 @@
 int launch_conv_igemm(const ConvArgs& a, hipStream_t stream);
 int launch_conv_igemm_split(const ConvArgs& a, hipStream_t stream);
 void conv_tile_for_split(int M, int cout_pad, int* bm, int* bn, bool gather = false);
+bool conv_split_v_out_supported(const ConvArgs& a, int out_align_bytes);
+int conv_split_v_out_entries(int W);
+void conv_split_v_out_tile(int B, int H, int W, int k, int* e);
 
 struct ConvArgsH {
     const void* in;
diff --git a/orienmask_amd/csrc/om_model.cpp b/orienmask_amd/csrc/om_model.cpp
--- a/orienmask_amd/csrc/om_model.cpp
+++ b/orienmask_amd/csrc/om_model.cpp
@@ -65,6 +65,8 @@
     int ksplit_max = 0;
     bool to_side = false;
     bool gather = false;
+    bool v_out = false, v_in = false;
+    size_t out_floats = 0;
 };
 
 static int algo_code(Form f, bool f16) {
@@ -97,13 +99,14 @@
 
 }
 
-enum : int { SW_STEM3 = 0, SW_STEM2_F16 = 1, SW_W14_WIDE = 2 };
+enum : int { SW_STEM3 = 0, SW_STEM2_F16 = 1, SW_W14_WIDE = 2, SW_W14_PAIR = 3 };
 static int switch_default(const char* env) {
     const char* e = std::getenv(env);
     return (e && e[0] == '1') ? 0 : 1;
 }
 static std::atomic<int>& switch_flag(int which) {
-    static std::atomic<int> flags[3] = {{switch_default("OM_NO_STEM3")}, {switch_default("OM_NO_STEM2_F16")}, {switch_default("OM_NO_W14_WIDE")}};
+    static std::atomic<int> flags[4] = {{switch_default("OM_NO_STEM3")}, {switch_default("OM_NO_STEM2_F16")}, {switch_default("OM_NO_W14_WIDE")},
+                                        {switch_default("OM_NO_W14_PAIR")}};
     return flags[which];
 }
 static bool switch_on(int which) { return switch_flag(which).load(std::memory_order_relaxed) != 0; }
@@ -379,6 +382,51 @@
                    ? 2 : 1;
     }
 
+    int pair_consumer(int index, int B, int H, int W) const {
+        if (!switch_on(SW_W14_PAIR) || !switch_on(SW_W14_WIDE) || precision != 1 || keep_all || !om::wino_enabled()) return -1;
+        if (latency_cells > 0 && (long long)B * (H / 32) * (W / 32) < latency_cells) return -1;
+        const om::LayerDef& P = layers[index];
+        const om_layer_info& pi = P.info;
+        if (P.stem || pi.ksize != 1 || pi.stride != 1 || pi.cout_pad % 128 != 0 || pi.cout != pi.cout_pad || pi.cin % 32 != 0 || P.has_res ||
+            P.out_mode != 0 || P.side >= 0 || P.out.buf < 0 || P.out.ch_off != 0 || bufs[P.out.buf].C != pi.cout || pi.wsplit_off < 0 ||
+            pi.wino_planes != 0 || !pair_adopted(P.in_div))
+            return -1;
+        int reader = -1;
+        for (int r = 0; r < (int)layers.size(); ++r) {
+            const om::LayerDef& R = layers[r];
+            if (r != index && R.out.buf == P.out.buf) return -1;
+            bool reads = R.in.buf == P.out.buf || (R.has_res && R.res.buf == P.out.buf);
+            for (const auto& sg : R.gather) reads = reads || sg.view.buf == P.out.buf;
+            if (!reads) continue;
+            if (reader >= 0) return -1;
+            reader = r;
+        }
+        if (reader <= index) return -1;
+        const om::LayerDef& C = layers[reader];
+        const om_layer_info& ci = C.info;
+        if (C.in.buf != P.out.buf || C.in.ch_off != 0 || ci.cin != pi.cout || ci.ksize != 3 || ci.stride != 1 || ci.wino_planes == 0 ||
+            C.in_div != P.in_div || C.out.buf < 0 || (C.has_res && (C.res.buf < 0 || C.res.buf == P.out.buf)) || ci.wsplit_off < 0)
+            return -1;
+        int R = 0, Ct = 0, ncb = 0, nrb = 0;
+        om::wino14_geometry(B, H / C.in_div, W / C.in_div, &R, &Ct, &ncb, &nrb);
+        if (ci.cin < 512 || (long long)nrb * ncb * (ci.cout_pad / 64) <= 256) return -1;
+        om::ConvArgs a{};
+        om::fill_conv_shape(a, B, H / C.in_div, W / C.in_div, ci.cin, pix_stride(C.in.buf), ci.cout, ci.cout_pad, 3, 1, ci.leaky,
+                            C.has_res ? pix_stride(C.res.buf) : 0, pix_stride(C.out.buf), C.out_mode, C.up);
+        if (!om::wino14_wide_supported(a, 256, view_align_bytes(C.out, false), C.has_res, C.has_res ? view_align_bytes(C.res, false) : 0)) return -1;
+        om::ConvArgs b{};
+        om::fill_conv_shape(b, B, H / P.in_div, W / P.in_div, pi.cin, pix_stride(P.in.buf), pi.cout, pi.cout_pad, 1, 1, pi.leaky, 0, pi.cout);
+        return om::conv_split_v_out_supported(b, 256) ? reader : -1;
+    }
+    int pair_producer(int index, int B, int H, int W) const {
+        const om::LayerDef& C = layers[index];
+        if (C.info.ksize != 3 || C.in.buf < 0) return -1;
+        for (int w = 0; w < index; ++w)
+            if (layers[w].out.buf == C.in.buf) return pair_consumer(w, B, H, W) == index ? w : -1;
+        return -1;
+    }
+    static bool pair_adopted(int div) { return div == 32; }
+
     template <class Args>
     void layer_shape(Args& a, const om::LayerDef& L, const om::LayerPlan& p, int B, int H, int W) const {
         const om_layer_info& li = L.info;
@@ -435,6 +483,10 @@
             }
             p.form = Form::Wino14; p.bm = 128; p.bn = 64;
             p.w_off = li.wsplit_off; p.scale_off = li.wsplit_scale_off;
+            if (pair_producer(index, B, H, W) >= 0) {
+                p.form = Form::Wino14Wide; p.bn = 128; p.v_in = true;
+                return p;
+            }
             int R = 0, Ct = 0, ncb = 0, nrb = 0;
             om::wino14_geometry(B, Hin, Win, &R, &Ct, &ncb, &nrb);
             if (switch_on(SW_W14_WIDE) && li.cin >= 512 && (long long)nrb * ncb * (li.cout_pad / 64) > 256 && L.in.buf >= 0 && L.out.buf >= 0 && (!L.has_res || L.res.buf >= 0)) {
@@ -463,6 +515,10 @@
             p.to_side = on_read && L.side >= 0; p.gather = on_read && !L.gather.empty();
             p.form = p.gather ? Form::SplitGather : Form::Split;
             om::conv_tile_for_split(B * Ho * Wo, li.cout_pad, &p.bm, &p.bn, p.gather);
+            if (pair_consumer(index, B, H, W) >= 0) {
+                p.v_out = true; p.bm = p.bn = 128;
+                p.out_floats = om::wino14_wide_scratch_floats(B, Ho, Wo, li.cout);
+            }
         } else {
             p.form = Form::Igemm;
             om::conv_tile_for(B * Ho * Wo, li.cout_pad, &p.bm, &p.bn);
@@ -500,6 +556,7 @@
             touch(L.in.buf); touch(L.out.buf);
             if (L.has_res) touch(L.res.buf);
             if (p.to_side) touch(L.side);
+            if (p.v_out) items[L.out.buf].bytes = std::max(items[L.out.buf].bytes, om::align_up(p.out_floats * sizeof(float), 256));
             if (p.gather)
                 for (const auto& sg : L.gather)
                     if (sg.producer >= 0) touch(layers[sg.producer].side);
@@ -660,7 +717,8 @@
         a.status = status;
         a.ksplit_max = p.ksplit_max;
         a.split = p.form == Form::Wino14 || p.form == Form::Wino14Wide ? 1 : 0;
-        float* scratch = reinterpret_cast<float*>(workspace + lay->scratch_off[index]);
+        a.v_out = p.v_out ? 1 : 0; a.v_ready = p.v_in ? 1 : 0;
+        float* scratch = p.v_in ? reinterpret_cast<float*>(buf(L.in.buf)) : reinterpret_cast<float*>(workspace + lay->scratch_off[index]);
         switch (p.form) {
             case Form::Wino: case Form::WinoFused: a.mid_event = ev.ev_mid; return om::launch_conv_winograd(a, scratch, stream);
             case Form::Wino24: a.mid_event = ev.ev_mid; return om::launch_conv_winograd24(a, scratch, stream);
@@ -1199,6 +1257,79 @@
     return om::launch_conv_wino14_wide(a, static_cast<float*>(scratch), static_cast<hipStream_t>(stream));
 }
 
+int om_set_wino14_pair(int on) {
+    OM_REQUIRE(on == 0 || on == 1, OM_EINVAL, "om_set_wino14_pair: %d", on);
+    switch_flag(SW_W14_PAIR).store(on, std::memory_order_relaxed);
+    return OM_OK;
+}
+int om_get_wino14_pair(void) { return switch_on(SW_W14_PAIR) ? 1 : 0; }
+
+int om_layer_pair(const om_model* m, int index, int B, int H, int W) {
+    OM_REQUIRE(m && index >= 0 && index < (int)m->layers.size() && B > 0 && H > 0 && W > 0 && H % 32 == 0 && W % 32 == 0, OM_EINVAL,
+               "om_layer_pair: bad argument");
+    const int c = m->pair_consumer(index, B, H, W);
+    return c >= 0 ? c : m->pair_producer(index, B, H, W);
+}
+
+int om_conv2d_wino14_pair_tiles(int B, int H, int W, int* entries_per_tile, long long* m_tiles) {
+    OM_REQUIRE(B > 0 && H > 0 && W > 0 && (long long)B * H * W < (1ll << 31) && entries_per_tile && m_tiles, OM_EINVAL,
+               "om_conv2d_wino14_pair_tiles: bad argument");
+    const int n = om::conv_split_v_out_entries(W);
+    *entries_per_tile = n;
+    *m_tiles = ((long long)B * H * ((W + 3) / 4) + n - 1) / n;
+    return OM_OK;
+}
+
+int om_conv2d_wino14_pair_tile(int B, int H, int W, long long tile, int* entry_first, int* entry_end, int* pixel_first, int* pixel_last) {
+    int n = 0;
+    long long tiles = 0;
+    if (int rc = om_conv2d_wino14_pair_tiles(B, H, W, &n, &tiles)) return rc;
+    OM_REQUIRE(tile >= 0 && tile < tiles && entry_first && entry_end && pixel_first && pixel_last, OM_EINVAL,
+               "om_conv2d_wino14_pair_tile: tile %lld of %lld", tile, tiles);
+    int e[4];
+    om::conv_split_v_out_tile(B, H, W, (int)tile, e);
+    *entry_first = e[0]; *entry_end = e[1]; *pixel_first = e[2]; *pixel_last = e[3];
+    return OM_OK;
+}
+
+int om_conv2d_split_v(int nseg, const float* const* seg_ptr, const int* seg_channels, const int* seg_pix_stride, const int* seg_up, int B,
+                      int H, int W, const void* w_split, const float* scale_split, const float* shift, int cout, int leaky, void* v,
+                      size_t v_bytes, int32_t* status_dev, om_stream stream) {
+    OM_REQUIRE(B > 0 && H > 0 && W > 0 && nseg >= 1 && nseg <= 4 && seg_ptr && seg_channels && seg_pix_stride && seg_up && cout > 0 &&
+                   cout % 16 == 0,
+               OM_EINVAL, "om_conv2d_split_v: bad shape / null segment table (nseg=%d)", nseg);
+    OM_REQUIRE(v && v_bytes >= om_conv2d_wino14_wide_scratch_bytes(B, H, W, cout), OM_ENOMEM, "om_conv2d_split_v: V too small");
+    om::ConvArgs a;
+    a.w = static_cast<const float*>(w_split); a.scale = scale_split; a.shift = shift; a.res = nullptr; a.out = static_cast<float*>(v);
+    int cin = 0;
+    for (int g = 0; g < nseg; ++g) cin += seg_channels[g];
+    const bool plain = nseg == 1 && seg_up[0] == 1;
+    a.in = plain ? seg_ptr[0] : nullptr;
+    if (!plain) {
+        a.nseg = nseg;
+        for (int g = 0; g < nseg; ++g) {
+            a.seg_ptr[g] = seg_ptr[g]; a.seg_channels[g] = seg_channels[g]; a.seg_pix_stride[g] = seg_pix_stride[g]; a.seg_up[g] = seg_up[g];
+        }
+    }
+    om::fill_conv_shape(a, B, H, W, cin, plain ? seg_pix_stride[0] : 0, cout, om::round_up(cout, 32), 1, 1, leaky, 0, cout);
+    a.status = status_dev; a.v_out = 1;
+    if (int rc = unit_ticket(static_cast<hipStream_t>(stream), &a.ticket)) return rc;
+    return om::launch_conv_igemm_split(a, static_cast<hipStream_t>(stream));
+}
+
+int om_conv2d_wino14_wide_v(const void* v, int B, int H, int W, int cin, const void* u14_split, const float* scale_split, const float* shift,
+                            int cout, int leaky, const float* res, int res_pix_stride, float* out, int out_pix_stride, int32_t* status_dev,
+                            om_stream stream) {
+    OM_REQUIRE(B > 0 && H > 0 && W > 0 && v, OM_EINVAL, "om_conv2d_wino14_wide_v: bad argument");
+    om::ConvArgs a;
+    a.in = static_cast<const float*>(v);
+    a.w = static_cast<const float*>(u14_split); a.scale = scale_split; a.shift = shift; a.res = res; a.out = out;
+    om::fill_conv_shape(a, B, H, W, cin, cin, cout, om::round_up(cout, 64), 3, 1, leaky, res_pix_stride, out_pix_stride);
+    a.split = 1; a.status = status_dev; a.v_ready = 1;
+    if (int rc = unit_ticket(static_cast<hipStream_t>(stream), &a.ticket)) return rc;
+    return om::launch_conv_wino14_wide(a, static_cast<float*>(const_cast<void*>(v)), static_cast<hipStream_t>(stream));
+}
+
 int om_set_wino14_wide(int on) {
     OM_REQUIRE(on == 0 || on == 1, OM_EINVAL, "om_set_wino14_wide: %d", on);
     switch_flag(SW_W14_WIDE).store(on, std::memory_order_relaxed);
diff --git a/orienmask_amd/csrc/wino14_shared.h b/orienmask_amd/csrc/wino14_shared.h
--- a/orienmask_amd/csrc/wino14_shared.h
+++ b/orienmask_amd/csrc/wino14_shared.h
@@ -49,6 +49,66 @@
     t.R = k ? p.cls[1].R : p.cls[0].R;
     t.Ct = k ? p.cls[1].Ct : p.cls[0].Ct;
     t.g0 = rb * t.R; t.t0 = (k ? p.cls[1].t0 : p.cls[0].t0) + cb * t.Ct; t.n0 = t.tile_n * W14_BN;
+}
+
+__device__ __forceinline__ f32x4 w14_point(const f32x4 (&d)[6], int j) {
+    const f32x4 c4 = 4.f, cm4 = -4.f, c2 = 2.f, cm2 = -2.f, cm5 = -5.f;
+    switch (j) {
+        case 0: return __builtin_elementwise_fma(d[2], cm5, __builtin_elementwise_fma(d[0], c4, d[4]));
+        case 1: return __builtin_elementwise_fma(d[1] + d[2], cm4, d[3] + d[4]);
+        case 2: return __builtin_elementwise_fma(d[1] - d[2], c4, d[4] - d[3]);
+        case 3: return __builtin_elementwise_fma(d[3] - d[1], c2, d[4] - d[2]);
+        case 4: return __builtin_elementwise_fma(d[3] - d[1], cm2, d[4] - d[2]);
+        default: return __builtin_elementwise_fma(d[3], cm5, __builtin_elementwise_fma(d[1], c4, d[5]));
+    }
+}
+
+__device__ __forceinline__ void w14_point_split8(const f32x4 (&d)[2][6], int j, f16x8& h, f16x8& l) {
+#pragma unroll
+    for (int q = 0; q < 2; ++q) {
+        const f32x4 v = w14_point(d[q], j);
+        const f16x4 hh = __builtin_convertvector(v, f16x4);
+        f32x4 rem;
+#pragma unroll
+        for (int k = 0; k < 4; ++k) rem[k] = __builtin_fmaf((float)hh[k], -1.0f, v[k]);
+        const f16x4 ll = __builtin_convertvector(rem, f16x4);
+#pragma unroll
+        for (int k = 0; k < 4; ++k) { h[4 * q + k] = hh[k]; l[4 * q + k] = ll[k]; }
+    }
+}
+
+constexpr int W14_PAIR_BM = 128;
+struct Wino14PairTile {
+    int e0, e1;
+    int p_lo, p_hi;
+};
+__host__ __device__ inline int w14_pair_first_pixel(int W, int TW, int e) {
+    const int row = e / TW, t = e - row * TW;
+    return row * W + (t > 0 ? 4 * t - 1 : 0);
+}
+__host__ __device__ inline int w14_pair_last_pixel(int W, int TW, int e) {
+    const int row = e / TW, t = e - row * TW;
+    return row * W + (4 * t + 4 < W ? 4 * t + 4 : W - 1);
+}
+__host__ __device__ inline void wino14_pair_tile(int W, int TW, int n, int entries, int k, Wino14PairTile& t) {
+    t.e0 = k * n;
+    t.e1 = t.e0 + n < entries ? t.e0 + n : entries;
+    t.p_lo = w14_pair_first_pixel(W, TW, t.e0);
+    t.p_hi = w14_pair_last_pixel(W, TW, t.e1 - 1);
+}
+inline int wino14_pair_entries(int W) {
+    const int TW = (W + 3) / 4;
+    int n = 0;
+    for (int cand = 1; cand <= W14_PAIR_BM; ++cand) {
+        int worst = 0;
+        for (int t0 = 0; t0 < TW; ++t0) {
+            const int rows = w14_pair_last_pixel(W, TW, t0 + cand - 1) - w14_pair_first_pixel(W, TW, t0) + 1;
+            worst = rows > worst ? rows : worst;
+        }
+        if (worst > W14_PAIR_BM) break;
+        n = cand;
+    }
+    return n;
 }
 
 template <int MODE> constexpr int W14_EPI_OPS = MODE == 0 ? 16 : MODE == 1 ? 28 : 0;
diff --git a/orienmask_amd/lib.py b/orienmask_amd/lib.py
--- a/orienmask_amd/lib.py
+++ b/orienmask_amd/lib.py
@@ -118,6 +118,15 @@
     "om_conv2d_wino14_wide": (_i, [_vp, _i, _i, _i, _i, _i, _vp, _vp, _vp, _i, _i, _vp, _i, _vp, _i, _vp, _sz, _vp, _vp]),
     "om_set_wino14_wide": (_i, [_i]),
     "om_get_wino14_wide": (_i, []),
+    "om_set_wino14_pair": (_i, [_i]),
+    "om_get_wino14_pair": (_i, []),
+    "om_layer_pair": (_i, [_vp, _i, _i, _i, _i]),
+    "om_conv2d_wino14_pair_tiles": (_i, [_i, _i, _i, ctypes.POINTER(_i), ctypes.POINTER(ctypes.c_longlong)]),
+    "om_conv2d_wino14_pair_tile": (_i, [_i, _i, _i, ctypes.c_longlong, ctypes.POINTER(_i), ctypes.POINTER(_i), ctypes.POINTER(_i),
+                                        ctypes.POINTER(_i)]),
+    "om_conv2d_split_v": (_i, [_i, ctypes.POINTER(_vp), ctypes.POINTER(_i), ctypes.POINTER(_i), ctypes.POINTER(_i), _i, _i, _i,
+                               _vp, _vp, _vp, _i, _i, _vp, _sz, _vp, _vp]),
+    "om_conv2d_wino14_wide_v": (_i, [_vp, _i, _i, _i, _i, _vp, _vp, _vp, _i, _i, _vp, _i, _vp, _i, _vp, _vp]),
     "om_forward_workspace_bytes": (_sz, [_vp, _i, _i, _i]),
     "om_forward_status_offset": (_sz, [_vp, _i, _i, _i]),
     "om_forward": (_i, [_vp, _vp, _i, _i, _i, _vp, _vp, _vp, _vp, _vp, _sz, _vp]),
diff --git a/orienmask_amd/model.py b/orienmask_amd/model.py
--- a/orienmask_amd/model.py
+++ b/orienmask_amd/model.py
@@ -276,7 +276,7 @@
         _lib.check(L.om_model_set_precision(h, 1 if split else 0), "om_model_set_precision")
         n_sub = self.n_streams if (self.n_streams > 1 and B % self.n_streams == 0) else 1
         Bs = B // n_sub
-        switches = (L.om_get_wino14_wide(), L.om_get_stem_fusion(0), L.om_get_stem_fusion(1))
+        switches = (L.om_get_wino14_wide(), L.om_get_stem_fusion(0), L.om_get_stem_fusion(1), L.om_get_wino14_pair())
         key = (dev, Bs, H, W, f16, n_sub, switches, split)
         cache = self._workspace if slot == 0 else self._slot_workspaces.setdefault(slot, {})
         ws = cache.get(key)
@@ -351,9 +351,23 @@
         mask = bytes(1 if l["name"] in set(names) else 0 for l in self._layers)
         _lib.check(_lib.load().om_profile_enable_layers(h, mask, len(mask)), "om_profile_enable_layers")
 
-    def layer_kernels(self, B, H, W):
+    def layer_pairs(self, B, H, W):
+        if self.precision != "f32_split":
+            return {}
+        h = self._ensure_handle()
+        L = _lib.load()
+        _lib.check(L.om_model_set_precision(h, 1), "om_model_set_precision")
+        names = [l["name"] for l in self._layers]
+        other = [L.om_layer_pair(h, i, B, H, W) for i in range(len(names))]
+        return {names[i]: names[j] for i, j in enumerate(other) if j > i}
+
+    def layer_kernels(self, B, H, W, name_pairs=False):
         h = self._ensure_handle()
         out = []
+        if name_pairs and self.precision == "f32_split":
+            pairs = self.layer_pairs(B, H, W)
+            paired = set(pairs) | set(pairs.values())
+            return [(n, k[:-1] + ",v>" if n in paired else k) for n, k in self.layer_kernels(B, H, W)]
         if self.precision == "f16":
             for i, l in enumerate(self._layers):
                 bm, bn, algo = ctypes.c_int(0), ctypes.c_int(0), ctypes.c_int(0)
```

Result: no change. 2196 (median of 6 runs) (-0.0%).
